# lvrcek/GNNome-assembly

Measured on AMD Instinct MI355X. Metric: GatedGCN edges/sec fwd+bwd, chr19 assembly graph, higher is better.
Workload: dtype f32 (f16x2 split products, f32 accumulate)

## Files before the change

### gnnome_assembly_amd/_lib.py

```python
from __future__ import annotations

import ctypes as C
import os

_HERE = os.path.dirname(os.path.abspath(__file__))
LIB_PATH = os.environ.get("GNM_LIBRARY") or os.path.join(_HERE, "libgnm.so")

_lib = None
ABI_VERSION = 7

_p = C.c_void_p
_i64 = C.c_int64
_i32 = C.c_int
_f32 = C.c_float
_sz = C.c_size_t
_pi = C.POINTER(C.c_int)

SIGNATURES = {
    "gnm_abi_version": (_i32, []),
    "gnm_last_error": (C.c_char_p, []),
    "gnm_num_cus": (_i32, []),
    "gnm_max_partial_blocks": (_i32, []),
    "gnm_graph_build_index": (_i32, [_p, _p, _i64, _i64, _p, _p, _p, _p, _p, _p, _p]),
    "gnm_graph_edge_locality": (_i32, [_p, _p, _i64, _i64, _i64, C.POINTER(C.c_double)]),
    "gnm_graph_locality_order": (_i32, [_p, _p, _i64, _i64, _p, _p, C.POINTER(C.c_double)]),
    "gnm_gemm_f32_workspace_bytes": (_sz, [_i32, _i64, _i64, _i64]),
    "gnm_gemm_f32": (_i32, [_i32, _i64, _i64, _i64, _p, _i64, _p, _i64, _p, _i64, _p, _p, _i64, _i32, _p, _sz, _p]),
    "gnm_gemm_tn_colsum_workspace_bytes": (_sz, [_i64, _i64, _i64]),
    "gnm_gemm_tn_colsum": (_i32, [_i64, _i64, _i64, _p, _i64, _p, _i64, _p, _i64, _p, _p, _sz, _p]),
    "gnm_colsum_workspace_bytes": (_sz, [_i64, _i64]),
    "gnm_colsum_f32": (_i32, [_i64, _i64, _p, _i64, _p, _p, _sz, _p]),
    "gnm_gather_rows_f32": (_i32, [_i64, _i64, _p, _p, _p, _p]),
    "gnm_relu_mask_f32": (_i32, [_i64, _p, _p, _p]),
    "gnm_bn_finalize": (_i32, [_p, _i32, _i64, _i32, _p, _p, _f32, _p, _p]),
    "gnm_bn_bwd_finalize": (_i32, [_p, _i32, _i64, _i32, _p, _p, _p, _p]),
    "gnm_edge_t_stats_fwd": (_i32, [_i64, _i32, _p, _p, _p, _p, _p, _pi, _p]),
    "gnm_edge_gate_fwd": (_i32, [_i64, _i64, _i32, _p, _p, _p, _p, _p, _p, _p, _p, _p, _p]),
    "gnm_node_agg_src_fwd": (_i32, [_i64, _i64, _i32, _p, _p, _p, _p, _p, _p, _p, _p, _p, _p, _pi, _p]),
    "gnm_node_update_fwd": (_i32, [_i64, _i32, _p, _p, _p, _p, _p]),
    "gnm_node_bwd_stats": (_i32, [_i64, _i32, _p, _p, _p, _p, _pi, _p]),
    "gnm_node_bwd_apply": (_i32, [_i64, _i32, _p, _p, _p, _p, _p, _p, _p, _p, _p, _p]),
    "gnm_edge_bwd_dst": (_i32, [_i64, _i64, _i32, _p, _p, _p, _p, _p, _p, _p, _p, _p, _p, _p, _p, _p, _p, _pi, _p]),
    "gnm_edge_bwd_src": (_i32, [_i64, _i64, _i32, _p, _p, _p, _p, _p, _p, _p, _p, _p, _p, _p, _p, _p, _p, _i32, _p]),
    "gnm_edge_bwd_gt": (_i32, [_i64, _i32, _p, _p, _p, _p, _p, _p, _p]),
    "gnm_ln_edge_gate_fwd": (_i32, [_i64, _i64, _i32, _p, _p, _p, _p, _p, _p, _p, _p, _p, _p, _i32, _p]),
    "gnm_ln_node_update_fwd": (_i32, [_i64, _i32, _p, _p, _p, _p, _p, _i32, _p]),
    "gnm_ln_node_bwd": (_i32, [_i64, _i32, _p, _p, _p, _p, _p, _p, _p, _p, _p, _p, _p, _pi, _i32, _p]),
    "gnm_ln_edge_bwd_dst": (_i32, [_i64, _i64, _i32, _p, _p, _p, _p, _p, _p, _p, _p, _p, _p, _p, _p, _pi, _i32, _p]),
    "gnm_ln_edge_bwd_src": (_i32, [_i64, _i64, _i32, _p, _p, _p, _p, _p, _p, _p, _p]),
    "gnm_rowtile_workspace_bytes": (_sz, [_i32]),
    "gnm_set_occupancy_cap": (_i32, [_i32]),
    "gnm_debug_set_variant": (_i32, [C.c_char_p, _i32]),
    "gnm_set_matmul_mode": (_i32, [_i32]),
    "gnm_get_matmul_mode": (_i32, []),
    "gnm_edge_t_fused_fwd": (_i32, [_i64, _i32, _p, _p, _p, _p, _p, _p, _p, _p, _pi, _p, _sz, _p]),
    "gnm_edge_bwd_gt_nn": (_i32, [_i64, _i32, _p, _p, _p, _p, _p, _p, _p, _p, _p, _sz, _p]),
    "gnm_node_proj_fwd": (_i32, [_i64, _i32, _i32, _p, _p, _p, _p, _p, _sz, _p]),
    "gnm_node_proj_bwd_workspace_bytes": (_sz, [_i32]),
    "gnm_node_proj_bwd": (_i32, [_i64, _i32, _i32, _p, _p, _p, _p, _p, _p, _p, _p, _p, _sz, _p]),
    "gnm_node_proj_bwd_nn": (_i32, [_i64, _i32, _i32, _p, _p, _p, _p, _p, _sz, _p]),
    "gnm_node_proj_bwd_tn": (_i32, [_i64, _i32, _i32, _p, _p, _p, _p, _p, _p, _sz, _i32, _p]),
    "gnm_node_proj_bwd_nn_stats": (_i32, [_i64, _i32, _i32, _p, _p, _p, _p, _p, _p, _p, _pi, _p, _sz, _p]),
    "gnm_tn128_bgrad": (_i32, [_i64, _i32, _p, _p, _p, _i64, _p, _p, _p, _p, _p, _p, _p, _p, _p, _p, _p, _sz, _p]),
    "gnm_edge_bwd_chain": (_i32, [_i64, _i64, _i32] + [_p] * 24 + [_pi, _p, _sz, _p]),
    "gnm_edge_bwd_chain_src": (_i32, [_i64, _i64, _i32] + [_p] * 24 + [_p, _i64, _p] + [_pi, _p, _sz, _p]),
    "gnm_edge_bwd_top": (_i32, [_i64, _i64, _i32] + [_p] * 15 + [_p, _i64, _p, _pi, _p, _sz, _p]),
    "gnm_edge_bwd_src_fix": (_i32, [_i64, _p, _i64, _i64, _i32] + [_p] * 10 + [_p]),
    "gnm_node_bgrad": (_i32, [_i64, _i32] + [_p] * 8 + [_i64, _p, _p]),
    "gnm_graph_build_sweep_plan": (_i32, [_p, _p, _p, _i64, _i64, _i64, _i32, _i32, _i64, _p, _p, _p, C.POINTER(C.c_int64), _pi]),
    "gnm_graph_build_sweep_plan_device": (_i32, [_p, _p, _p, _i64, _i64, _i64, _i32, _i32, _i64, _p, _p, _p, _p, _p, _p, _p, _p]),
    "gnm_sweep_partition": (_i32, [_i64, _i32, C.POINTER(C.c_int64), _pi]),
    "gnm_edge_gate2_fwd": (_i32, [_i64, _i64, _i32] + [_p] * 9 + [_i64, _i64] + [_p] * 11 + [_pi, _p]),
    "gnm_ln_edge_gate2_fwd": (_i32, [_i64, _i64, _i32] + [_p] * 4 + [_i32] + [_p] * 6 + [_i64, _i64] + [_p] * 11 + [_pi, _p]),
    "gnm_edge_bwd_fused_workspace_bytes": (_sz, []),
    "gnm_edge_bwd_fused": (_i32, [_i64, _i32, _p, _p, _p, _p, _p, _p, _p, _p, _p, _p, _p, _p, _sz, _p]),
    "gnm_edge_bwd_fused_gt": (_i32, [_i64, _i32, _p, _p, _p, _p, _p, _p, _p, _p, _p, _sz, _p]),
    "gnm_ln_edge_bwd_top": (_i32, [_i64, _i64, _i32, _p, _p, _p, _p, _p, _i32, _p, _p, _p, _p, _p, _p, _p, _p, _p, _p, _p, _i64, _p, _p, _sz, _p]),
    "gnm_ln_edge_bwd_chain": (_i32, [_i64, _i64, _i32, _p, _p, _p, _p, _p, _p, _p, _p, _p, _p, _i32, _p, _p, _p, _p, _p, _p, _p, _p, _p, _p, _p, _i64,
                                     _p, _p, _sz, _p]),
    "gnm_ln_edge_bwd_src_fix": (_i32, [_i64, _p, _i64, _i64, _i32, _p, _p, _p, _p, _p, _p, _p, _p]),
    "gnm_edge_encoder_fwd": (_i32, [_i64, _i32, _i32, _i32, _p, _p, _p, _p, _p, _p, _p, _p]),
    "gnm_edge_encoder_bwd_workspace_bytes": (_sz, []),
    "gnm_edge_encoder_bwd": (_i32, [_i64, _i32, _i32, _i32, _p, _p, _p, _p, _p, _p, _p, _p, _p, _p, _p, _sz, _p]),
    "gnm_edge_encoder_bwd_dx": (_i32, [_i64, _i32, _i32, _i32, _p, _p, _p, _p, _p, _p, _p, _p, _p, _p, _p, _p, _sz, _p]),
    "gnm_predictor_score_fwd": (_i32, [_i64, _i32, _p, _p, _p, _p, _p, _p, _p, _p, _p]),
    "gnm_predictor_score_bwd": (_i32, [_i64, _i32, _p, _p, _p, _p, _p, _pi, _p]),
    "gnm_predictor_fused_workspace_bytes": (_sz, []),
    "gnm_predictor_fused_fwd": (_i32, [_i64, _i32, _i32, _p, _p, _i64, _p, _p, _p, _p, _p, _p, _p, _p, _p, _p, _sz, _p]),
    "gnm_predictor_fused_bwd": (_i32, [_i64, _i32, _i32, _p, _p, _p, _p, _p, _p, _i64, _p, _p, _p, _p, _p, _sz, _p]),
    "gnm_tn128_workspace_bytes": (_sz, []),
    "gnm_tn128": (_i32, [_i64, _p, _i64, _i32, _p, _p, _p, _p, _p, _sz, _p]),
    "gnm_compose_workspace_bytes": (_sz, [_i32]),
    "gnm_compose_partials_doubles": (_sz, []),
    "gnm_layer_forward": (_i32, [_p, _i32, _p, _p, _p, _p]),
    "gnm_stack_backward": (_i32, [_p, _i32, _i32, _p, _p, _p, _p, _p, _p, _p, _p, _p]),
    "gnm_decode_build_adjacency": (_i32, [_p, _p, _i64, _i64, _p, _p, _p, _p, _p, _p]),
    "gnm_decode_iteration": (_i64, [_i64, _p, _p, _p, _p, _p, _p, _p, _p, _p, _p, _i32, _p, _p, _i32, _p, _i64, _p]),
    "gnm_decode_iteration_mt": (_i64, [_i64, _p, _p, _p, _p, _p, _p, _p, _p, _p, _p, _i32, _p, _p, _i32, _p, _i64, _p, _i32]),
    "gnm_decode_sample_workspace_bytes": (_sz, [_i64]),
    "gnm_decode_candidate_sums": (_i32, [_i64, _i64, _p, _p, _p, _p, _p, _sz, _p, _p, _p]),
    "gnm_decode_pick": (_i32, [_i64, _i64, _p, _p, _p, _p, _p, _p, _i32, _p, _p, _p]),
    "gnm_reduce_partials": (_i32, [_p, _i32, _i32, _i32, _p, _p]),
    "gnm_seg_sum_rows": (_i32, [_i64, _i32, _p, _p, _p, _p, _i64, _p]),
    "gnm_pagerank_pe_workspace_bytes": (_sz, [_i64]),
    "gnm_pagerank_pe": (_i32, [_i64, _i64, _p, _p, _p, _i32, C.c_double, _p, _p, _sz, _p]),
    "gnm_edge_feats_zscore": (_i32, [_i64, _p, _p, _p, _p, _sz, _p]),
    "gnm_bce_fwd_bwd": (_i32, [_i64, _p, _p, _f32, _p, _p, _p, _sz, _p]),
}


class GnmError(RuntimeError):
    pass


def load():
    global _lib
    if _lib is not None:
        return _lib
    if not os.path.exists(LIB_PATH):
        raise GnmError(
            f"{LIB_PATH} not found: build it with `python __graft_entry__.py` (hipcc --offload-arch=gfx950). "
            "There is no CPU fallback for the product path.")
    lib = C.CDLL(LIB_PATH)
    for name, (res, args) in SIGNATURES.items():
        try:
# ... 56 lines not shown
```

### gnnome_assembly_amd/csrc/gnm_fused.hip

```cpp
#include <string.h>
#include <type_traits>

#include "gnm_common.h"
#include "gnm_tr.h"

namespace gnm {

typedef float floatx16 __attribute__((ext_vector_type(16)));

constexpr int FH = 128;
constexpr int FTR = 64;
constexpr int FP = FH + 4;
constexpr int FKQ = FH / 8;

using full_t = std::true_type;
using ragged_t = std::false_type;

__global__ void pack_w_k(const float* __restrict__ W, int64_t ld, int ncb, int nn, float* __restrict__ Wp) {
  const int total = ncb * FKQ * 64;
  for (int idx = blockIdx.x * blockDim.x + threadIdx.x; idx < total; idx += gridDim.x * blockDim.x) {
    const int lane = idx & 63, q = (idx >> 6) % FKQ, cb = idx / (64 * FKQ);
    const int i = lane & 31, g = lane >> 5;
    float v[4];
#pragma unroll
// ... 1711 lines not shown

template <class MM>
static int node_proj_fwd_impl(int64_t N, int ncols, const float* h, const float* W, const float* b, float* Pout,
                              void* ws, void* stream) {
  hipStream_t st = (hipStream_t)stream;
  launch_pack<MM>(W, FH, ncols / 32, 0, ws, st);
  GNM_LAUNCH_CHECK("pack_w (NT, node)");
  const int64_t ntiles = cdiv_(N, FTR);
  if constexpr (MM::kSplit) {
    const int ncg = ncols / FH;
    int nslot = (num_cus() * occ_blocks<rowtile_nt_k<MM, false, 1>>()) / ncg / kXcds * kXcds;
    if (nslot > (int)((ntiles + kXcds - 1) / kXcds * kXcds)) nslot = (int)((ntiles + kXcds - 1) / kXcds * kXcds);
    if (nslot < kXcds) nslot = kXcds;
    hipLaunchKernelGGL((rowtile_nt_k<MM, false, 1>), dim3(nslot * ncg), dim3(kBlock), 0, st, N, h, (const void*)ws, b,
                       Pout, (int64_t)ncols, (const float*)nullptr, (const int32_t*)nullptr,
                       (const int32_t*)nullptr, (double*)nullptr, cdiv_(ntiles, nslot), ncg);
  } else {
    const int grid = persistent_grid(ntiles, 2, occ_blocks<rowtile_nt_k<MM, false, 5>>());
    hipLaunchKernelGGL((rowtile_nt_k<MM, false, 5>), dim3(grid), dim3(kBlock), 0, st, N, h, (const void*)ws, b, Pout,
                       (int64_t)ncols, (const float*)nullptr, (const int32_t*)nullptr,
                       (const int32_t*)nullptr, (double*)nullptr, cdiv_(ntiles, grid), 1);
  }
  GNM_LAUNCH_CHECK("node_proj_fwd");
  return 0;
}

extern "C" int gnm_node_proj_fwd(int64_t N, int H, int ncols, const float* h, const float* W, const float* b,
                                 float* Pout, void* ws, size_t ws_bytes, void* stream) {
  GNM_CHECK_ARG(H == FH, "node_proj_fwd: H=%d (only 128 is built)", H);
  GNM_CHECK_ARG(N > 0 && ncols == 5 * FH && h && W && b && Pout, "node_proj_fwd: bad argument (ncols must be 5*128)");
  GNM_CHECK_ARG(ws && ws_bytes >= gnm_rowtile_workspace_bytes(ncols), "node_proj_fwd: workspace too small");
  return g_matmul_mode == 2 ? node_proj_fwd_impl<MmH2>(N, ncols, h, W, b, Pout, ws, stream)
         : g_matmul_mode  ? node_proj_fwd_impl<MmB3>(N, ncols, h, W, b, Pout, ws, stream)
                          : node_proj_fwd_impl<MmF32>(N, ncols, h, W, b, Pout, ws, stream);
}

namespace gnm {
int edge_bwd_chain_launch(const ChainArgs& in, const float* W3, void* wpack, hipStream_t st, bool h2 = false);
}
extern "C" size_t gnm_edge_bwd_fused_workspace_bytes(void);

static int edge_bwd_chain_impl(int64_t N, int64_t E, int H, const float* ge, float* ge_out, const float* t_hi,
                               const float* e_mid, const float* stat_hi, const float* bstat_hi, const float* gamma_hi,
                               const float* W3_hi, float* gW3_hi, float* gb3_hi, double* partials_hi,
                               const float* t_lo, const float* stat_lo, const float* P_lo, const float* Q_lo,
                               const float* hf_lo, const float* hb_lo, const int32_t* isrc, const int32_t* idst,
                               const int32_t* in_ptr, float* gP_lo, float* Ud_lo, float* Td_lo, double* partials_lo,
                               const uint32_t* sinfo, int64_t plan_nodes_per_block, float* UT_lo,
                               int* nblk_out, void* ws, size_t ws_bytes, void* stream) {
  GNM_CHECK_ARG(H == FH, "edge_bwd_chain: H=%d (only 128 is built)", H);
  GNM_CHECK_ARG(g_matmul_mode >= 1, "edge_bwd_chain: only built for the split matmul modes");
  GNM_CHECK_ARG(N > 0 && E > 0 && ge && ge_out && t_hi && e_mid && stat_hi && bstat_hi && gamma_hi && W3_hi && gW3_hi &&
                    gb3_hi && partials_hi && t_lo && stat_lo && P_lo && Q_lo && hf_lo && hb_lo && isrc && idst && in_ptr &&
                    gP_lo && Ud_lo && Td_lo && partials_lo && nblk_out && partials_hi != partials_lo,
                "edge_bwd_chain: null / aliased argument");
  GNM_CHECK_ARG(ws && ws_bytes >= gnm_edge_bwd_fused_workspace_bytes(), "edge_bwd_chain: workspace %zu < %zu", ws_bytes,
                gnm_edge_bwd_fused_workspace_bytes());
  hipStream_t st = (hipStream_t)stream;
  float* slab = (float*)((char*)ws + gnm_rowtile_workspace_bytes(FH));
  ChainArgs a{};
  a.E = E; a.N = N;
  a.ge = ge; a.ge_out = ge_out; a.t_hi = t_hi; a.e_mid = e_mid;
  a.stat_hi = stat_hi; a.bstat_hi = bstat_hi; a.gamma_hi = gamma_hi;
  a.slab = slab; a.partials = partials_hi;
  a.t_lo = t_lo; a.stat_lo = stat_lo; a.P_lo = P_lo; a.Q_lo = Q_lo; a.hf_lo = hf_lo; a.hb_lo = hb_lo;
  a.isrc = isrc; a.idst = idst; a.in_ptr = in_ptr;
  a.gP_lo = gP_lo; a.Ud_lo = Ud_lo; a.Td_lo = Td_lo; a.partials_lo = partials_lo;
  a.sinfo = sinfo; a.UT_lo = UT_lo; a.margin = kSweepMargin;
  a.ud_pitch = Td_lo == Ud_lo + FH ? 2 * FH : FH;
  int64_t npb = 0;
  gnm_sweep_partition(N, 1, &npb, nullptr);
  GNM_CHECK_ARG((npb + 2 * kSweepMargin) * 5 * FH * 4 < (int64_t)INT32_MAX, "edge_bwd_chain: %lld nodes per workgroup exceed the 32-bit buffer offsets",
                (long long)npb);
  if (sinfo) {
    GNM_CHECK_ARG(UT_lo, "edge_bwd_chain_src: UT_lo is null");
    GNM_CHECK_ARG(plan_nodes_per_block == npb, "edge_bwd_chain_src: the sweep plan was built for %lld nodes per workgroup, the kernel uses %lld "
                  "(gnm_sweep_partition(N, 1))", (long long)plan_nodes_per_block, (long long)npb);
  }
  const int grid = edge_bwd_chain_launch(a, W3_hi, ws, st, g_matmul_mode == 2);
  GNM_LAUNCH_CHECK("edge_bwd_chain");
  hipLaunchKernelGGL(slab_reduce_k, dim3(FH * FH / 128), dim3(256), 0, st, (const float*)slab, grid, FH * FH, gW3_hi);
  GNM_LAUNCH_CHECK("edge_bwd_chain slab reduce");
  *nblk_out = grid;
  return gnm_reduce_partials(partials_hi, grid, 1, FH, gb3_hi, stream) ? -3 : 0;
}

extern "C" int gnm_edge_bwd_top(int64_t N, int64_t E, int H, float* ge, const float* e_out, const float* t,
                                const float* stat_e, const float* P, const float* Q, const float* hf, const float* hb,
                                const int32_t* isrc, const int32_t* idst, const int32_t* in_ptr, float* gP, float* Ud,
                                float* Td, double* partials, const uint32_t* sinfo, int64_t plan_nodes_per_block,
                                float* UT, int* nblk_out, void* ws, size_t ws_bytes, void* stream) {
  GNM_CHECK_ARG(H == FH || (H == 2 * FH && sinfo), "edge_bwd_top: H=%d (128; 256 with a sweep plan, one sweep per 128-column half)", H);
  GNM_CHECK_ARG(N > 0 && E > 0 && ge && e_out && t && stat_e && P && Q && hf && hb && isrc && idst && in_ptr && gP && Ud &&
                    Td && partials && nblk_out && (!sinfo || UT), "edge_bwd_top: null argument");
  GNM_CHECK_ARG(ws && ws_bytes >= gnm_edge_bwd_fused_workspace_bytes(), "edge_bwd_top: workspace %zu < %zu", ws_bytes,
                gnm_edge_bwd_fused_workspace_bytes());
  int64_t npb = 0;
  gnm_sweep_partition(N, 1, &npb, nullptr);
  GNM_CHECK_ARG((npb + 2 * kSweepMargin) * 5 * H * 4 < (int64_t)INT32_MAX, "edge_bwd_top: %lld nodes per workgroup exceed the 32-bit buffer offsets",
                (long long)npb);
  GNM_CHECK_ARG(!sinfo || plan_nodes_per_block == npb, "edge_bwd_top: the sweep plan was built for %lld nodes per workgroup, the kernel uses %lld",
                (long long)plan_nodes_per_block, (long long)npb);
  for (int c0 = 0; c0 < H; c0 += FH) {
    ChainArgs a{};
    a.E = E; a.N = N; a.hfull = H;
    a.ge = ge + c0; a.ge_out = ge + c0; a.e_mid = e_out + c0;
    a.slab = (float*)((char*)ws + gnm_rowtile_workspace_bytes(FH));
    a.t_lo = t + c0; a.stat_lo = stat_e + c0; a.P_lo = P + c0; a.Q_lo = Q + c0; a.hf_lo = hf + c0; a.hb_lo = hb + c0;
    a.isrc = isrc; a.idst = idst; a.in_ptr = in_ptr;
    a.gP_lo = gP + c0; a.Ud_lo = Ud + c0; a.Td_lo = Td + c0; a.partials_lo = partials + c0;
    a.sinfo = sinfo; a.UT_lo = UT ? UT + c0 : nullptr; a.margin = kSweepMargin;
    a.ud_pitch = Td == Ud + H ? 2 * H : H;
    const int g = edge_bwd_chain_launch(a, nullptr, nullptr, (hipStream_t)stream);
    GNM_CHECK_ARG(g > 0, "edge_bwd_top: no kernel for this configuration");
    *nblk_out = g;
    GNM_LAUNCH_CHECK("edge_bwd_top");
  }
  return 0;
}

extern "C" int gnm_ln_edge_bwd_top(int64_t N, int64_t E, int H, float* ge, const float* e_out, const float* t, const float* gamma_e,
                                   const float* beta_e, int width, const float* P, const float* Q, const float* hf, const float* hb,
                                   const int32_t* isrc, const int32_t* idst, const int32_t* in_ptr, float* gP, float* gt,
                                   double* partials, const uint32_t* sinfo, int64_t plan_nodes_per_block, int* nblk_out, void* ws,
                                   size_t ws_bytes, void* stream) {
  GNM_CHECK_ARG(H == FH, "ln_edge_bwd_top: H=%d (only 128 is built)", H);
  GNM_CHECK_ARG(width >= 1 && width <= H, "ln_edge_bwd_top: width must be in [1, H]");
  GNM_CHECK_ARG(N > 0 && E > 0 && ge && e_out && t && gamma_e && beta_e && P && Q && hf && hb && isrc && idst && in_ptr && gP && gt &&
                    partials && sinfo && nblk_out, "ln_edge_bwd_top: null argument");
  GNM_CHECK_ARG(ws && ws_bytes >= gnm_edge_bwd_fused_workspace_bytes(), "ln_edge_bwd_top: workspace %zu < %zu", ws_bytes,
                gnm_edge_bwd_fused_workspace_bytes());
  int64_t npb = 0;
  gnm_sweep_partition(N, 1, &npb, nullptr);
  GNM_CHECK_ARG((npb + 2 * kSweepMargin) * 5 * H * 4 < (int64_t)INT32_MAX, "ln_edge_bwd_top: %lld nodes per workgroup exceed the 32-bit buffer offsets",
                (long long)npb);
  GNM_CHECK_ARG(plan_nodes_per_block == npb, "ln_edge_bwd_top: the sweep plan was built for %lld nodes per workgroup, the kernel uses %lld",
                (long long)plan_nodes_per_block, (long long)npb);
  ChainArgs a{};
  a.E = E; a.N = N; a.hfull = H;
  a.ge = ge; a.ge_out = ge; a.e_mid = e_out;
  a.slab = (float*)((char*)ws + gnm_rowtile_workspace_bytes(FH));
  a.t_lo = t; a.P_lo = P; a.Q_lo = Q; a.q_pitch = 4 * H; a.qb_off = 2 * H; a.hf_lo = hf; a.hb_lo = hb;
  a.isrc = isrc; a.idst = idst; a.in_ptr = in_ptr;
  a.gP_lo = gP; a.Ud_lo = gP + 4 * H; a.Td_lo = gP + 4 * H; a.ud_pitch = 5 * H;
  a.UT_lo = gP + 3 * H; a.ut_pitch = 5 * H;
  a.partials_lo = partials;
  a.sinfo = sinfo; a.margin = kSweepMargin;
  a.ln_gamma = gamma_e; a.ln_beta = beta_e; a.ln_width = width; a.gt_out = gt;
  const int g = edge_bwd_chain_launch(a, nullptr, nullptr, (hipStream_t)stream);
  GNM_CHECK_ARG(g > 0, "ln_edge_bwd_top: no kernel for this configuration");
  *nblk_out = g;
  GNM_LAUNCH_CHECK("ln_edge_bwd_top");
  return 0;
}

extern "C" int gnm_ln_edge_bwd_chain(int64_t N, int64_t E, int H, float* ge, const float* gt_hi, const float* e_mid, const float* W3_hi,
                                     float* gW3_hi, float* gb3_hi, double* partials_hi, const float* t_lo, const float* gamma_lo,
                                     const float* beta_lo, int width, const float* P_lo, const float* Q_lo, const float* hf_lo,
                                     const float* hb_lo, const int32_t* isrc, const int32_t* idst, const int32_t* in_ptr, float* gP_lo,
                                     float* gt_lo, double* partials_lo, const uint32_t* sinfo, int64_t plan_nodes_per_block,
                                     int* nblk_out, void* ws, size_t ws_bytes, void* stream) {
  GNM_CHECK_ARG(H == FH, "ln_edge_bwd_chain: H=%d (only 128 is built)", H);
  GNM_CHECK_ARG(g_matmul_mode >= 1, "ln_edge_bwd_chain: only built for the split matmul modes");
  GNM_CHECK_ARG(width >= 1 && width <= H, "ln_edge_bwd_chain: width must be in [1, H]");
  GNM_CHECK_ARG(N > 0 && E > 0 && ge && gt_hi && e_mid && W3_hi && gW3_hi && gb3_hi && partials_hi && t_lo && gamma_lo && beta_lo && P_lo &&
// ... 272 lines not shown
  GNM_LAUNCH_CHECK("pack_w (NN, node, stats)");
  constexpr int T = 4;
  const int64_t ngroups = cdiv_(N, NR3 * T);
  const int grid = persistent_grid(ngroups, 1, h2 ? occ_blocks<rowtile_nn2_k<MmH2, T>>() : occ_blocks<rowtile_nn2_k<MmB3, T>>());
  const Nn2Args a{N, gP, (int64_t)ncols, ncg, (const void*)ws, gh_out, gh_in, cdiv_(ngroups, grid), z_lo, stat_h_lo, partials};
  if (h2) hipLaunchKernelGGL((rowtile_nn2_k<MmH2, T>), dim3(grid), dim3(kBlock), 0, st, a);
  else hipLaunchKernelGGL((rowtile_nn2_k<MmB3, T>), dim3(grid), dim3(kBlock), 0, st, a);
  *nblk_out = grid;
  GNM_LAUNCH_CHECK("node_proj_bwd_nn_stats");
  return 0;
}

extern "C" int gnm_node_proj_bwd_tn(int64_t N, int H, int ncols, const float* gP, const float* h_in, float* gW, float* gb,
                                    double* partials, void* ws, size_t ws_bytes, int max_blocks_per_cu, void* stream) {
  GNM_CHECK_ARG(H == FH, "node_proj_bwd_tn: H=%d (only 128 is built)", H);
  GNM_CHECK_ARG(N > 0 && ncols > 0 && ncols % FH == 0 && gP && h_in && gW && gb && partials && max_blocks_per_cu >= 0,
                "node_proj_bwd_tn: bad argument");
  GNM_CHECK_ARG(ws && ws_bytes >= gnm_node_proj_bwd_workspace_bytes(ncols), "node_proj_bwd_tn: workspace too small");
  float* slab = (float*)((char*)ws + gnm_rowtile_workspace_bytes(ncols));
  return tn_colgroups(N, gP, ncols, ncols / FH, h_in, gW, gb, partials, slab, stream, max_blocks_per_cu);
}

extern "C" int gnm_node_proj_bwd(int64_t N, int H, int ncols, const float* gP, const float* h_in, const float* W,
                                 const float* gh_out, float* gh_in, float* gW, float* gb, double* partials,
                                 void* ws, size_t ws_bytes, void* stream) {
  GNM_CHECK_ARG(ws && ws_bytes >= gnm_node_proj_bwd_workspace_bytes(ncols), "node_proj_bwd: workspace too small");
  const int rc = gnm_node_proj_bwd_nn(N, H, ncols, gP, W, gh_out, gh_in, ws, ws_bytes, stream);
  return rc ? rc : gnm_node_proj_bwd_tn(N, H, ncols, gP, h_in, gW, gb, partials, ws, ws_bytes, 0, stream);
}

extern "C" size_t gnm_tn128_workspace_bytes(void) { return (size_t)kMaxPartialBlocks * FH * FH * sizeof(float); }

extern "C" int gnm_tn128(int64_t M, const float* A, int64_t lda, int ncg, const float* B, float* out, float* colsum,
                         double* partials, void* ws, size_t ws_bytes, void* stream) {
  GNM_CHECK_ARG(M > 0 && A && B && out && colsum && partials && ncg > 0 && lda >= (int64_t)ncg * FH && ncg <= 16,
                "tn128: bad argument");
  GNM_CHECK_ARG(ws && ws_bytes >= gnm_tn128_workspace_bytes(), "tn128: workspace too small");
  return tn_colgroups(M, A, lda, ncg, B, out, colsum, partials, (float*)ws, stream);
}

extern "C" int gnm_tn128_bgrad(int64_t M, int H, const float* UT, const float* Ud, const float* Td, int64_t ud_pitch,
                               const float* stat_e, const float* bstat_e, const float* gamma_e, const int32_t* in_ptr,
                               const int32_t* out_ptr, float* gP, const float* B, float* out, float* colsum,
                               double* partials, void* ws, size_t ws_bytes, void* stream) {
  GNM_CHECK_ARG(H == FH, "tn128_bgrad: H=%d (only 128 is built)", H);
  GNM_CHECK_ARG(g_matmul_mode >= 1, "tn128_bgrad: split matmul modes only");
  GNM_CHECK_ARG(M > 0 && UT && Ud && Td && (ud_pitch == H || ud_pitch == 2 * H) && stat_e && bstat_e && gamma_e && in_ptr &&
                    out_ptr && gP && B && out && colsum && partials, "tn128_bgrad: bad argument");
  GNM_CHECK_ARG(ws && ws_bytes >= gnm_tn128_workspace_bytes(), "tn128_bgrad: workspace too small");
  const TnConv cv{{UT, Ud}, {UT + H, Td}, {(int64_t)2 * H, ud_pitch}, {out_ptr, in_ptr}, stat_e, bstat_e, gamma_e,
                  gP + 3 * H, (int64_t)5 * H};
  return tn_colgroups(M, nullptr, 0, 2, B, out, colsum, partials, (float*)ws, stream, 0, &cv);
}
```

### gnnome_assembly_amd/csrc/gnm_sweep.hip

```cpp
#include <type_traits>

#include "gnm_tr.h"
#include "gnm_ln.h"

namespace gnm {

int gate2_wg();
constexpr int GT = 512;
constexpr int GR = kSweepTileRows;
typedef unsigned int u32x4g_ __attribute__((ext_vector_type(4)));

struct Gate2Args {
  int64_t N, E;
  const float* t; const float* e_in; const float* stat; const float* P;
  const int32_t* isrc; const int32_t* idst; const int32_t* in_ptr;
  const uint32_t* sinfo; const uint32_t* dinfo;
  float* e_out; float* hf; float* inv_f; float* hb; float* inv_b;
  int64_t nodes_per_block, margin;
  const float* gamma; const float* beta; int width;
};

constexpr int G2_LDS = 3 * GR * SW * 4 + 2 * kSweepSlots * SW * 4 + 2 * 2 * SW * 4 + 2 * SW * 4 + 3 * 4 * GR * 4;

__device__ __forceinline__ u32x4g_ bits4g(const float4& v) {
  const u32x4g_ b = {__builtin_bit_cast(unsigned, v.x), __builtin_bit_cast(unsigned, v.y),
                     __builtin_bit_cast(unsigned, v.z), __builtin_bit_cast(unsigned, v.w)};
  return b;
}

template <bool RES, bool INV, int HF, bool LN = false>
__global__ __launch_bounds__(GT, 4) void edge_gate2_fwd_k(const Gate2Args a) {
  static_assert(!LN || HF == SW, "the LayerNorm sweep is built for 128-wide layers");
  __shared__ __attribute__((aligned(16))) unsigned char lds[G2_LDS];
  float* i1 = reinterpret_cast<float*>(lds);
  float* i2 = i1 + GR * SW;
  float* i3 = i2 + GR * SW;
  float* sslots = i3 + GR * SW;
  float* dslots = sslots + 2 * kSweepSlots * SW;
  float* cs = dslots + 2 * 2 * SW;
  int* ring = reinterpret_cast<int*>(cs + 2 * SW);
  const int tid = threadIdx.x;
  const int row = tid >> 5, c4 = (tid & 31) * 4;
  const int chunk = xcd_chunk(blockIdx.x, gridDim.x);
  const int64_t v0 = (int64_t)chunk * a.nodes_per_block < a.N ? (int64_t)chunk * a.nodes_per_block : a.N;
  const int64_t v1 = v0 + a.nodes_per_block < a.N ? v0 + a.nodes_per_block : a.N;
  const int64_t rb = a.in_ptr[v0], re = a.in_ptr[v1];
  const int64_t ntile = (re - rb + GR - 1) / GR;
  for (int c = tid; c < SW; c += GT) {
    cs[c] = LN ? a.gamma[c] : a.stat[2 * HF + c];
    cs[SW + c] = LN ? a.beta[c] : a.stat[3 * HF + c];
  }
  const int64_t vbase = v0 - a.margin;
  const int nspan = (int)(v1 - v0 + 2 * a.margin);
  const __amdgpu_buffer_rsrc_t rs_e = __builtin_amdgcn_make_buffer_rsrc(a.e_out + rb * HF, 0, (int)(re - rb) * HF * 4, 0x00020000);
  const __amdgpu_buffer_rsrc_t rs_hf = __builtin_amdgcn_make_buffer_rsrc(a.hf + v0 * HF, 0, (int)(v1 - v0) * HF * 4, 0x00020000);
  const __amdgpu_buffer_rsrc_t rs_if = __builtin_amdgcn_make_buffer_rsrc(INV ? a.inv_f + v0 * HF : a.hf, 0, INV ? (int)(v1 - v0) * HF * 4 : 0, 0x00020000);
  const __amdgpu_buffer_rsrc_t rs_hb = __builtin_amdgcn_make_buffer_rsrc(a.hb + vbase * HF, 0, nspan * HF * 4, 0x00020000);
  const __amdgpu_buffer_rsrc_t rs_ib = __builtin_amdgcn_make_buffer_rsrc(INV ? a.inv_b + vbase * HF : a.hb, 0, INV ? nspan * HF * 4 : 0, 0x00020000);
  __syncthreads();
  if (ntile == 0) return;

  float4 ptA, peA = f4(0.f), ptB, peB = f4(0.f), ptC, peC = f4(0.f);
  float4 ga2, ga3;
  int fs = 0, fd = 0;
  unsigned fi = 0, fj = 0;
  const int64_t klast = ntile - 1;
  auto clamp_row = [&](int64_t k) __attribute__((always_inline)) {
    const int64_t left = re - (rb + k * GR);
    const int nv = left < GR ? (int)left : GR;
    return row < nv ? row : nv - 1;
  };
  auto prefetch_idx = [&](int64_t k) __attribute__((always_inline)) {
    const int cr = clamp_row(k);
    const int64_t r = rb + k * GR + cr;
    fs = a.isrc[r];
    fd = a.idst[r];
    const unsigned w1 = a.sinfo[r], w2 = a.dinfo[r];
    fi = cr == row ? w1 : 0u;
    fj = cr == row ? w2 : 0u;
  };
  auto prefetch_rows = [&](int64_t k, float4& pt, float4& pe_) __attribute__((always_inline)) {
    const int64_t o = (rb + k * GR + clamp_row(k)) * HF + c4;
    pt = ld4_nt(a.t + o);
    if constexpr (RES) pe_ = ld4_nt(a.e_in + o);
  };
  auto gather = [&](int64_t s, int64_t d) __attribute__((always_inline)) {
    ga2 = ld4(a.P + s * (5 * HF) + HF + c4);
    ga3 = ld4(a.P + d * (5 * HF) + 2 * HF + c4);
  };
  auto ring_put = [&](int64_t k) __attribute__((always_inline)) {
    if ((tid & 31) == 0) {
      int* rk = ring + (int)(k % 3) * 4 * GR;
      rk[row] = fs;
      rk[GR + row] = fd;
      rk[2 * GR + row] = (int)fi;
      rk[3 * GR + row] = (int)fj;
    }
  };
  prefetch_idx(0);
  ring_put(0);
  const int s0 = fs, d0 = fd;
  prefetch_idx(klast < 1 ? klast : 1);
  prefetch_rows(0, ptA, peA);
  prefetch_rows(klast < 1 ? klast : 1, ptB, peB);
  prefetch_rows(klast < 2 ? klast : 2, ptC, peC);
  gather(s0, d0);
  const float4 sc = ld4(cs + c4), sh = ld4(cs + SW + c4);
  const float4 ln_live = LN ? live_mask(c4, a.width) : f4(1.f);
  const float ln_inv_w = LN ? 1.0f / (float)a.width : 0.f;
  auto tile = [&](int64_t k, float4& pt, float4& pe_) __attribute__((always_inline)) {
    const int64_t r0 = rb + k * GR;
    const int nvalid = re - r0 < GR ? (int)(re - r0) : GR;
    const int* rk = ring + (int)(k % 3) * 4 * GR;
    {
      const bool live = row < nvalid;
      float4 x = pt;
      if constexpr (LN) {
        float rstd;
        x = row_normalize<SW>(pt, ln_live, ln_inv_w, rstd);
      }
      const float4 eo = relu4(fma4(x, sc, sh)) + pe_;
      __builtin_amdgcn_raw_buffer_store_b128(bits4g(eo), rs_e, live ? (int)(((k * GR + row) * HF + c4) * 4) : (int)0x80000000, 0, 2);
      const float4 sg = live ? sigmoid4(eo) : f4(0.f);
      st4(i1 + row * SW + c4, sg * ga2);
      st4(i2 + row * SW + c4, sg);
      st4(i3 + row * SW + c4, sg * ga3);
      ring_put(k + 1);
    }
    __syncthreads();
    prefetch_idx(k + 2 < klast ? k + 2 : klast);
    prefetch_rows(k + 3 < klast ? k + 3 : klast, pt, pe_);
    {
      const int* rn = ring + (int)((k + 1) % 3) * 4 * GR;
      gather(rn[row], rn[GR + row]);
    }
    {
      const unsigned wd = (unsigned)rk[3 * GR + row], ws_ = (unsigned)rk[2 * GR + row];
      const unsigned md = wd & 0xffffu;
      unsigned ms = ws_ & 0xffffu;
      const int nd = __builtin_popcount(md);
      float4 dn_ = ld4(i1 + row * SW + c4), dd = ld4(i2 + row * SW + c4);
      float4 sn_ = ld4(i3 + row * SW + c4), sdn = dd;
      float* pd = dslots + ((wd >> 16) & 1u) * SW + c4;
      float* ps = sslots + ((ws_ >> 16) & (kSweepSlots - 1)) * SW + c4;
      const float4 e1 = ld4(pd), e2 = ld4(pd + 2 * SW);
      const float4 q1 = ld4(ps), q2 = ld4(ps + kSweepSlots * SW);
      float4 x1[3] = {f4(0.f), f4(0.f), f4(0.f)}, x2[3] = {f4(0.f), f4(0.f), f4(0.f)};
#pragma unroll
      for (int j = 0; j < 3; ++j) {
        if (j + 1 < nd) {
          x1[j] = ld4(i1 + (row + 1 + j) * SW + c4);
          x2[j] = ld4(i2 + (row + 1 + j) * SW + c4);
        }
      }
#pragma unroll
      for (int j = 0; j < 3; ++j) {
        dn_ += x1[j];
        dd += x2[j];
      }
      for (int j = 4; j < nd; ++j) {
        dn_ += ld4(i1 + (row + j) * SW + c4);
        dd += ld4(i2 + (row + j) * SW + c4);
      }
      ms &= ms - 1;
      while (ms) {
        const int b = __builtin_ctz(ms);
        ms &= ms - 1;
        sn_ += ld4(i3 + b * SW + c4);
        sdn += ld4(i2 + b * SW + c4);
      }
      const bool ld_ = md != 0, ls_ = (ws_ & 0xffffu) != 0;
      if (ld_ && !(wd & kSweepOpen)) { dn_ += e1; dd += e2; }
      if (ls_ && !(ws_ & kSweepOpen)) { sn_ += q1; sdn += q2; }
      if (ld_ && !(wd & kSweepClose)) { st4(pd, dn_); st4(pd + 2 * SW, dd); }
      if (ls_ && !(ws_ & kSweepClose)) { st4(ps, sn_); st4(ps + kSweepSlots * SW, sdn); }
      const bool outd = ld_ && (wd & kSweepClose), outs = ls_ && (ws_ & kSweepClose);
      if (__builtin_amdgcn_ballot_w64(outd) != 0) {
        const float4 inv = make_float4(1.f / (dd.x + kEpsDen), 1.f / (dd.y + kEpsDen), 1.f / (dd.z + kEpsDen), 1.f / (dd.w + kEpsDen));
        const int o = outd ? ((rk[GR + row] - (int)v0) * HF + c4) * 4 : (int)0x80000000;
        __builtin_amdgcn_raw_buffer_store_b128(bits4g(dn_ * inv), rs_hf, o, 0, 2);
        if constexpr (INV) __builtin_amdgcn_raw_buffer_store_b128(bits4g(inv), rs_if, o, 0, 2);
      }
      if (__builtin_amdgcn_ballot_w64(outs) != 0) {
        const float4 inv = make_float4(1.f / (sdn.x + kEpsDen), 1.f / (sdn.y + kEpsDen), 1.f / (sdn.z + kEpsDen), 1.f / (sdn.w + kEpsDen));
        const int o = outs ? ((rk[row] - (int)vbase) * HF + c4) * 4 : (int)0x80000000;
        __builtin_amdgcn_raw_buffer_store_b128(bits4g(sn_ * inv), rs_hb, o, 0, 2);
        if constexpr (INV) __builtin_amdgcn_raw_buffer_store_b128(bits4g(inv), rs_ib, o, 0, 2);
      }
    }
    __syncthreads();
  };
  for (int64_t k = 0; k < ntile; k += 3) {
    tile(k, ptA, peA);
    if (k + 1 < ntile) tile(k + 1, ptB, peB);
    if (k + 2 < ntile) tile(k + 2, ptC, peC);
  }
}

template <int HF>
__global__ __launch_bounds__(256) void gate2_empty_segments_k(int64_t N, const int32_t* __restrict__ in_ptr,
                                                              float* __restrict__ hf, float* __restrict__ inv_f) {
  const int lane = threadIdx.x & 63;
  const int64_t wave0 = ((int64_t)blockIdx.x * 4 + (threadIdx.x >> 6)) * 64;
  const int64_t stride = (int64_t)gridDim.x * 4 * 64;
  for (int64_t base = wave0; base < N; base += stride) {
    const int64_t v = base + lane;
    const bool empty = v < N && in_ptr[v + 1] == in_ptr[v];
    unsigned long long m = __ballot(empty);
    while (m) {
      const int b = __ffsll((long long)m) - 1;
      m &= m - 1;
      const int64_t u = base + b;
      const int c4 = (lane & 31) * 4;
      if (lane < 32) st4(hf + u * HF + c4, f4(0.f));
      else if (inv_f) st4(inv_f + u * HF + c4, f4(1.f / kEpsDen));
    }
  }
}

template <int HF>
__global__ __launch_bounds__(kBlock, 8) void node_agg_src_fix_k(int64_t nfix, const int32_t* __restrict__ fix_nodes,
                                                                const float* __restrict__ e_out, const float* __restrict__ P,
                                                                const int32_t* __restrict__ out_ptr,
                                                                const int32_t* __restrict__ out_pos,
                                                                const int32_t* __restrict__ out_dst, float* __restrict__ hb,
                                                                float* __restrict__ inv_b) {
  constexpr int H = SW, G = H / 4, RPW = 64 / G;
  const int lane = threadIdx.x & 63;
  const int wave = __builtin_amdgcn_readfirstlane(threadIdx.x >> 6);
  const int sub = lane / G, c4 = (lane % G) * 4;
  for (int64_t i = (int64_t)blockIdx.x * kWavesPerBlock + wave; i < nfix; i += (int64_t)gridDim.x * kWavesPerBlock) {
    const int64_t v = fix_nodes[i];
    if (v < 0) continue;
    const int a = out_ptr[v], b = out_ptr[v + 1];
    float4 num = f4(0.f), den = f4(0.f);
    for (int64_t m = a + sub; m < b; m += RPW) {
      const int64_t j = out_pos[m], d = out_dst[m];
      const float4 sg = sigmoid4(ld4_nt(e_out + j * HF + c4));
      num = fma4(sg, ld4(P + d * (5 * HF) + 2 * HF + c4), num);
      den += sg;
    }
#pragma unroll
    for (int off = G; off < 64; off <<= 1) {
      num += shfl_xor4(num, off);
      den += shfl_xor4(den, off);
    }
    if (sub == 0) {
      const float4 inv = make_float4(1.f / (den.x + kEpsDen), 1.f / (den.y + kEpsDen), 1.f / (den.z + kEpsDen),
                                     1.f / (den.w + kEpsDen));
      st4_nt(hb + v * HF + c4, num * inv);
      if (inv_b) st4_nt(inv_b + v * HF + c4, inv);
    }
  }
}

template <int HF>
__global__ __launch_bounds__(kBlock) void node_z_stats_k(int64_t N, const float* __restrict__ P, const float* __restrict__ hf,
                                                         const float* __restrict__ hb, float* __restrict__ z,
                                                         double* __restrict__ partials, int64_t rows_per_block) {
  constexpr int H = SW, G = H / 4, RPW = 64 / G;
  __shared__ double lds[kWavesPerBlock * 2 * H];
  const int lane = threadIdx.x & 63, wave = threadIdx.x >> 6;
  const int sub = lane / G, c4 = (lane % G) * 4;
  const int chunk = xcd_chunk(blockIdx.x, gridDim.x);
  const int64_t r0 = (int64_t)chunk * rows_per_block;
  const int64_t r1 = min(N, r0 + rows_per_block);
  Stat4 st;
  st.zero();
  for (int64_t v = r0 + wave * RPW + sub; v < r1; v += kWavesPerBlock * RPW) {
    const float4 zz = ld4_nt(P + v * (5 * HF) + c4) + ld4_nt(hf + v * HF + c4) + ld4_nt(hb + v * HF + c4);
    st4_nt(z + v * HF + c4, zz);
    st.add_prod(zz, zz);
  }
  block_stat_store<H, HF>(st, lds, partials, chunk);
}

}

using namespace gnm;

extern "C" int gnm_sweep_partition(int64_t N, int wg_per_cu, int64_t* nodes_per_block, int* grid_out) {
  GNM_CHECK_ARG(N > 0 && nodes_per_block && wg_per_cu >= 1 && wg_per_cu <= 8, "sweep_partition: bad argument");
  const int grid = persistent_grid(N, 64, wg_per_cu, 8);
  *nodes_per_block = (N + grid - 1) / grid;
  if (grid_out) *grid_out = grid;
  return 0;
}

static int edge_gate2_fwd_impl(int64_t N, int64_t E, int H, const float* t, const float* e_in, const float* stat_e,
                               const float* ln_gamma, const float* ln_beta, int ln_width,
                               const float* P, const int32_t* isrc, const int32_t* idst, const int32_t* in_ptr,
                               const uint32_t* sinfo, const uint32_t* dinfo, int64_t plan_nodes_per_block,
                               int64_t nfix, const int32_t* fix_nodes, const int32_t* out_ptr, const int32_t* out_pos,
                               const int32_t* out_dst, float* e_out, float* hf, float* inv_f, float* hb, float* inv_b,
                               float* z, double* partials, int* nblk_out, void* stream) {
  GNM_CHECK_ARG(H == SW || (H == 2 * SW && !ln_gamma), "edge_gate2_fwd: H=%d (128 and 256 are built; LayerNorm: 128)", H);
  GNM_CHECK_ARG(N > 0 && E > 0 && t && (stat_e || ln_gamma) && P && isrc && idst && in_ptr && sinfo && dinfo && (nfix == 0 || fix_nodes) &&
                    nfix >= 0 && out_ptr && out_pos && out_dst && e_out && hf && hb && z && partials && nblk_out &&
                    (inv_f != nullptr) == (inv_b != nullptr),
                "edge_gate2_fwd: null/neg argument");
  hipStream_t st = (hipStream_t)stream;
  Gate2Args a{};
  a.N = N; a.E = E; a.t = t; a.e_in = e_in; a.stat = stat_e; a.P = P; a.isrc = isrc; a.idst = idst; a.in_ptr = in_ptr;
  a.sinfo = sinfo; a.dinfo = dinfo; a.e_out = e_out; a.hf = hf; a.inv_f = inv_f; a.hb = hb; a.inv_b = inv_b;
  a.margin = kSweepMargin;
  a.gamma = ln_gamma; a.beta = ln_beta; a.width = ln_width;
  int grid = 0;
  gnm_sweep_partition(N, gate2_wg(), &a.nodes_per_block, &grid);
  GNM_CHECK_ARG(plan_nodes_per_block == a.nodes_per_block, "edge_gate2_fwd: the sweep plan was built for %lld nodes per workgroup, the "
                "kernel uses %lld (gnm_sweep_partition(N, %d))", (long long)plan_nodes_per_block, (long long)a.nodes_per_block, gate2_wg());
  GNM_CHECK_ARG((a.nodes_per_block + 2 * kSweepMargin) * H * 4 < (int64_t)INT32_MAX && (E / grid + 64) * H * 4 < (int64_t)INT32_MAX,
                "edge_gate2_fwd: a workgroup's share exceeds the 32-bit buffer offsets");
  const int gz = H == SW ? persistent_grid(N, 256, occ_blocks<node_z_stats_k<SW>>()) : persistent_grid(N, 256, occ_blocks<node_z_stats_k<2 * SW>>());
  auto run = [&](auto hf_tag, int c0) -> int {
    constexpr int HF = decltype(hf_tag)::value;
    Gate2Args b = a;
    b.t = t + c0; b.e_in = e_in ? e_in + c0 : nullptr; b.stat = stat_e ? stat_e + c0 : nullptr; b.P = P + c0; b.e_out = e_out + c0; b.hf = hf + c0;
    b.inv_f = inv_f ? inv_f + c0 : nullptr; b.hb = hb + c0; b.inv_b = inv_b ? inv_b + c0 : nullptr;
    hipLaunchKernelGGL(gate2_empty_segments_k<HF>, dim3(num_cus() * 2), dim3(256), 0, st, N, in_ptr, b.hf, b.inv_f);
    auto launch = [&](auto ln_tag) {
      constexpr bool LN_ = decltype(ln_tag)::value;
      if (e_in && inv_f) hipLaunchKernelGGL((edge_gate2_fwd_k<true, true, HF, LN_>), dim3(grid), dim3(GT), 0, st, b);
      else if (e_in) hipLaunchKernelGGL((edge_gate2_fwd_k<true, false, HF, LN_>), dim3(grid), dim3(GT), 0, st, b);
      else if (inv_f) hipLaunchKernelGGL((edge_gate2_fwd_k<false, true, HF, LN_>), dim3(grid), dim3(GT), 0, st, b);
      else hipLaunchKernelGGL((edge_gate2_fwd_k<false, false, HF, LN_>), dim3(grid), dim3(GT), 0, st, b);
    };
    if constexpr (HF == SW) {
      if (ln_gamma) launch(std::true_type{});
      else launch(std::false_type{});
    } else {
      launch(std::false_type{});
    }
    GNM_LAUNCH_CHECK("edge_gate2_fwd");
    if (nfix > 0) {
      int64_t g2 = (nfix + kWavesPerBlock - 1) / kWavesPerBlock;
      const int64_t cap = (int64_t)num_cus() * 8;
      if (g2 > cap) g2 = cap;
      hipLaunchKernelGGL(node_agg_src_fix_k<HF>, dim3((int)g2), dim3(kBlock), 0, st, nfix, fix_nodes, b.e_out, b.P, out_ptr, out_pos,
                         out_dst, b.hb, b.inv_b);
      GNM_LAUNCH_CHECK("edge_gate2_fwd fix");
    }
    hipLaunchKernelGGL(node_z_stats_k<HF>, dim3(gz), dim3(kBlock), 0, st, N, b.P, b.hf, b.hb, z + c0, partials + c0, (N + gz - 1) / gz);
    GNM_LAUNCH_CHECK("edge_gate2_fwd z");
    return 0;
  };
  if (H == SW) {
    if (run(std::integral_constant<int, SW>{}, 0)) return -2;
  } else {
    for (int c0 = 0; c0 < H; c0 += SW)
      if (run(std::integral_constant<int, 2 * SW>{}, c0)) return -2;
  }
  *nblk_out = gz;
  return 0;
}

extern "C" int gnm_edge_gate2_fwd(int64_t N, int64_t E, int H, const float* t, const float* e_in, const float* stat_e,
                                  const float* P, const int32_t* isrc, const int32_t* idst, const int32_t* in_ptr,
                                  const uint32_t* sinfo, const uint32_t* dinfo, int64_t plan_nodes_per_block,
                                  int64_t nfix, const int32_t* fix_nodes, const int32_t* out_ptr, const int32_t* out_pos,
                                  const int32_t* out_dst, float* e_out, float* hf, float* inv_f, float* hb, float* inv_b,
                                  float* z, double* partials, int* nblk_out, void* stream) {
  GNM_CHECK_ARG(stat_e, "edge_gate2_fwd: stat_e is null");
  return edge_gate2_fwd_impl(N, E, H, t, e_in, stat_e, nullptr, nullptr, 0, P, isrc, idst, in_ptr, sinfo, dinfo, plan_nodes_per_block, nfix,
                             fix_nodes, out_ptr, out_pos, out_dst, e_out, hf, inv_f, hb, inv_b, z, partials, nblk_out, stream);
}

extern "C" int gnm_ln_edge_gate2_fwd(int64_t N, int64_t E, int H, const float* t, const float* e_in, const float* gamma_e,
                                     const float* beta_e, int width, const float* P, const int32_t* isrc, const int32_t* idst,
                                     const int32_t* in_ptr, const uint32_t* sinfo, const uint32_t* dinfo, int64_t plan_nodes_per_block,
                                     int64_t nfix, const int32_t* fix_nodes, const int32_t* out_ptr, const int32_t* out_pos,
                                     const int32_t* out_dst, float* e_out, float* hf, float* inv_f, float* hb, float* inv_b,
                                     float* z, double* partials, int* nblk_out, void* stream) {
  GNM_CHECK_ARG(gamma_e && beta_e && width >= 1 && width <= H, "ln_edge_gate2_fwd: null argument or width outside [1, H]");
  return edge_gate2_fwd_impl(N, E, H, t, e_in, nullptr, gamma_e, beta_e, width, P, isrc, idst, in_ptr, sinfo, dinfo, plan_nodes_per_block, nfix,
                             fix_nodes, out_ptr, out_pos, out_dst, e_out, hf, inv_f, hb, inv_b, z, partials, nblk_out, stream);
}
```

### gnnome_assembly_amd/csrc/gnm_tr.h

```cpp
#pragma once
#include "gnm_common.h"

namespace gnm {

typedef float floatx16 __attribute__((ext_vector_type(16)));
typedef __bf16 bf16x8 __attribute__((ext_vector_type(8)));
typedef __bf16 bf16x4 __attribute__((ext_vector_type(4)));
typedef __attribute__((__vector_size__(4 * sizeof(__bf16)))) __bf16 tr_bf16x4;

constexpr int SW = 128;
constexpr int SPITCH = SW * 2;

__device__ __forceinline__ int swz(int r) { return ((r & 3) << 2) | ((0x78 >> (((r >> 2) & 3) * 2)) & 3); }
__device__ __forceinline__ int simg_off(int r, int c) {
  return r * SPITCH + ((((c >> 3) ^ swz(r)) << 4) | ((c & 4) << 1));
}

__device__ __forceinline__ void split3f(const float4& v, bf16x4& hi, bf16x4& mid, bf16x4& lo) {
  const float x[4] = {v.x, v.y, v.z, v.w};
#pragma unroll
  for (int j = 0; j < 4; ++j) {
    const __bf16 h = (__bf16)x[j];
    const float r1 = x[j] - (float)h;
    const __bf16 m = (__bf16)r1;
// ... 124 lines not shown
  const tr_bf16x4 b = __builtin_amdgcn_ds_read_tr16_b64_v4bf16((lds_ptr)(img + base1_x_mb));
  bf16x8 f;
#pragma unroll
  for (int j = 0; j < 4; ++j) {
    f[j] = a[j];
    f[4 + j] = b[j];
  }
  return f;
}

__device__ __forceinline__ h16x8 simg_col_frag_h(const unsigned char* img, int k0, int c0, int lane) {
  return __builtin_bit_cast(h16x8, simg_col_frag(img, k0, c0, lane));
}

typedef float floatx4_acc __attribute__((ext_vector_type(4)));
__device__ __forceinline__ void mfb16s(floatx4_acc& acc, const bf16x8& a, const bf16x8& b) {
  acc = __builtin_amdgcn_mfma_f32_16x16x32_bf16(a, b, acc, 0, 0, 0);
}
__device__ __forceinline__ void mfh16s(floatx4_acc& acc, const h16x8& a, const h16x8& b) {
  acc = __builtin_amdgcn_mfma_f32_16x16x32_f16(a, b, acc, 0, 0, 0);
}
__device__ __forceinline__ void mfb16(floatx16& acc, const bf16x8& a, const bf16x8& b) {
  acc = __builtin_amdgcn_mfma_f32_32x32x16_bf16(a, b, acc, 0, 0, 0);
}

__device__ __forceinline__ constexpr int b3_pa(int t) { return t == 0 ? 2 : (t == 2 || t == 3) ? 1 : 0; }
__device__ __forceinline__ constexpr int b3_pb(int t) { return t == 1 ? 2 : (t == 2 || t == 4) ? 1 : 0; }

struct ChainArgs {
  int64_t E, N;
  const float* ge; float* ge_out; const float* t_hi; const float* e_mid;
  const float* stat_hi; const float* bstat_hi; const float* gamma_hi; const bf16x8* Wp;
  float* slab; double* partials;
  const float* t_lo; const float* stat_lo; const float* P_lo; const float* Q_lo; const float* hf_lo; const float* hb_lo;
  const int32_t* isrc; const int32_t* idst; const int32_t* in_ptr;
  float* gP_lo; float* Ud_lo; float* Td_lo; double* partials_lo;
  int64_t nodes_per_block;
  const uint32_t* sinfo; float* UT_lo; int64_t margin; int ud_pitch;
  int hfull;
  const float* ln_gamma; const float* ln_beta; int ln_width; float* gt_out;
  int ut_pitch;
  int q_pitch, qb_off;
};

struct TnConv {
  const float* U[2]; const float* T[2]; int64_t pitch[2]; const int32_t* ptr[2];
  const float* stat_e; const float* bstat_e; const float* gamma_e;
  float* Xw; int64_t ldxw;
};


constexpr int kSweepTileRows = 16;
constexpr int kSweepSlots = 32;
constexpr int64_t kSweepMargin = 1 << 16;
constexpr unsigned kSweepOpen = 1u << 22, kSweepClose = 1u << 23;

}
```

### gnnome_assembly_amd/csrc/gnm_tr.hip

```cpp
#include <stdlib.h>

#include "gnm_tr.h"
#include "gnm_ln.h"

namespace gnm {

constexpr int TRR = 32;
constexpr int TRIMG = TRR * SPITCH;

__device__ __forceinline__ int h2_tn_da(int R, int P) { const int d = R - P; return d > 0 ? (d > 200 ? 100 : d >> 1) : 0; }
template <bool CONV, int OCC, bool H2 = false>
__global__ __launch_bounds__(kBlock, OCC) void tn_tr_k(int64_t M, const float* __restrict__ A, int64_t lda, int ncg,
                                                     const void* __restrict__ Bv, int64_t ldb, int ncgb,
                                                     float* __restrict__ slab, double* __restrict__ partials, int nslot,
                                                     int64_t tiles_per_slot, const TnConv cv) {
  const float* __restrict__ B = reinterpret_cast<const float*>(Bv);
  __shared__ __attribute__((aligned(16))) unsigned char lds[6 * TRIMG];
  unsigned char* ia = lds;
  unsigned char* ib = lds + 3 * TRIMG;
  const int tid = threadIdx.x, lane = tid & 63;
  const int wave = __builtin_amdgcn_readfirstlane(tid >> 6);
  const int li = lane & 31, lg = lane >> 5;
  const int wn = wave >> 1, wc = wave & 1;
  const int xcd = blockIdx.x % kXcds, jj = blockIdx.x / kXcds;
// ... 572 lines not shown
#pragma unroll
    for (int k = 0; k < 8; ++k) s_ += all[4 * (32 * k + (tid >> 2)) + (tid & 3)];
    partials[(size_t)chunk * SW + tid] = s_;
  }
}

int eb_variant();
size_t edge_bwd_tr_pack_bytes() { return (size_t)(SW / 16) * (SW / 32) * 3 * 64 * sizeof(bf16x8); }
int edge_bwd_tr_launch(int64_t E, const float* ge, float* ge_out, const float* t, const float* e_in, const float* stat_e,
                       const float* bstat_e, const float* gamma_e, const float* W3, void* wpack, float* slab,
                       double* partials, hipStream_t st, bool h2, bool given) {
  if (h2) {
    hipLaunchKernelGGL(pack_w2_nn16_k, dim3(SW / 16), dim3(256), 0, st, W3, (int64_t)SW, (unsigned char*)wpack);
    const int64_t ntiles = (E + ER - 1) / ER;
    const int grid = persistent_grid(ntiles, 16, occ_blocks<edge_bwd_tr_k<3, true>>());
    if (given)
      hipLaunchKernelGGL((edge_bwd_tr_k<7, true>), dim3(grid), dim3(kBlock), 0, st, E, ge, ge_out, t, e_in, stat_e, bstat_e, gamma_e,
                         (const bf16x8*)wpack, slab, partials, (ntiles + grid - 1) / grid);
    else
      hipLaunchKernelGGL((edge_bwd_tr_k<3, true>), dim3(grid), dim3(kBlock), 0, st, E, ge, ge_out, t, e_in, stat_e, bstat_e, gamma_e,
                         (const bf16x8*)wpack, slab, partials, (ntiles + grid - 1) / grid);
    return grid;
  }
  hipLaunchKernelGGL(pack_w3_nn16_k, dim3(8), dim3(256), 0, st, W3, (int64_t)SW, (bf16x8*)wpack);
  const int64_t ntiles = (E + ER - 1) / ER;
  if (given) {
    const int grid = persistent_grid(ntiles, 16, occ_blocks<edge_bwd_tr_k<3>>());
    hipLaunchKernelGGL(edge_bwd_tr_k<7>, dim3(grid), dim3(kBlock), 0, st, E, ge, ge_out, t, e_in, stat_e, bstat_e, gamma_e,
                       (const bf16x8*)wpack, slab, partials, (ntiles + grid - 1) / grid);
    return grid;
  }
  const int var = eb_variant();
  const int grid = persistent_grid(ntiles, 16, occ_blocks<edge_bwd_tr_k<3>>());
#define GNM_EB_LAUNCH(V)                                                                                               \
  hipLaunchKernelGGL(edge_bwd_tr_k<V>, dim3(grid), dim3(kBlock), 0, st, E, ge, ge_out, t, e_in, stat_e, bstat_e, gamma_e, \
                     (const bf16x8*)wpack, slab, partials, (ntiles + grid - 1) / grid)
  if (var == 2) GNM_EB_LAUNCH(0);
  else GNM_EB_LAUNCH(3);
#undef GNM_EB_LAUNCH
  return grid;
}


constexpr int CT = 512;
constexpr int WG_ = 4;
typedef unsigned int u32x4_ __attribute__((ext_vector_type(4)));
constexpr int CH_LDS = 6 * EIMG + ER * EOP * 4 + 7 * SW * 4 + 4 * SW * 4 + 5 * ER * SW * 4 + 3 * 2 * ER * 4;
constexpr int CH_LDS_SRC = CH_LDS + 3 * ER * 4 + ER * SW * 4 + 3 * kSweepSlots * SW * 4;
static_assert(ER == kSweepTileRows, "the sweep plan is built for the chained kernel's tile");
static_assert(CH_LDS % 16 == 0 && CH_LDS_SRC <= 160 * 1024, "LDS layout");

struct W3Frag16 { bf16x8 w[SW / 32][3]; };

template <int ABL, bool SRC, bool WSKIP = true, bool HI = true, int HF = SW, bool H2 = false, bool LN = false>
__global__ __launch_bounds__(CT, 2) void edge_bwd_chain_k(const ChainArgs a) {
  static_assert(HF == SW || !HI, "the chained (matrix) half of the kernel is built for 128-wide layers only");
  static_assert(HI || !H2, "f16x2 belongs to the matrix half");
  static_assert(!LN || (SRC && HF == SW), "the LayerNorm sweep: two-sided, 128 wide");
  __shared__ __attribute__((aligned(16))) unsigned char lds[(SRC ? CH_LDS_SRC : CH_LDS) + (LN ? ER * SW * 4 : 0)];
  unsigned char* ig = lds;
  unsigned char* ie = lds + 3 * EIMG;
  float* og = reinterpret_cast<float*>(lds + 6 * EIMG);
  float* cs = og + ER * EOP;
  float* cl = cs + 7 * SW;
  float* v1 = cl + 4 * SW;
  float* v2 = v1 + ER * SW;
  float* v3 = v2 + ER * SW;
  float* tl = v3 + ER * SW;
  float* ef = tl + ER * SW;
  int* sd = reinterpret_cast<int*>(ef + ER * SW);
  unsigned* si = reinterpret_cast<unsigned*>(sd + 3 * 2 * ER);
  float* v5 = reinterpret_cast<float*>(si + 3 * ER);
  float* slots = v5 + ER * SW;
  float* v6 = slots + 3 * kSweepSlots * SW;
  const int tid = threadIdx.x, lane = tid & 63;
  const int wave = __builtin_amdgcn_readfirstlane(tid >> 6);
  const int li = lane & 31, lg = lane >> 5;
  const int wn = wave >> 2, wc = wave & 3;
  const int chunk = xcd_chunk(blockIdx.x, gridDim.x);
  const int64_t v0 = (int64_t)chunk * a.nodes_per_block < a.N ? (int64_t)chunk * a.nodes_per_block : a.N;
  const int64_t v1n = v0 + a.nodes_per_block < a.N ? v0 + a.nodes_per_block : a.N;
  const int64_t rb = a.in_ptr[v0], re = a.in_ptr[v1n];
  const int64_t ntile = (re - rb + ER - 1) / ER;
  const int row = tid >> 5, lc4 = (tid & 31) * 4;
  for (int c = tid; c < SW; c += CT) {
    if constexpr (HI && !LN) {
      cs[c] = a.stat_hi[c];
      cs[SW + c] = a.stat_hi[SW + c];
      cs[2 * SW + c] = a.stat_hi[2 * SW + c];
      cs[3 * SW + c] = a.stat_hi[3 * SW + c];
      cs[4 * SW + c] = a.bstat_hi[c];
      cs[5 * SW + c] = a.bstat_hi[SW + c];
      cs[6 * SW + c] = a.gamma_hi[c] * a.stat_hi[SW + c];
    }
    if constexpr (LN) {
      cl[2 * SW + c] = a.ln_gamma[c];
      cl[3 * SW + c] = a.ln_beta[c];
    } else {
      cl[c] = a.stat_lo[c];
      cl[SW + c] = a.stat_lo[HF + c];
      cl[2 * SW + c] = a.stat_lo[2 * HF + c];
      cl[3 * SW + c] = a.stat_lo[3 * HF + c];
    }
  }
  W3Frag16 wf;
  h16x8 wfh[H2 ? SW / 32 : 1][2];
  float cinv = 1.f;
  if constexpr (HI && !H2) {
    const bf16x8* p = a.Wp + ((int64_t)wave * (SW / 32) * 3) * 64 + lane;
#pragma unroll
    for (int kc = 0; kc < SW / 32; ++kc)
#pragma unroll
      for (int s_ = 0; s_ < 3; ++s_) wf.w[kc][s_] = p[(kc * 3 + s_) * 64];
  }
  if constexpr (H2) {
    const unsigned char* wp = reinterpret_cast<const unsigned char*>(a.Wp);
    const h16x8* p = reinterpret_cast<const h16x8*>(wp) + ((int64_t)wave * (SW / 32) * 2) * 64 + lane;
#pragma unroll
    for (int kc = 0; kc < SW / 32; ++kc)
#pragma unroll
      for (int s_ = 0; s_ < 2; ++s_) wfh[kc][s_] = p[(kc * 2 + s_) * 64];
    cinv = reinterpret_cast<const float*>(wp + kW2Nn16FragBytes)[wave * 16 + (lane & 15)];
  }
  int* const rexp = reinterpret_cast<int*>(lds + 2 * EIMG);
  float* const rinv = reinterpret_cast<float*>(lds + 2 * EIMG) + ER;
  constexpr int kNoRef = -100000;
  int Rref = kNoRef;
  if constexpr (H2) { if (tid == 0) rexp[2 * ER] = 0; }
  floatx16 tn[2];
#pragma unroll
  for (int x = 0; x < 2; ++x)
#pragma unroll
    for (int e = 0; e < 16; ++e) tn[x][e] = 0.f;
  double cg0 = 0.0, cg1 = 0.0, cg2 = 0.0, cg3 = 0.0;
  const int trq0 = simg_tr_base(lane, 0), trq1 = simg_tr_base(lane, 1);
  const int ni = lane & 15, ng = lane >> 4;
  const int nnb = ni * SPITCH + ((((ni & 3) << 2) | (ng ^ (swz(ni) & 3))) << 4);
  const bool walker = wave < 3 && lane < 32 && !(LN && wave == 1), bnsum = tid >= 256;
  const int role = wave, wc4 = (tid & 31) * 4;
  const int brow = 2 * ((tid - 256) >> 5);
  int cur = -1;
  float4 acc0 = f4(0.f);
  double s_gu[4] = {0.0, 0.0, 0.0, 0.0}, s_gut[4] = {0.0, 0.0, 0.0, 0.0};
  float* const wout = role == 0 ? a.gP_lo + 2 * HF : role == 1 ? a.Td_lo : a.Ud_lo;
  const int wpitch32 = role == 0 ? 5 * HF : a.ud_pitch;
  const __amdgpu_buffer_rsrc_t wrs = __builtin_amdgcn_make_buffer_rsrc(wout + v0 * wpitch32, 0, (int)(v1n - v0) * wpitch32 * 4, 0x00020000);
  float* const dummy_row = a.slab + (size_t)(gridDim.x + chunk) * SW * SW + lc4;
  const int64_t vbase = v0 - a.margin;
  const int nspan = (int)(v1n - v0 + 2 * a.margin);
  const __amdgpu_buffer_rsrc_t srs_g = __builtin_amdgcn_make_buffer_rsrc(
      SRC ? a.gP_lo + vbase * (5 * HF) + HF : a.gP_lo, 0, SRC ? nspan * 5 * HF * 4 : 0, 0x00020000);
  const int utp = a.ut_pitch ? a.ut_pitch : 2 * HF;
  const __amdgpu_buffer_rsrc_t srs_u = __builtin_amdgcn_make_buffer_rsrc(
      SRC ? a.UT_lo + vbase * utp : a.gP_lo, 0, SRC ? nspan * utp * 4 : 0, 0x00020000);
  const int qp = a.q_pitch ? a.q_pitch : 2 * HF, qbo = a.q_pitch ? a.qb_off : HF;
  const float4 ln_live = LN ? live_mask((tid & 31) * 4, a.ln_width) : f4(1.f);
  const float ln_inv_w = LN ? 1.0f / (float)a.ln_width : 0.f;
  __syncthreads();

  float4 pg, pt, pe_, pl;
  float4 gt_keep = f4(0.f);
  int row_ea = 0;
  float4 ga2, gqb, ghb, gqf, ghf, ga3;
  int fs = 0, fd = 0;
  unsigned fi = 0;
  const int64_t klast = ntile - 1;
  auto clamp_row = [&](int64_t k) __attribute__((always_inline)) {
    const int64_t left = re - (rb + k * ER);
    const int nv = left < ER ? (int)left : ER;
    return row < nv ? row : nv - 1;
  };
  auto prefetch_idx = [&](int64_t k) __attribute__((always_inline)) {
    const int cr = clamp_row(k);
    const int64_t r = rb + k * ER + cr;
    fs = a.isrc[r];
    fd = a.idst[r];
    if constexpr (SRC) {
      const unsigned w = a.sinfo[r];
      fi = cr == row ? w : 0u;
    }
  };
  auto prefetch_rows = [&](int64_t k) __attribute__((always_inline)) {
    const int64_t r0 = rb + k * ER;
    const int o = clamp_row(k) * HF + lc4;
    pg = ld4(a.ge + r0 * HF + o);
    if constexpr (HI) pt = ld4(a.t_hi + r0 * HF + o);
    pe_ = ld4(a.e_mid + r0 * HF + o);
    pl = ld4_nt(a.t_lo + r0 * HF + o);
  };
  auto gather = [&](int64_t s, int64_t d) __attribute__((always_inline)) {
    ga2 = ld4(a.P_lo + s * (5 * HF) + HF + lc4);
// ... 210 lines not shown
#pragma unroll
      for (int r4 = 0; r4 < ER; r4 += WG_) {
        int dn[WG_];
        float4 xs[WG_];
#pragma unroll
        for (int q = 0; q < WG_; ++q) {
          dn[q] = __builtin_amdgcn_readfirstlane(sdk[ER + r4 + q]);
          xs[q] = ld4(vsrc + (r4 + q) * SW);
        }
        const int dafter = r4 + WG_ < ER ? __builtin_amdgcn_readfirstlane(sdk[ER + r4 + WG_])
                                         : (k == klast ? -1 : __builtin_amdgcn_readfirstlane(sd[(int)((k + 1) % 3) * 2 * ER + ER]));
#pragma unroll
        for (int q = 0; q < WG_; ++q) {
          const float keep = dn[q] == cur ? 1.f : 0.f;
          acc0 = fma4(acc0, f4(keep), xs[q]);
          cur = dn[q];
          const bool ends = (q + 1 < WG_ ? dn[q + 1] : dafter) != cur;
          const u32x4_ bits = {__builtin_bit_cast(unsigned, acc0.x), __builtin_bit_cast(unsigned, acc0.y),
                               __builtin_bit_cast(unsigned, acc0.z), __builtin_bit_cast(unsigned, acc0.w)};
          if (WSKIP) { if (ends) __builtin_amdgcn_raw_buffer_store_b128(bits, wrs, ((cur - (int)v0) * wpitch32 + wc4) * 4, 0, 0); }
          else __builtin_amdgcn_raw_buffer_store_b128(bits, wrs, ends ? ((cur - (int)v0) * wpitch32 + wc4) * 4 : (int)0x80000000, 0, 0);
        }
      }
    }
    if (!(ABL & 1) && bnsum) {
#pragma unroll
      for (int q = 0; q < 2; ++q) {
        const float4 x = ld4((LN ? v6 : v2) + (brow + q) * SW + wc4);
        const float4 th = ld4(v3 + (brow + q) * SW + wc4);
        s_gu[0] += (double)x.x; s_gu[1] += (double)x.y; s_gu[2] += (double)x.z; s_gu[3] += (double)x.w;
        s_gut[0] += (double)x.x * (double)th.x; s_gut[1] += (double)x.y * (double)th.y;
        s_gut[2] += (double)x.z * (double)th.z; s_gut[3] += (double)x.w * (double)th.w;
      }
    }
    if constexpr (SRC) {
      auto bits4 = [](const float4& v) __attribute__((always_inline)) {
        const u32x4_ b = {__builtin_bit_cast(unsigned, v.x), __builtin_bit_cast(unsigned, v.y),
                          __builtin_bit_cast(unsigned, v.z), __builtin_bit_cast(unsigned, v.w)};
        return b;
      };
      if (!(ABL & 1) && !(ABL & 8) && wave >= 3) {
        const int q = (tid - 192) >> 5;
        const unsigned* sik = si + (int)(k % 3) * ER;
        const int rr[2] = {q, (q + 10) & (ER - 1)};
        unsigned w[2] = {sik[rr[0]], q + 10 < ER ? sik[rr[1]] : 0u};
        float4 s1[2], s2[2], s3[2], p1[2], p2[2], p3[2];
        unsigned m[2];
#pragma unroll
        for (int u = 0; u < 2; ++u) {
          m[u] = w[u] & 0xffffu;
          const int b = rr[u];
          s1[u] = ld4(v5 + b * SW + wc4);
          s2[u] = ld4(v2 + b * SW + wc4);
          s3[u] = ld4(v3 + b * SW + wc4);
          const float* p = slots + ((w[u] >> 16) & (kSweepSlots - 1)) * SW + wc4;
          p1[u] = ld4(p);
          p2[u] = ld4(p + kSweepSlots * SW);
          p3[u] = ld4(p + 2 * kSweepSlots * SW);
          m[u] &= m[u] - 1;
        }
#pragma unroll
        for (int u = 0; u < 2; ++u) {
          while (m[u]) {
            const int b = __builtin_ctz(m[u]);
            m[u] &= m[u] - 1;
            s1[u] += ld4(v5 + b * SW + wc4);
            s2[u] += ld4(v2 + b * SW + wc4);
            s3[u] += ld4(v3 + b * SW + wc4);
          }
          const bool lead = (w[u] & 0xffffu) != 0;
          if (lead && !(w[u] & kSweepOpen)) {
            s1[u] += p1[u];
            s2[u] += p2[u];
            s3[u] += p3[u];
          }
          float* p = slots + ((w[u] >> 16) & (kSweepSlots - 1)) * SW + wc4;
          if (lead && !(w[u] & kSweepClose)) {
            st4(p, s1[u]);
            st4(p + kSweepSlots * SW, s2[u]);
            st4(p + 2 * kSweepSlots * SW, s3[u]);
          }
          const bool out = lead && (w[u] & kSweepClose);
          const int sn = sdk[rr[u]] - (int)vbase;
          const int og_ = out ? (sn * (5 * HF) + wc4) * 4 : (int)0x80000000;
          const int ou_ = out ? (sn * utp + wc4) * 4 : (int)0x80000000;
          if (!(ABL & 16) && __builtin_amdgcn_ballot_w64(out) != 0) {
            __builtin_amdgcn_raw_buffer_store_b128(bits4(s1[u]), srs_g, og_, 0, 0);
            __builtin_amdgcn_raw_buffer_store_b128(bits4(s2[u]), srs_u, ou_, 0, 0);
            if constexpr (!LN) __builtin_amdgcn_raw_buffer_store_b128(bits4(s3[u]), srs_u, ou_, HF * 4, 0);
          }
        }
      }
    }
    {
      const int* sdn = sd + (int)((k + 1) % 3) * 2 * ER;
      gather(sdn[row], sdn[ER + row]);
    }
  }

  if constexpr (HI) {
    float* sl = a.slab + (size_t)chunk * SW * SW;
    const float unit = !H2 ? 1.f : Rref == kNoRef ? 0.f : pow2_biased(127 + Rref - 8);
#pragma unroll
    for (int x = 0; x < 2; ++x)
#pragma unroll
      for (int e = 0; e < 16; ++e) {
        const int m = (2 * wn + x) * 32 + (e & 3) + 8 * (e >> 2) + 4 * lg;
        sl[m * SW + wc * 32 + li] = H2 ? tn[x][e] * unit : tn[x][e];
      }
  }
  __syncthreads();
  {
    double* bnr = reinterpret_cast<double*>(lds);
    if (bnsum) {
      const int grp = brow >> 1;
#pragma unroll
      for (int j = 0; j < 4; ++j) {
        bnr[(grp * 2 + 0) * SW + wc4 + j] = s_gu[j];
        bnr[(grp * 2 + 1) * SW + wc4 + j] = s_gut[j];
      }
    }
    __syncthreads();
    if (tid < 2 * SW) {
      double s_ = 0.0;
#pragma unroll
      for (int g8 = 0; g8 < 8; ++g8) s_ += bnr[g8 * 2 * SW + tid];
      a.partials_lo[(size_t)chunk * 2 * HF + (tid / SW) * HF + (tid % SW)] = s_;
    }
    __syncthreads();
  }
  if constexpr (!HI) return;
  double* red = reinterpret_cast<double*>(lds);
  red[row * SW + lc4 + 0] = cg0;
  red[row * SW + lc4 + 1] = cg1;
  red[row * SW + lc4 + 2] = cg2;
  red[row * SW + lc4 + 3] = cg3;
  __syncthreads();
  if (tid < SW) {
    double s_ = 0.0;
#pragma unroll
    for (int k = 0; k < ER; ++k) s_ += red[k * SW + tid];
    a.partials[(size_t)chunk * SW + tid] = s_;
  }
}


template <int HF>
__global__ __launch_bounds__(256) void zero_empty_segments_k(int64_t N, const int32_t* __restrict__ in_ptr,
                                                             float* __restrict__ gP, float* __restrict__ Ud,
                                                             float* __restrict__ Td, int ud_pitch) {
  const int lane = threadIdx.x & 63;
  const int64_t wave0 = ((int64_t)blockIdx.x * 4 + (threadIdx.x >> 6)) * 64;
  const int64_t stride = (int64_t)gridDim.x * 4 * 64;
  for (int64_t base = wave0; base < N; base += stride) {
    const int64_t v = base + lane;
    const bool empty = v < N && in_ptr[v + 1] == in_ptr[v];
    unsigned long long m = __ballot(empty);
    while (m) {
      const int b = __ffsll((long long)m) - 1;
      m &= m - 1;
      const int64_t u = base + b;
      const int c4 = (lane & 31) * 4;
      if (lane < 32) {
        st4(gP + u * (5 * HF) + 2 * HF + c4, f4(0.f));
        st4(Td + u * ud_pitch + c4, f4(0.f));
      } else {
        st4(Ud + u * ud_pitch + c4, f4(0.f));
      }
    }
  }
}

int edge_bwd_chain_launch(const ChainArgs& in, const float* W3, void* wpack, hipStream_t st, bool h2) {
  if (W3 && h2) {
    hipLaunchKernelGGL(pack_w2_nn16_k, dim3(SW / 16), dim3(256), 0, st, W3, (int64_t)SW, (unsigned char*)wpack);
  }
  else if (W3) hipLaunchKernelGGL(pack_w3_nn16_k, dim3(8), dim3(256), 0, st, W3, (int64_t)SW, (bf16x8*)wpack);
  ChainArgs a = in;
  a.Wp = (const bf16x8*)wpack;
  int grid = 0;
  gnm_sweep_partition(a.N, 1, &a.nodes_per_block, &grid);
  if (a.hfull == 2 * SW) {
    hipLaunchKernelGGL(zero_empty_segments_k<2 * SW>, dim3(num_cus() * 2), dim3(256), 0, st, a.N, a.in_ptr, a.gP_lo, a.Ud_lo, a.Td_lo, a.ud_pitch);
    if (a.t_hi || !a.sinfo) return -1;
    hipLaunchKernelGGL((edge_bwd_chain_k<0, true, true, false, 2 * SW>), dim3(grid), dim3(CT), 0, st, a);
    return grid;
  }
  hipLaunchKernelGGL(zero_empty_segments_k<SW>, dim3(num_cus() * 2), dim3(256), 0, st, a.N, a.in_ptr, a.gP_lo, a.Ud_lo, a.Td_lo, a.ud_pitch);
#ifdef GNM_TIMING_ABLATIONS
  static const int abl = getenv("GNM_CHAIN_ABL") ? atoi(getenv("GNM_CHAIN_ABL")) : 0;
  switch (abl) {
    case 1: hipLaunchKernelGGL((edge_bwd_chain_k<1, false>), dim3(grid), dim3(CT), 0, st, a); return grid;
    case 2: hipLaunchKernelGGL((edge_bwd_chain_k<2, false>), dim3(grid), dim3(CT), 0, st, a); return grid;
    case 4: hipLaunchKernelGGL((edge_bwd_chain_k<4, false>), dim3(grid), dim3(CT), 0, st, a); return grid;
    case 7: hipLaunchKernelGGL((edge_bwd_chain_k<7, false>), dim3(grid), dim3(CT), 0, st, a); return grid;
    case 8: if (a.sinfo && a.t_hi) { hipLaunchKernelGGL((edge_bwd_chain_k<8, true>), dim3(grid), dim3(CT), 0, st, a); return grid; } break;
    case 16: if (a.sinfo && a.t_hi) { hipLaunchKernelGGL((edge_bwd_chain_k<16, true>), dim3(grid), dim3(CT), 0, st, a); return grid; } break;
    case 9: if (a.sinfo && a.t_hi) { hipLaunchKernelGGL((edge_bwd_chain_k<9, true>), dim3(grid), dim3(CT), 0, st, a); return grid; } break;
    default: break;
  }
#endif
  if (!a.t_hi) {
    if (a.ln_gamma) {
      if (!a.sinfo || !a.gt_out || !a.ln_beta) return -1;
      hipLaunchKernelGGL((edge_bwd_chain_k<0, true, true, false, SW, false, true>), dim3(grid), dim3(CT), 0, st, a);
      return grid;
    }
    if (a.sinfo) hipLaunchKernelGGL((edge_bwd_chain_k<0, true, true, false>), dim3(grid), dim3(CT), 0, st, a);
    else hipLaunchKernelGGL((edge_bwd_chain_k<0, false, true, false>), dim3(grid), dim3(CT), 0, st, a);
    return grid;
  }
  if (a.ln_gamma) {
    if (!a.sinfo || !a.gt_out || !a.ln_beta) return -1;
    if (h2) hipLaunchKernelGGL((edge_bwd_chain_k<0, true, true, true, SW, true, true>), dim3(grid), dim3(CT), 0, st, a);
    else hipLaunchKernelGGL((edge_bwd_chain_k<0, true, true, true, SW, false, true>), dim3(grid), dim3(CT), 0, st, a);
    return grid;
  }
  if (h2) {
    if (a.sinfo) hipLaunchKernelGGL((edge_bwd_chain_k<0, true, true, true, SW, true>), dim3(grid), dim3(CT), 0, st, a);
    else hipLaunchKernelGGL((edge_bwd_chain_k<0, false, true, true, SW, true>), dim3(grid), dim3(CT), 0, st, a);
    return grid;
  }
  if (a.sinfo) hipLaunchKernelGGL((edge_bwd_chain_k<0, true>), dim3(grid), dim3(CT), 0, st, a);
  else hipLaunchKernelGGL((edge_bwd_chain_k<0, false>), dim3(grid), dim3(CT), 0, st, a);
  return grid;
}

int tn_tr_rows_per_tile() { return TRR; }
int tn_tr_occupancy(bool conv, bool h2) {
  if (h2) return conv ? occ_blocks<tn_tr_k<true, 2, true>>() : occ_blocks<tn_tr_k<false, 2, true>>();
  return conv ? occ_blocks<tn_tr_k<true, 2>>() : occ_blocks<tn_tr_k<false, 2>>();
}
void tn_tr_launch(int64_t M, const float* A, int64_t lda, int ncg, const void* B, int64_t ldb, int ncgb, float* slab,
                  double* partials, int nslot, int64_t tiles_per_slot, hipStream_t st, const TnConv* cv, bool h2) {
  const TnConv none{};
  const dim3 grid(nslot * ncg * (cv ? 1 : ncgb));
#define GNM_TN_LAUNCH(CONV, H2)                                                                                             \
  hipLaunchKernelGGL((tn_tr_k<CONV, 2, H2>), grid, dim3(kBlock), 0, st, M, A, lda, ncg, B, ldb, cv ? 1 : ncgb, slab, partials, \
                     nslot, tiles_per_slot, cv ? *cv : none)
  if (cv && h2) GNM_TN_LAUNCH(true, true);
  else if (cv) GNM_TN_LAUNCH(true, false);
  else if (h2) GNM_TN_LAUNCH(false, true);
  else GNM_TN_LAUNCH(false, false);
#undef GNM_TN_LAUNCH
}

}
```

### gnnome_assembly_amd/engine.py

```python
from __future__ import annotations

import contextlib
import ctypes as C
import functools
import operator
import os
import threading
from dataclasses import dataclass, field
from typing import Dict, List, Optional

import torch

from . import _lib

NT, NN, TN = 0, 1, 2
_D_FUSED = True
EPS_BN = 1e-5

LIN5 = ("A_1", "A_2", "A_3", "B_1", "B_2")

_D_ACTIVATIONS = os.environ.get("GNM_ACTIVATIONS", "saved").strip().lower()


_OPTION_NAMES = ("FUSED", "ACTIVATIONS", "CHAIN", "TN_SIDE", "TN_SIDE_CAP", "SRC_SIDE_CAP", "TN_AT", "TN_SPLIT", "TWO_SIDED", "TWO_SIDED_FWD", "WIDE_FUSED",
                 "NODE_FUSED", "LN_SWEEP")


class Options:
    __slots__ = _OPTION_NAMES

    def __init__(self, **kw):
        for k in _OPTION_NAMES:
            object.__setattr__(self, k, kw[k])

    def __setattr__(self, k, v):
        raise AttributeError("engine.Options is immutable: use replace(), options(...) or set_default(...)")

    def replace(self, **kw) -> "Options":
        bad = [k for k in kw if k not in _OPTION_NAMES]
        if bad:
            raise _lib.GnmError(f"engine.options: unknown switch {bad}; known: {_OPTION_NAMES}")
        if "ACTIVATIONS" in kw and kw["ACTIVATIONS"] not in ("saved", "lean"):
            raise _lib.GnmError(f"activation mode {kw['ACTIVATIONS']!r}: expected 'saved' or 'lean'")
        if "TN_AT" in kw and kw["TN_AT"] not in ("now", "next", "auto"):
            raise _lib.GnmError(f"TN_AT {kw['TN_AT']!r}: expected 'now', 'next' or 'auto'")
        d = {k: getattr(self, k) for k in _OPTION_NAMES}
        d.update(kw)
        return Options(**d)

    def __repr__(self):
        return "Options(" + ", ".join(f"{k}={getattr(self, k)!r}" for k in _OPTION_NAMES) + ")"


_tls = threading.local()
_default: Optional[Options] = None


def current() -> Options:
    o = getattr(_tls, "opts", None)
    return o if o is not None else _default


@contextlib.contextmanager
def use(opts: Optional[Options]):
    if opts is None:
        yield current()
        return
    prev = getattr(_tls, "opts", None)
    _tls.opts = opts
    try:
        yield opts
    finally:
        _tls.opts = prev


@contextlib.contextmanager
def options(**kw):
    with use(current().replace(**kw)) as o:
        yield o


def set_default(**kw) -> None:
    global _default
    _default = _default.replace(**kw)


def _scoped(saved_arg: Optional[int] = None):
    def deco(fn):
        @functools.wraps(fn)
        def w(*a, opts: Optional[Options] = None, **k):
            if opts is None and saved_arg is not None and len(a) > saved_arg:
                opts = getattr(a[saved_arg], "opts", None)
                scoped = getattr(_tls, "opts", None)
                if opts is not None and scoped is not None and scoped is not opts and repr(scoped) != repr(opts):
                    import warnings
                    warnings.warn("engine: this backward runs under the options its forward saved "
# ... 257 lines not shown
    if nperm is None:
        return x
    out = torch.empty_like(x)
    _call("gnm_gather_rows_f32", x.shape[0], x.shape[1], _ptr(x), _ptr(nperm), _ptr(out), _stream())
    return out


def edge_rank(idx) -> torch.Tensor:
    er = idx.get("erank")
    if er is None:
        perm = idx["perm"]
        er = torch.empty_like(perm)
        er[perm.long()] = torch.arange(perm.numel(), dtype=perm.dtype, device=perm.device)
        idx["erank"] = er
    return er


def node_rows_out(idx, x: torch.Tensor) -> torch.Tensor:
    nrank = idx.get("nrank")
    if nrank is None:
        return x
    out = torch.empty_like(x)
    _call("gnm_gather_rows_f32", x.shape[0], x.shape[1], _ptr(x), _ptr(nrank), _ptr(out), _stream())
    return out



@dataclass
class LayerParams:
    W5: torch.Tensor
    b5: torch.Tensor
    W3: torch.Tensor
    b3: torch.Tensor
    gamma_e: torch.Tensor
    beta_e: torch.Tensor
    gamma_h: torch.Tensor
    beta_h: torch.Tensor


@dataclass
class LayerSaved:
    h_in: torch.Tensor = None
    e_in: torch.Tensor = None
    P: torch.Tensor = None
    t: torch.Tensor = None
    stat_e: torch.Tensor = None
    e_out: torch.Tensor = None
    hf: torch.Tensor = None
    inv_f: torch.Tensor = None
    hb: torch.Tensor = None
    inv_b: torch.Tensor = None
    z: torch.Tensor = None
    stat_h: torch.Tensor = None
    opts: "Options" = None
    chunks: list = None
    matmul: str = None


def _proj_and_t(idx, N, E, H, prm, h_in, e_in, nblk):
    lib = _lib.load()
    dev = h_in.device
    sc = scratch(dev)
    st = _stream()
    P = torch.empty(N, 5 * H, dtype=torch.float32, device=dev)
    t = torch.empty(E, H, dtype=torch.float32, device=dev)
    if H == 128 and current().FUSED and h_in.shape[1] == H:
        need = lib.gnm_rowtile_workspace_bytes(5 * H)
        ws = sc.ws(need)
        _call("gnm_node_proj_fwd", N, H, 5 * H, _ptr(h_in), _ptr(prm.W5), _ptr(prm.b5), _ptr(P), _ptr(ws), need, st)
        _call("gnm_edge_t_fused_fwd", E, H, _ptr(e_in), _ptr(prm.W3), _ptr(prm.b3), _ptr(P), _ptr(idx["isrc"]),
              _ptr(idx["idst"]), _ptr(t), _ptr(sc.partials), C.byref(nblk), _ptr(ws), need, st)
    elif H == 256 and current().FUSED and current().WIDE_FUSED and e_in.shape[1] == H and _lib.split_mode():
        gemm(NT, h_in, prm.W5, P, bias=prm.b5)
        need = lib.gnm_rowtile_workspace_bytes(5 * H)
        ws = sc.ws(need)
        _call("gnm_edge_t_fused_fwd", E, H, _ptr(e_in), _ptr(prm.W3), _ptr(prm.b3), _ptr(P), _ptr(idx["isrc"]),
              _ptr(idx["idst"]), _ptr(t), _ptr(sc.partials), C.byref(nblk), _ptr(ws), need, st, tag="gnm_edge_t_fused_fwd[256]")
    else:
        gemm(NT, h_in, prm.W5, P, bias=prm.b5)
        gemm(NT, e_in, prm.W3, t, bias=prm.b3)
        _call("gnm_edge_t_stats_fwd", E, H, _ptr(t), _ptr(P), _ptr(idx["isrc"]), _ptr(idx["idst"]),
              _ptr(sc.partials), C.byref(nblk), st)
    return P, t


@on_device_of(lambda idx, N, E, H, prm, h_in, *a, **k: h_in)
@_scoped()
def layer_forward(idx, N: int, E: int, H: int, prm: LayerParams, h_in, e_in, save: bool, batch_norm: bool = True,
                  residual: bool = True, plan: Optional[dict] = None, ln_width: Optional[int] = None):
    lnw = H if ln_width is None else int(ln_width)
    if residual and h_in.shape[1] != H:
        raise _lib.GnmError("layer_forward: a residual layer needs in_channels == out_channels")
    if H > WIDE_CHUNK:
        return _wide_layer_forward(idx, N, E, H, prm, h_in, e_in, save, batch_norm, residual, plan)
    nblk = C.c_int(0)
    P, t = _proj_and_t(idx, N, E, H, prm, h_in, e_in, nblk)
    return _layer_forward_tail(idx, N, E, H, prm, h_in, e_in, P, t, nblk, save, batch_norm, residual, plan, lnw)


def _layer_forward_tail(idx, N, E, H, prm, h_in, e_in, P, t, nblk, save, batch_norm, residual, plan, lnw):
    res_e = _ptr(e_in) if residual else C.c_void_p(0)
    res_h = _ptr(h_in) if residual else C.c_void_p(0)
    lib = _lib.load()
    dev = h_in.device
    sc = scratch(dev)
    st = _stream()
    f32 = dict(dtype=torch.float32, device=dev)
    e_out = torch.empty(E, H, **f32)
    hf = torch.empty(N, H, **f32)
    two_sided = plan is not None and (H in (128, 256) if batch_norm else H == 128) and current().TWO_SIDED_FWD
    inv_f = torch.empty(N, H, **f32) if (save or not two_sided) else None
    if two_sided and not batch_norm:
        hb = torch.empty(N, H, **f32)
        inv_b = torch.empty(N, H, **f32) if save else None
        z = torch.empty(N, H, **f32)
        stat_e = None
        _call("gnm_ln_edge_gate2_fwd", N, E, H, _ptr(t), res_e, _ptr(prm.gamma_e), _ptr(prm.beta_e), lnw, _ptr(P), _ptr(idx["isrc"]),
              _ptr(idx["idst"]), _ptr(idx["in_ptr"]), _ptr(plan["sinfo"]), _ptr(plan["dinfo"]), plan["nodes_per_block"], plan["nfix"],
              _ptr(plan["fix_nodes"]), _ptr(idx["out_ptr"]), _ptr(idx["out_pos"]), _ptr(idx["out_dst"]), _ptr(e_out),
              _ptr(hf), _ptr(inv_f), _ptr(hb), _ptr(inv_b), _ptr(z), _ptr(sc.partials), C.byref(nblk), st)
    elif two_sided:
        hb = torch.empty(N, H, **f32)
        inv_b = torch.empty(N, H, **f32) if save else None
        z = torch.empty(N, H, **f32)
        stat_e = bn_finalize(sc.partials, nblk.value, E, H, prm.gamma_e, prm.beta_e)
        _call("gnm_edge_gate2_fwd", N, E, H, _ptr(t), res_e, _ptr(stat_e), _ptr(P), _ptr(idx["isrc"]), _ptr(idx["idst"]),
              _ptr(idx["in_ptr"]), _ptr(plan["sinfo"]), _ptr(plan["dinfo"]), plan["nodes_per_block"], plan["nfix"],
              _ptr(plan["fix_nodes"]), _ptr(idx["out_ptr"]), _ptr(idx["out_pos"]), _ptr(idx["out_dst"]), _ptr(e_out),
              _ptr(hf), _ptr(inv_f), _ptr(hb), _ptr(inv_b), _ptr(z), _ptr(sc.partials), C.byref(nblk), st)
    elif batch_norm:
        stat_e = bn_finalize(sc.partials, nblk.value, E, H, prm.gamma_e, prm.beta_e)
        _call("gnm_edge_gate_fwd", N, E, H, _ptr(t), res_e, _ptr(stat_e), _ptr(P), _ptr(idx["isrc"]),
              _ptr(idx["in_ptr"]), _ptr(e_out), _ptr(hf), _ptr(inv_f), st)
    else:
        stat_e = None
        _call("gnm_ln_edge_gate_fwd", N, E, H, _ptr(t), res_e, _ptr(prm.gamma_e), _ptr(prm.beta_e), _ptr(P),
              _ptr(idx["isrc"]), _ptr(idx["in_ptr"]), _ptr(e_out), _ptr(hf), _ptr(inv_f), lnw, st)
    if not two_sided:
        hb = torch.empty(N, H, **f32)
        inv_b = torch.empty(N, H, **f32)
        z = torch.empty(N, H, **f32)
        _call("gnm_node_agg_src_fwd", N, E, H, _ptr(e_out), _ptr(P), _ptr(idx["out_ptr"]),
              _ptr(idx["out_pos"]), _ptr(idx["out_dst"]), _ptr(hf), _ptr(hb),
              _ptr(inv_b), _ptr(z), _ptr(sc.partials), C.byref(nblk), st)
    h_out = torch.empty(N, H, **f32)
    if batch_norm:
        stat_h = bn_finalize(sc.partials, nblk.value, N, H, prm.gamma_h, prm.beta_h)
        _call("gnm_node_update_fwd", N, H, _ptr(z), _ptr(stat_h), res_h, _ptr(h_out), st)
    else:
        stat_h = None
        _call("gnm_ln_node_update_fwd", N, H, _ptr(z), _ptr(prm.gamma_h), _ptr(prm.beta_h), res_h, _ptr(h_out), lnw, st)
    saved = None
    if save:
        lean = current().ACTIVATIONS == "lean"
        saved = LayerSaved(opts=current(), h_in=h_in, e_in=e_in, P=None if lean else P, t=None if lean else t, stat_e=stat_e, e_out=e_out,
                           hf=hf, inv_f=inv_f, hb=hb, inv_b=inv_b, z=z, stat_h=stat_h, matmul=_lib.get_matmul_mode())
    return h_out, e_out, saved


WIDE_CHUNK = 256


def _cols(x: torch.Tensor, c0: int, w: int, blocks: int = 1) -> torch.Tensor:
    R, Hb = x.shape[0], x.shape[1] // blocks
    return x.view(R, blocks, Hb)[:, :, c0:c0 + w].reshape(R, blocks * w).contiguous()


def _put_cols(dst: torch.Tensor, src: torch.Tensor, c0: int, w: int, blocks: int = 1) -> None:
    R, Hb = dst.shape[0], dst.shape[1] // blocks
    dst.view(R, blocks, Hb)[:, :, c0:c0 + w] = src.view(R, blocks, w)


def _chunk_params(prm: LayerParams, c0: int, w: int) -> LayerParams:
    sl = slice(c0, c0 + w)
    return LayerParams(W5=None, b5=None, W3=None, b3=None, gamma_e=prm.gamma_e[sl], beta_e=prm.beta_e[sl],
                       gamma_h=prm.gamma_h[sl], beta_h=prm.beta_h[sl])


def _wide_layer_forward(idx, N, E, H, prm, h_in, e_in, save, batch_norm, residual, plan):
    if not batch_norm:
        raise NotImplementedError(f"GatedGCN_1d with LayerNorm at width {H}: the LayerNorm kernels hold a row in one wavefront "
                                  f"(widths up to {WIDE_CHUNK}); BatchNorm layers run at any width")
    if H % WIDE_CHUNK:
        raise _lib.GnmError(f"layer_forward: a wide layer runs zero-padded to a multiple of {WIDE_CHUNK} (layers.padded_width), got {H}")
    dev = h_in.device
    sc = scratch(dev)
    f32 = dict(dtype=torch.float32, device=dev)
    P = torch.empty(N, 5 * H, **f32)
    t = torch.empty(E, H, **f32)
    gemm(NT, h_in, prm.W5, P, bias=prm.b5)
    gemm(NT, e_in, prm.W3, t, bias=prm.b3)
    h_out, e_out = torch.empty(N, H, **f32), torch.empty(E, H, **f32)
    chunks = []
    w = WIDE_CHUNK
    for c0 in range(0, H, w):
        Pc, tc = _cols(P, c0, w, 5), _cols(t, c0, w)
        hc = _cols(h_in, c0, w) if residual else h_in
        ec = _cols(e_in, c0, w) if residual else e_in
        nblk = C.c_int(0)
        _call("gnm_edge_t_stats_fwd", E, w, _ptr(tc), _ptr(Pc), _ptr(idx["isrc"]), _ptr(idx["idst"]), _ptr(sc.partials), C.byref(nblk),
              _stream())
        ho, eo, sv = _layer_forward_tail(idx, N, E, w, _chunk_params(prm, c0, w), hc, ec, Pc, tc, nblk, save, True, residual, plan, w)
        _put_cols(h_out, ho, c0, w)
        _put_cols(e_out, eo, c0, w)
        if save:
            sv.h_in = sv.e_in = None
            chunks.append(sv)
    saved = LayerSaved(opts=current(), h_in=h_in, e_in=e_in, chunks=chunks, matmul=_lib.get_matmul_mode()) if save else None
    return h_out, e_out, saved
# ... 193 lines not shown
                deferred_first = False
            else:
                g["b3"] = gemm_tn_colsum(gt, s.e_in, g["W3"], out.get("b3"))
            del gt
        else:
            gt = torch.empty(E, H, **f32)
            _call("gnm_edge_bwd_gt", E, H, _ptr(ge), _ptr(s.t), _ptr(s.stat_e), _ptr(bstat_e),
                  _ptr(prm.gamma_e), _ptr(gt), st)
            g["b3"] = gemm_tn_colsum(gt, s.e_in, g["W3"], out.get("b3"))
            if residual:
                gemm(NN, gt, prm.W3, ge, resid=ge)
            else:
                ge = gemm(NN, gt, prm.W3, torch.empty(E, Hin, **f32))
            del gt
    g["W5"] = new("W5", 5 * H, Hin)
    gh_in = torch.empty(N, Hin, **f32)
    if fused:
        g["b5"] = new("b5", 5 * H)
        need = lib.gnm_node_proj_bwd_workspace_bytes(5 * H)
        ws = sc.ws(need)
        _call("gnm_node_proj_bwd_nn", N, H, 5 * H, _ptr(gP), _ptr(prm.W5), _ptr(gh_out), _ptr(gh_in), _ptr(ws), need, st)
        if lane is not None:
            lane.begin()
            lane.node_proj_bwd_tn(N, H, gP, s.h_in, g["W5"], g["b5"])
        else:
            _call("gnm_node_proj_bwd_tn", N, H, 5 * H, _ptr(gP), _ptr(s.h_in), _ptr(g["W5"]), _ptr(g["b5"]),
                  _ptr(sc.partials), _ptr(ws), need, 0, st)
    else:
        gemm(NN, gP, prm.W5, gh_in, resid=gh_out if residual else None)
        if defer_side:
            g["b5"] = new("b5", 5 * H)
            lane.begin() if deferred_first else lane.wait_for_main()
            lane.gemm_tn_colsum(gP, s.h_in, g["W5"], g["b5"])
        else:
            g["b5"] = gemm_tn_colsum(gP, s.h_in, g["W5"], out.get("b5"))
    return gh_in, ge, g


_D_CHAIN = os.environ.get("GNM_CHAIN", "1") != "0"
_D_TN_SIDE = os.environ.get("GNM_TN_SIDE", "1") != "0"
_D_TN_SIDE_CAP = int(os.environ.get("GNM_TN_CAP", "0"))
_D_TN_AT = os.environ.get("GNM_TN_AT", "auto")
TN_AT_NOW_NODES = int(os.environ.get("GNM_TN_AT_NOW_NODES", "1100000"))


def tn_at(N: int) -> str:
    v = current().TN_AT
    return ("now" if N >= TN_AT_NOW_NODES else "next") if v == "auto" else v
_D_TN_SPLIT = os.environ.get("GNM_TN_SPLIT", "1") != "0"
_D_SRC_SIDE_CAP = int(os.environ.get("GNM_SRC_CAP", "4"))


_D_TWO_SIDED = os.environ.get("GNM_TWO_SIDED", "1") != "0"
_D_TWO_SIDED_FWD = os.environ.get("GNM_TWO_SIDED_FWD", "1") != "0"
_D_WIDE_FUSED = os.environ.get("GNM_WIDE_FUSED", "1") != "0"


_D_NODE_FUSED = os.environ.get("GNM_NODE_FUSED", "1") != "0"
_D_LN_SWEEP = os.environ.get("GNM_LN_SWEEP", "1") != "0"


def tn128(N: int, A: torch.Tensor, lda: int, ncg: int, h: torch.Tensor, W, b, partials, ws, need, tag: str = None):
    _call("gnm_tn128", N, _ptr(A), lda, ncg, _ptr(h), _ptr(W), _ptr(b), _ptr(partials), _ptr(ws), need, _stream(), tag=tag)


GATE2_WG = int(os.environ.get("GNM_GATE2_WG", "2"))


def sweep_width(H: int, batch_norm: bool = True) -> bool:
    return H == 128 or (batch_norm and (H == 256 or (H > WIDE_CHUNK and H % WIDE_CHUNK == 0)))


def chain_eligible(H: int, batch_norm: bool) -> bool:
    return current().CHAIN and current().FUSED and H == 128 and batch_norm and _lib.split_mode()


def layers_backward_chained(idx, N: int, E: int, H: int, P: Dict[str, torch.Tensor], L: int, saved: List[LayerSaved],
                            gh, ge, outs: List[Optional[Dict[str, torch.Tensor]]], plan: Optional[dict] = None,
                            lane: Optional[SideLane] = None, first: int = 0):
    lib = _lib.load()
    dev = gh.device
    sc, sc2 = scratch(dev), scratch(dev, "chain")
    st = _stream()
    f32 = dict(dtype=torch.float32, device=dev)
    grads: List[Dict[str, torch.Tensor]] = [dict() for _ in range(L)]
    prms = [None] * L

    def tgt(i, key, *shape):
        o = outs[i] or {}
        return o[key] if key in o else torch.empty(*shape, **f32)

    def ensure(i):
        if prms[i] is None:
            prms[i] = layer_params(P, first + i)
        s = saved[i]
        if s.P is None or s.t is None:
            s.P, s.t = _proj_and_t(idx, N, E, H, prms[i], s.h_in, s.e_in, C.c_int(0))
        return prms[i], s

    def node(i, gh_out, nblk_h=None):
        prm, s = ensure(i)
        o = outs[i] or {}
        gP = torch.empty(N, 5 * H, **f32)
        Q = torch.empty(N, 2 * H, **f32)
        if nblk_h is None:
            nblk_h = C.c_int(0)
            _call("gnm_node_bwd_stats", N, H, _ptr(s.z), _ptr(s.stat_h), _ptr(gh_out), _ptr(sc.partials), C.byref(nblk_h), st)
        bstat_h, grads[i]["gamma_h"], grads[i]["beta_h"] = bn_bwd_finalize(sc.partials, nblk_h.value, N, H, dev,
                                                                          o.get("gamma_h"), o.get("beta_h"))
        _call("gnm_node_bwd_apply", N, H, _ptr(s.z), _ptr(s.stat_h), _ptr(bstat_h), _ptr(prm.gamma_h),
              _ptr(gh_out), _ptr(s.inv_f), _ptr(s.inv_b), _ptr(gP), _ptr(Q), st)
        return gP, Q

    need_f = lib.gnm_edge_bwd_fused_workspace_bytes()
    need_p = lib.gnm_node_proj_bwd_workspace_bytes(5 * H)
    need_t = lib.gnm_tn128_workspace_bytes()
    i = L - 1
    prm, s = ensure(i)
    gP, Q = node(i, gh)
    nblk = C.c_int(0)
    UT = None
    if plan is None:
        Ud, Td = torch.empty(N, H, **f32), torch.empty(N, H, **f32)
        _call("gnm_edge_bwd_dst", N, E, H, _ptr(s.e_out), _ptr(s.t), _ptr(s.stat_e), _ptr(ge), _ptr(s.P),
              _ptr(Q), _ptr(s.hf), _ptr(s.hb), _ptr(idx["isrc"]), _ptr(idx["in_ptr"]), _ptr(gP), _ptr(Ud), _ptr(Td),
              _ptr(sc.partials), C.byref(nblk), st)
    else:
        UT = torch.empty(N, 2 * H, **f32)
        DT = torch.empty(N, 2 * H, **f32)
        Ud, Td = DT[:, :H], DT[:, H:]
        ws = sc.ws(max(need_p, need_f, need_t))
        _call("gnm_edge_bwd_top", N, E, H, _ptr(ge), _ptr(s.e_out), _ptr(s.t), _ptr(s.stat_e), _ptr(s.P), _ptr(Q), _ptr(s.hf),
              _ptr(s.hb), _ptr(idx["isrc"]), _ptr(idx["idst"]), _ptr(idx["in_ptr"]), _ptr(gP), _ptr(Ud), _ptr(Td),
              _ptr(sc.partials), _ptr(plan["sinfo"]), plan["nodes_per_block"], _ptr(UT), C.byref(nblk), _ptr(ws), need_f, st)
        _call("gnm_edge_bwd_src_fix", plan["nfix"], _ptr(plan["fix_nodes"]), N, E, H, _ptr(s.e_out), _ptr(s.t),
              _ptr(s.stat_e), _ptr(ge), _ptr(Q), _ptr(idx["out_ptr"]), _ptr(idx["out_pos"]), _ptr(idx["out_dst"]),
              _ptr(gP), _ptr(UT), st)
    if current().ACTIVATIONS == "lean":
        s.P = None
    fusedn = current().NODE_FUSED and plan is not None
    at_now = tn_at(N) == "now"
    pending = None
    pending2 = None
    while True:
        prm, s = prms[i], saved[i]
        o = outs[i] or {}
        g = grads[i]
        bstat_e, g["gamma_e"], g["beta_e"] = bn_bwd_finalize(sc.partials, nblk.value, E, H, dev, o.get("gamma_e"), o.get("beta_e"))
        g["W5"], g["b5"] = tgt(i, "W5", 5 * H, H), tgt(i, "b5", 5 * H)
        gh_in = torch.empty(N, H, **f32)
        ws = sc.ws(max(need_p, need_f, need_t))
        nblk_h = None
        if fusedn:
            if pending is not None:
                lane.begin()
                lane.tn128(N, pending[0], 5 * H, 3, *pending[1:])
                pending = None
            _call("gnm_tn128_bgrad", N, H, _ptr(UT), _ptr(Ud), _ptr(Td), Ud.stride(0), _ptr(s.stat_e), _ptr(bstat_e),
                  _ptr(prm.gamma_e), _ptr(idx["in_ptr"]), _ptr(idx["out_ptr"]), _ptr(gP),
                  _ptr(s.h_in), _ptr(g["W5"][3 * H:]), _ptr(g["b5"][3 * H:]),
                  _ptr(sc.partials), _ptr(ws), need_t, st)
            del Ud, Td, Q
            UT = None
            if i > 0:
                s_j = ensure(i - 1)[1]
                nblk_h = C.c_int(0)
                _call("gnm_node_proj_bwd_nn_stats", N, H, 5 * H, _ptr(gP), _ptr(prm.W5), _ptr(gh), _ptr(gh_in), _ptr(s_j.z),
                      _ptr(s_j.stat_h), _ptr(sc.partials), C.byref(nblk_h), _ptr(ws), need_p, st)
            else:
                _call("gnm_node_proj_bwd_nn", N, H, 5 * H, _ptr(gP), _ptr(prm.W5), _ptr(gh), _ptr(gh_in), _ptr(ws), need_p, st)
            if lane is not None and at_now:
                lane.begin()
                lane.tn128(N, gP, 5 * H, 3, s.h_in, g["W5"], g["b5"])
            elif lane is not None and i > 0:
                pending = (gP, s.h_in, g["W5"], g["b5"])
            else:
                sw = sc if nblk_h is None else scratch(dev, "wgrad")
                tn128(N, gP, 5 * H, 3, s.h_in, g["W5"], g["b5"], sw.partials, sw.ws(need_t), need_t, tag="gnm_tn128[3]")
        else:
            src_cap = 0
            if pending is not None:
                pgP, ph, pW, pb = pending
                lane.begin()
                if current().TN_SPLIT and UT is not None:
                    lane.tn128(N, pgP[:, 3 * H:], 5 * H, 2, ph, pW[3 * H:], pb[3 * H:])
                    pending2 = pending
                else:
                    lane.node_proj_bwd_tn(N, H, *pending)
                pending = None
                src_cap = current().SRC_SIDE_CAP
            if UT is None:
                _call("gnm_edge_bwd_src", N, E, H, _ptr(s.e_out), _ptr(s.t), _ptr(s.stat_e), _ptr(bstat_e),
                      _ptr(prm.gamma_e), _ptr(ge), _ptr(Q), _ptr(idx["in_ptr"]), _ptr(idx["out_ptr"]),
                      _ptr(idx["out_pos"]), _ptr(idx["out_dst"]), _ptr(Ud), _ptr(Td), _ptr(gP), src_cap, st)
            else:
                _call("gnm_node_bgrad", N, H, _ptr(s.stat_e), _ptr(bstat_e), _ptr(prm.gamma_e), _ptr(idx["in_ptr"]),
                      _ptr(idx["out_ptr"]), _ptr(UT), _ptr(Ud), _ptr(Td), Ud.stride(0), _ptr(gP), st)
            split2 = UT is not None
            del Ud, Td, Q
            UT = None
            if not (lane is not None and at_now):
                _call("gnm_node_proj_bwd_nn", N, H, 5 * H, _ptr(gP), _ptr(prm.W5), _ptr(gh), _ptr(gh_in), _ptr(ws), need_p, st)
            if pending2 is not None:
                lane.wait_for_main()
                lane.tn128(N, pending2[0], 5 * H, 3, *pending2[1:])
                pending2 = None
            if lane is not None and at_now:
                lane.begin()
                lane.node_proj_bwd_tn(N, H, gP, s.h_in, g["W5"], g["b5"])
                _call("gnm_node_proj_bwd_nn", N, H, 5 * H, _ptr(gP), _ptr(prm.W5), _ptr(gh), _ptr(gh_in), _ptr(ws), need_p, st)
            elif lane is not None and i > 0:
                pending = (gP, s.h_in, g["W5"], g["b5"])
            elif lane is None and i > 0 and current().TN_SPLIT and split2:
                ws_t = sc.ws(max(need_p, need_f, need_t))
                tn128(N, gP[:, 3 * H:], 5 * H, 2, s.h_in, g["W5"][3 * H:], g["b5"][3 * H:], sc.partials, ws_t, need_t,
                      tag="gnm_node_proj_bwd_tn")
                tn128(N, gP, 5 * H, 3, s.h_in, g["W5"], g["b5"], sc.partials, ws_t, need_t, tag="gnm_node_proj_bwd_tn")
            else:
                _call("gnm_node_proj_bwd_tn", N, H, 5 * H, _ptr(gP), _ptr(s.h_in), _ptr(g["W5"]), _ptr(g["b5"]),
                      _ptr(sc.partials), _ptr(ws), need_p, 0, st)
        del gP
        gh = gh_in
        g["W3"], g["b3"] = tgt(i, "W3", H, H), tgt(i, "b3", H)
        if i == 0:
            _call("gnm_edge_bwd_fused", E, H, _ptr(ge), _ptr(ge), _ptr(s.t), _ptr(s.e_in), _ptr(s.stat_e), _ptr(bstat_e),
                  _ptr(prm.gamma_e), _ptr(prm.W3), _ptr(g["W3"]), _ptr(g["b3"]), _ptr(sc.partials), _ptr(ws), need_f, st)
            saved[0] = None
            break
        j = i - 1
        prm_j, s_j = ensure(j)
        gP, Q = node(j, gh, nblk_h)
        if plan is None:
            Ud, Td = torch.empty(N, H, **f32), torch.empty(N, H, **f32)
            _call("gnm_edge_bwd_chain", N, E, H, _ptr(ge), _ptr(ge), _ptr(s.t), _ptr(s.e_in), _ptr(s.stat_e), _ptr(bstat_e),
                  _ptr(prm.gamma_e), _ptr(prm.W3), _ptr(g["W3"]), _ptr(g["b3"]), _ptr(sc2.partials),
                  _ptr(s_j.t), _ptr(s_j.stat_e), _ptr(s_j.P), _ptr(Q), _ptr(s_j.hf), _ptr(s_j.hb),
                  _ptr(idx["isrc"]), _ptr(idx["idst"]), _ptr(idx["in_ptr"]), _ptr(gP), _ptr(Ud), _ptr(Td), _ptr(sc.partials),
                  C.byref(nblk), _ptr(ws), need_f, st)
        else:
            UT = torch.empty(N, 2 * H, **f32)
            DT = torch.empty(N, 2 * H, **f32)
            Ud, Td = DT[:, :H], DT[:, H:]
            _call("gnm_edge_bwd_chain_src", N, E, H, _ptr(ge), _ptr(ge), _ptr(s.t), _ptr(s.e_in), _ptr(s.stat_e), _ptr(bstat_e),
                  _ptr(prm.gamma_e), _ptr(prm.W3), _ptr(g["W3"]), _ptr(g["b3"]), _ptr(sc2.partials),
                  _ptr(s_j.t), _ptr(s_j.stat_e), _ptr(s_j.P), _ptr(Q), _ptr(s_j.hf), _ptr(s_j.hb),
                  _ptr(idx["isrc"]), _ptr(idx["idst"]), _ptr(idx["in_ptr"]), _ptr(gP), _ptr(Ud), _ptr(Td), _ptr(sc.partials),
                  _ptr(plan["sinfo"]), plan["nodes_per_block"], _ptr(UT), C.byref(nblk), _ptr(ws), need_f, st)
            _call("gnm_edge_bwd_src_fix", plan["nfix"], _ptr(plan["fix_nodes"]), N, E, H, _ptr(s_j.e_out), _ptr(s_j.t),
                  _ptr(s_j.stat_e), _ptr(ge), _ptr(Q), _ptr(idx["out_ptr"]), _ptr(idx["out_pos"]), _ptr(idx["out_dst"]),
                  _ptr(gP), _ptr(UT), st)
        saved[i] = None
        if current().ACTIVATIONS == "lean":
            s_j.P = None
        i = j
    return gh, ge, grads


def ln_chain_eligible(H: int, batch_norm: bool) -> bool:
    o = current()
    return (not batch_norm) and o.CHAIN and o.FUSED and o.TWO_SIDED and o.LN_SWEEP and H == 128 and _lib.split_mode()


def layers_backward_chained_ln(idx, N: int, E: int, H: int, P: Dict[str, torch.Tensor], L: int, saved: List[LayerSaved], gh, ge,
                               outs: List[Optional[Dict[str, torch.Tensor]]], plan: dict, lnw: int, lane: Optional[SideLane] = None,
                               first: int = 0):
    lib = _lib.load()
    dev = gh.device
    sc, sc2 = scratch(dev), scratch(dev, "chain")
    st = _stream()
    f32 = dict(dtype=torch.float32, device=dev)
    grads: List[Dict[str, torch.Tensor]] = [dict() for _ in range(L)]
    prms = [None] * L
    need_f = lib.gnm_edge_bwd_fused_workspace_bytes()
    need_p = lib.gnm_node_proj_bwd_workspace_bytes(5 * H)

    def tgt(i, key, *shape):
        o = outs[i] or {}
        return o[key] if key in o else torch.empty(*shape, **f32)

    def ensure(i):
        if prms[i] is None:
            prms[i] = layer_params(P, first + i)
        s = saved[i]
        _same_matmul_mode(s)
        if s.P is None or s.t is None:
            s.P, s.t = _proj_and_t(idx, N, E, H, prms[i], s.h_in, s.e_in, C.c_int(0))
        return prms[i], s

    def node(i, gh_out):
        prm, s = ensure(i)
        o = outs[i] or {}
        gP = torch.empty(N, 5 * H, **f32)
        Q = torch.empty(N, 4 * H, **f32)
        nb = C.c_int(0)
        _call("gnm_ln_node_bwd", N, H, _ptr(s.z), _ptr(prm.gamma_h), _ptr(prm.beta_h), _ptr(gh_out), _ptr(s.hf),
              _ptr(s.inv_f), _ptr(s.hb), _ptr(s.inv_b), _ptr(gP), _ptr(Q), _ptr(sc.partials), C.byref(nb), lnw, st)
        _, grads[i]["gamma_h"], grads[i]["beta_h"] = bn_bwd_finalize(sc.partials, nb.value, N, H, dev, o.get("gamma_h"), o.get("beta_h"))
        return gP, Q

    def fix_and_finalize(j, s_j, gt_j, Q_j, gP_j, nblk):
# ... 251 lines not shown
    t0 = ts[0]
    adjacent = all(t.is_contiguous() and t.dtype == t0.dtype and t.shape[1:] == t0.shape[1:] for t in ts) and all(
        a.untyped_storage().data_ptr() == b.untyped_storage().data_ptr()
        and a.data_ptr() + a.numel() * a.element_size() == b.data_ptr() for a, b in zip(ts[:-1], ts[1:]))
    if not adjacent:
        return torch.cat(ts, 0)
    rows = sum(t.shape[0] for t in ts)
    size = (rows,) + tuple(t0.shape[1:])
    stride = t0.stride()
    return torch.as_strided(t0, size, stride)


def layer_params(P: Dict[str, torch.Tensor], i: int) -> LayerParams:
    p = f"gnn.convs.{i}."
    return LayerParams(
        W5=stacked([P[p + k + ".weight"] for k in LIN5]),
        b5=stacked([P[p + k + ".bias"] for k in LIN5]),
        W3=P[p + "B_3.weight"], b3=P[p + "B_3.bias"],
        gamma_e=P[p + "bn_e.weight"], beta_e=P[p + "bn_e.bias"],
        gamma_h=P[p + "bn_h.weight"], beta_h=P[p + "bn_h.bias"])


@on_device_of(lambda graph, e_raw, pe, *a, **k: pe)
@_scoped()
def model_forward(graph, e_raw, pe, P: Dict[str, torch.Tensor], num_layers: int, save: bool, batch_norm: bool = True,
                  ln_width: Optional[int] = None, checkpoint: int = 0):
    checkpoint = _checkpoint_arg(checkpoint)
    lib = _lib.load()
    dev = pe.device
    _chk_dev(e_raw, pe)
    idx = graph.index(dev)
    N, E = graph.num_nodes(), graph.num_edges()
    H = P["linear_pe.weight"].shape[0]
    f32 = dict(dtype=torch.float32, device=dev)
    pe = node_rows_in(idx, _f32c(pe))
    e_raw = _f32c(e_raw)
    h = torch.empty(N, H, **f32)
    gemm(NT, pe, P["linear_pe.weight"], h, bias=P["linear_pe.bias"])
    Fe, Q = e_raw.shape[1], P["linear1_edge.weight"].shape[0]
    fused_enc = current().FUSED and (H == 128 or (H == 256 and current().WIDE_FUSED)) and Fe == 2 and Q == 16
    e = torch.empty(E, H, **f32)
    e_int = a1 = None
    if fused_enc:
        _call("gnm_edge_encoder_fwd", E, H, Fe, Q, _ptr(e_raw), _ptr(idx["perm"]), _ptr(P["linear1_edge.weight"]),
              _ptr(P["linear1_edge.bias"]), _ptr(P["linear2_edge.weight"]), _ptr(P["linear2_edge.bias"]),
              _ptr(e), _stream())
    else:
        e_int = torch.empty(E, Fe, **f32)
        _call("gnm_gather_rows_f32", E, Fe, _ptr(e_raw), _ptr(idx["perm"]), _ptr(e_int), _stream())
        a1 = torch.empty(E, Q, **f32)
        gemm(NT, e_int, P["linear1_edge.weight"], a1, bias=P["linear1_edge.bias"], relu=True)
        gemm(NT, a1, P["linear2_edge.weight"], e, bias=P["linear2_edge.bias"])
    ms = ModelSaved(pe=pe, e_int=e_int, a1=a1, e_raw=e_raw, opts=current(), matmul=_lib.get_matmul_mode()) if save else None
    plan2 = graph.sweep_plan(dev, GATE2_WG) if (current().TWO_SIDED_FWD and sweep_width(H, batch_norm) and hasattr(graph, "sweep_plan")) else None
    if save and checkpoint:
        ms.checkpoint = checkpoint
        firsts = {a for a, _ in checkpoint_segments(num_layers, checkpoint)}
        for i in range(num_layers):
            if i in firsts:
                ms.boundaries.append((h, e))
            h, e, _ = layer_forward(idx, N, E, H, layer_params(P, i), h, e, False, batch_norm, plan=plan2, ln_width=ln_width)
    else:
        for i in range(num_layers):
            h, e, ls = layer_forward(idx, N, E, H, layer_params(P, i), h, e, save, batch_norm, plan=plan2, ln_width=ln_width)
            if save:
                ms.layers.append(ls)
    scores, ps = predictor_forward(idx, N, E, H, P["predictor.W1.weight"], P["predictor.W1.bias"],
                                   P["predictor.W2.weight"], P["predictor.W2.bias"], h, e, save)
    if save:
        ms.pred = ps
    return scores, ms


def grad_targets(out: Dict[str, torch.Tensor], i: int) -> Optional[Dict[str, torch.Tensor]]:
    p = f"gnn.convs.{i}."
    w = [out[p + k + ".weight"] for k in LIN5]
    b = [out[p + k + ".bias"] for k in LIN5]
    W5, b5 = stacked(w), stacked(b)
    if W5.data_ptr() != w[0].data_ptr() or b5.data_ptr() != b[0].data_ptr():
        return None
    return {"W5": W5, "b5": b5, "W3": out[p + "B_3.weight"], "b3": out[p + "B_3.bias"],
            "gamma_e": out[p + "bn_e.weight"], "beta_e": out[p + "bn_e.bias"],
            "gamma_h": out[p + "bn_h.weight"], "beta_h": out[p + "bn_h.bias"]}


@on_device_of(lambda graph, P, num_layers, ms, gscores, *a, **k: gscores)
@_scoped(3)
def model_backward(graph, P: Dict[str, torch.Tensor], num_layers: int, ms: ModelSaved, gscores, batch_norm: bool = True,
                   out: Optional[Dict[str, torch.Tensor]] = None, ln_width: Optional[int] = None, inputs: bool = False):
    dev = ms.pe.device
    _same_matmul_mode(ms)
    idx = graph.index(dev)
    N, E = graph.num_nodes(), graph.num_edges()
    H = P["linear_pe.weight"].shape[0]
    f32 = dict(dtype=torch.float32, device=dev)
    G: Dict[str, torch.Tensor] = {}
    tgt = (lambda k, like: out[k]) if out else (lambda k, like: torch.empty_like(like))
    pout = {"W1": out["predictor.W1.weight"], "b1": out["predictor.W1.bias"], "W2": out["predictor.W2.weight"],
            "b2": out["predictor.W2.bias"]} if out else None
    gh, ge, gp = predictor_backward(idx, N, E, H, P["predictor.W1.weight"], P["predictor.W2.weight"],
                                    ms.pred, gscores, pout)
    G["predictor.W1.weight"], G["predictor.W1.bias"] = gp["W1"], gp["b1"]
    G["predictor.W2.weight"], G["predictor.W2.bias"] = gp["W2"], gp["b2"]
    ms.pred = None
    louts = [grad_targets(out, i) if out else None for i in range(num_layers)]
    plan_w = graph.sweep_plan(dev) if (sweep_width(H, batch_norm) and current().TWO_SIDED and not chain_eligible(H, batch_norm)
                                       and hasattr(graph, "sweep_plan")) else None
    lane = SideLane(dev) if (current().TN_SIDE and _prof is None and current().ACTIVATIONS != "lean") else None
    segs = checkpoint_segments(num_layers, ms.checkpoint) if ms.checkpoint else [(0, num_layers)]
    plan2 = (graph.sweep_plan(dev, GATE2_WG) if (ms.checkpoint and current().TWO_SIDED_FWD and sweep_width(H, batch_norm)
                                                 and hasattr(graph, "sweep_plan")) else None)
    grads = [None] * num_layers
    try:
        for si in reversed(range(len(segs))):
            a, b = segs[si]
            if ms.checkpoint:
                h, e = ms.boundaries[si]
                ms.boundaries[si] = None
                layers = []
                for i in range(a, b):
                    h, e, ls = layer_forward(idx, N, E, H, layer_params(P, i), h, e, True, batch_norm, plan=plan2, ln_width=ln_width)
                    layers.append(ls)
                del h, e, ls
            else:
                layers = ms.layers
            if chain_eligible(H, batch_norm):
                plan = graph.sweep_plan(dev) if current().TWO_SIDED and hasattr(graph, "sweep_plan") else None
                gh, ge, grads[a:b] = layers_backward_chained(idx, N, E, H, P, b - a, layers, gh, ge, louts[a:b], plan, lane, first=a)
            elif ln_chain_eligible(H, batch_norm) and plan_w is not None:
                gh, ge, grads[a:b] = layers_backward_chained_ln(idx, N, E, H, P, b - a, layers, gh, ge, louts[a:b], plan_w,
                                                                H if ln_width is None else int(ln_width), lane, first=a)
            else:
                for i in reversed(range(a, b)):
                    gh, ge, grads[i] = layer_backward(idx, N, E, H, layer_params(P, i), layers[i - a], gh, ge, batch_norm, louts[i],
                                                      plan=plan_w, ln_width=ln_width, lane=lane)
                    layers[i - a] = None
            del layers
            if lane is not None and si > 0:
                lane.drain()
    finally:
        if lane is not None:
            lane.drain()
    for i in reversed(range(num_layers)):
        p = f"gnn.convs.{i}."
        gl = grads[i]
        for j, k in enumerate(LIN5):
            G[p + k + ".weight"] = gl["W5"][j * H:(j + 1) * H]
            G[p + k + ".bias"] = gl["b5"][j * H:(j + 1) * H]
        if out and louts[i] is None:
            for j, k in enumerate(LIN5):
                G[p + k + ".weight"] = out[p + k + ".weight"].copy_(G[p + k + ".weight"])
                G[p + k + ".bias"] = out[p + k + ".bias"].copy_(G[p + k + ".bias"])
            for key, name in (("W3", "B_3.weight"), ("b3", "B_3.bias"), ("gamma_e", "bn_e.weight"), ("beta_e", "bn_e.bias"),
                              ("gamma_h", "bn_h.weight"), ("beta_h", "bn_h.bias")):
                gl[key] = out[p + name].copy_(gl[key])
        G[p + "B_3.weight"], G[p + "B_3.bias"] = gl["W3"], gl["b3"]
        G[p + "bn_e.weight"], G[p + "bn_e.bias"] = gl["gamma_e"], gl["beta_e"]
        G[p + "bn_h.weight"], G[p + "bn_h.bias"] = gl["gamma_h"], gl["beta_h"]
    lib = _lib.load()
    G["linear_pe.weight"] = tgt("linear_pe.weight", P["linear_pe.weight"])
    G["linear_pe.bias"] = gemm_tn_colsum(gh, ms.pe, G["linear_pe.weight"], out["linear_pe.bias"] if out else None)
    g_e_raw = g_pe = None
    if inputs:
        g_pe = node_rows_out(idx, gemm(NN, gh, P["linear_pe.weight"], torch.empty(N, ms.pe.shape[1], **f32)))
# ... 51 lines not shown
```

### gnnome_assembly_amd/graph.py

```python
from __future__ import annotations

import contextlib
import ctypes as C
import collections
import os
import time

import numpy as np
import torch

from . import _lib

__all__ = ["AssemblyGraph", "from_dgl", "as_assembly_graph"]

_INDEX_KEYS = ("perm", "isrc", "idst", "in_ptr", "out_ptr", "out_pos", "out_dst")

NODE_ORDER = os.environ.get("GNM_NODE_ORDER", "auto").strip().lower()
LOCAL_WINDOW = 2048
LOCAL_FRAC = 0.9


def set_node_order(mode: str) -> None:
    global NODE_ORDER
    if mode not in ("auto", "keep", "bfs"):
# ... 133 lines not shown
            if self._nrank_t is not None:
                rank = np.ascontiguousarray(self._nrank_t.cpu().numpy(), dtype=np.int32)
                order = np.ascontiguousarray(np.argsort(rank, kind="stable").astype(np.int32))
                src, dst = np.ascontiguousarray(rank[src]), np.ascontiguousarray(rank[dst])
                info = {"mode": "given", "relabelled": True}
                relabel = False
            elif mode == "auto":
                frac = C.c_double(1.0)
                _lib.check(lib.gnm_graph_edge_locality(ptr(src), ptr(dst), n, e, LOCAL_WINDOW, C.byref(frac)),
                           "gnm_graph_edge_locality")
                info["local_edge_fraction"] = frac.value
                relabel = n > LOCAL_WINDOW and frac.value < LOCAL_FRAC
            else:
                relabel = mode == "bfs"
            if relabel:
                t0 = time.perf_counter()
                order, rank = np.empty(n, np.int32), np.empty(n, np.int32)
                core = C.c_double(0.0)
                _lib.check(lib.gnm_graph_locality_order(ptr(src), ptr(dst), n, e, ptr(order), ptr(rank), C.byref(core)),
                           "gnm_graph_locality_order")
                src, dst = np.ascontiguousarray(rank[src]), np.ascontiguousarray(rank[dst])
                frac = C.c_double(1.0)
                lib.gnm_graph_edge_locality(ptr(src), ptr(dst), n, e, LOCAL_WINDOW, C.byref(frac))
                info.update(relabelled=True, seconds=time.perf_counter() - t0, triangle_edge_fraction=core.value,
                            local_edge_fraction_after=frac.value)
            self.relabel_info.clear()
            self.relabel_info.update(info)
            idx = {
                "perm": np.empty(e, np.int32), "isrc": np.empty(e, np.int32), "idst": np.empty(e, np.int32),
                "in_ptr": np.empty(n + 1, np.int32), "out_ptr": np.empty(n + 1, np.int32),
                "out_pos": np.empty(e, np.int32), "out_dst": np.empty(e, np.int32),
            }
            _lib.check(lib.gnm_graph_build_index(ptr(src), ptr(dst), n, e, *[ptr(idx[k]) for k in _INDEX_KEYS]),
                       "gnm_graph_build_index")
            if order is not None:
                idx["nperm"], idx["nrank"] = order, rank
            self._host_index = idx
        return self._host_index

    def index(self, device=None):
        device = torch.device(device) if device is not None else self.device
        if device not in self._dev_index:
            if self._src_t is not None and self._host_index is None:
                idx = tensor_index(self._src_t, self._dst_t, self._n, self._nrank_t)
                self._dev_index[self._src_t.device] = idx
                if device != self._src_t.device:
                    self._dev_index[device] = {k: v.to(device) for k, v in idx.items()}
            else:
                h = self.host_index()
                self._dev_index[device] = {k: torch.from_numpy(v).to(device) for k, v in h.items()}
        return self._dev_index[device]


    def sweep_plan(self, device=None, wg_per_cu: int = 1):
        device = torch.device(device) if device is not None else self.device
        key = (device, wg_per_cu)
        if key in self._plans:
            return self._plans[key]
        plan = None
        if (self._src_t is None or self._host_index is not None) and self.num_edges() > 0 and device.type == "cuda":
            lib = _lib.load()
            h = self.host_index()
            n, e = self._n, self.num_edges()
            npb, grid = C.c_int64(0), C.c_int(0)
            with torch.cuda.device(device):
                _lib.check(lib.gnm_sweep_partition(n, wg_per_cu, C.byref(npb), C.byref(grid)), "gnm_sweep_partition")
            plan = build_sweep_plan(h, n, npb.value)
            if plan is not None:
                plan = {k: (torch.from_numpy(v).to(device) if isinstance(v, np.ndarray) else v) for k, v in plan.items()}
        elif self.num_edges() > 0 and device.type == "cuda" and DEVICE_PLANS:
            plan = build_sweep_plan_device(self.index(device), self._n, device, wg_per_cu)
        self._plans[key] = plan
        return plan


SWEEP_TILE_ROWS, SWEEP_SLOTS, SWEEP_MARGIN = 16, 32, 1 << 16


def build_sweep_plan(host_index, n: int, nodes_per_block: int, nslots: int = SWEEP_SLOTS, margin: int = SWEEP_MARGIN):
    lib = _lib.load()
    e = int(host_index["isrc"].size)
    ptr = lambda a: a.ctypes.data_as(C.c_void_p)
    sinfo, dinfo = np.zeros(e, np.uint32), np.zeros(e, np.uint32)
    fix = np.empty(max(n, 1), np.int32)
    nfix, peak = C.c_int64(0), C.c_int(0)
    rc = lib.gnm_graph_build_sweep_plan(ptr(host_index["isrc"]), ptr(host_index["idst"]), ptr(host_index["in_ptr"]), n, e,
                                        int(nodes_per_block), SWEEP_TILE_ROWS, nslots, margin, ptr(sinfo), ptr(dinfo),
                                        ptr(fix), C.byref(nfix), C.byref(peak))
    if rc == 3:
        return None
    _lib.check(rc, "gnm_graph_build_sweep_plan")
    return {"sinfo": sinfo.view(np.int32), "dinfo": dinfo.view(np.int32), "fix_nodes": fix[:nfix.value].copy(),
            "nodes_per_block": int(nodes_per_block), "nfix": int(nfix.value), "peak_live": int(peak.value)}


DEVICE_PLANS = os.environ.get("GNM_DEVICE_PLANS", "1") != "0"


def build_sweep_plan_device(idx, n: int, device, wg_per_cu: int, nslots: int = SWEEP_SLOTS, margin: int = SWEEP_MARGIN):
    lib = _lib.load()
    e = int(idx["isrc"].numel())
    i32 = dict(dtype=torch.int32, device=device)
    npb, grid = C.c_int64(0), C.c_int(0)
    with torch.cuda.device(device):
        _lib.check(lib.gnm_sweep_partition(n, wg_per_cu, C.byref(npb), C.byref(grid)), "gnm_sweep_partition")
        if (e + 64) * 1024 >= 2 ** 31:
            b = torch.arange(0, n + npb.value, npb.value, device=device).clamp_(max=n)
            rows = idx["in_ptr"].long()[b]
            if int((rows[1:] - rows[:-1]).max()) + 64 >= 2 ** 21:
                return None
        sinfo, dinfo = torch.empty(e, **i32), torch.empty(e, **i32)
        served = torch.empty(n, dtype=torch.uint8, device=device)
        fix = torch.empty(n, **i32)
        first, last, peak = torch.empty(n, **i32), torch.empty(n, **i32), torch.empty(1, **i32)
        p = lambda t: C.c_void_p(t.data_ptr())
        _lib.check(lib.gnm_graph_build_sweep_plan_device(p(idx["isrc"]), p(idx["idst"]), p(idx["in_ptr"]), n, e, npb.value,
                                                         SWEEP_TILE_ROWS, nslots, margin, p(sinfo), p(dinfo), p(served), p(fix),
                                                         p(first), p(last), p(peak),
                                                         C.c_void_p(torch.cuda.current_stream(device).cuda_stream)),
                   "gnm_graph_build_sweep_plan_device")
    return {"sinfo": sinfo, "dinfo": dinfo, "fix_nodes": fix, "nodes_per_block": int(npb.value), "nfix": int(n),
            "peak_live": None, "served": served, "peak_dev": peak}


def _to_numpy(a):
    if isinstance(a, torch.Tensor):
        return a.detach().cpu().numpy()
    return np.asarray(a)


def from_dgl(g):
    s, d = g.edges()
    ag = AssemblyGraph(s, d, g.num_nodes())
    ag.ndata = dict(getattr(g, "ndata", {}))
    ag.edata = dict(getattr(g, "edata", {}))
    dev = getattr(g, "device", None)
    if dev is None and torch.is_tensor(s):
        dev = s.device
    return ag.to(dev) if dev is not None and torch.device(dev).type != "cpu" else ag


_WRAPPED = {}
_BY_CONTENT = collections.OrderedDict()
GRAPH_CACHE = int(os.environ.get("GNM_GRAPH_CACHE", "16"))
GRAPH_CACHE_BYTES = int(os.environ.get("GNM_GRAPH_CACHE_BYTES", str(8 << 30)))
GRAPH_CACHE_MIN_EDGES = int(os.environ.get("GNM_GRAPH_CACHE_MIN_EDGES", "65536"))


def _edge_tensors(g):
    s, d = g.edges()
    if not (torch.is_tensor(s) and torch.is_tensor(d)):
        s, d = torch.as_tensor(np.asarray(s)), torch.as_tensor(np.asarray(d))
    return s, d


def _fingerprint(g):
    s, d = _edge_tensors(g)
    w = torch.arange(1, 2 * s.numel() + 1, 2, dtype=torch.int64, device=s.device)
    h = torch.stack(((s.long() * w).sum(), (d.long() * w).sum()))
    return (int(g.num_nodes()), int(s.numel())) + tuple(int(x) for x in h.cpu())


def _same_edges(base: "AssemblyGraph", g) -> bool:
    s, d = _edge_tensors(g)
    if s.numel() != base.num_edges():
        return False
    have = base._dev_edges.get(s.device)
    if have is None and s.device.type != "cpu":
        have = (torch.from_numpy(base._src).to(s.device), torch.from_numpy(base._dst).to(s.device))
        base._dev_edges[s.device] = have
    if have is None:
        have = (torch.from_numpy(base._src), torch.from_numpy(base._dst))
    return bool(torch.equal(have[0].to(torch.int64), s.to(torch.int64)) and torch.equal(have[1].to(torch.int64), d.to(torch.int64)))


# ... 69 lines not shown
```

### include/gnm.h

```cpp
#ifndef GNM_H
#define GNM_H

#include <stddef.h>
#include <stdint.h>

#ifdef __cplusplus
extern "C" {
#endif

#define GNM_ABI_VERSION 7

#define GNM_GEMM_NT 0
#define GNM_GEMM_NN 1
#define GNM_GEMM_TN 2

int gnm_abi_version(void);
const char* gnm_last_error(void);
int gnm_num_cus(void);
int gnm_max_partial_blocks(void);
int gnm_set_occupancy_cap(int blocks_per_cu);

int gnm_graph_build_index(const int32_t* src, const int32_t* dst, int64_t N, int64_t E,
                          int32_t* perm, int32_t* isrc, int32_t* idst, int32_t* in_ptr,
                          int32_t* out_ptr, int32_t* out_pos, int32_t* out_dst);
// ... 21 lines not shown
                             const int32_t* pred_eid, uint8_t* visited, int nb, const int32_t* start_src,
                             const int32_t* start_dst, int len_threshold, int32_t* walk_out,
                             int64_t walk_cap, int64_t* best_length_out);
int64_t gnm_decode_iteration_mt(int64_t N, const float* scores, const int64_t* prefix_length,
                                const int64_t* read_length, const int32_t* succ_ptr, const int32_t* succ_nbr,
                                const int32_t* succ_eid, const int32_t* pred_ptr, const int32_t* pred_nbr,
                                const int32_t* pred_eid, uint8_t* visited, int nb, const int32_t* start_src,
                                const int32_t* start_dst, int len_threshold, int32_t* walk_out,
                                int64_t walk_cap, int64_t* best_length_out, int threads);

size_t gnm_decode_sample_workspace_bytes(int64_t E);
int gnm_decode_candidate_sums(int64_t E, int64_t N, const float* scores, const int32_t* src, const int32_t* dst,
                              const uint8_t* visited, void* ws, size_t ws_bytes, float* w_out, void* stats, void* stream);
int gnm_decode_pick(int64_t E, int64_t N, const float* scores, const int32_t* src, const int32_t* dst,
                    const uint8_t* visited, const void* ws, const void* stats, int nb, const double* u, int32_t* picks,
                    void* stream);

size_t gnm_gemm_f32_workspace_bytes(int mode, int64_t M, int64_t N, int64_t K);
int gnm_gemm_f32(int mode, int64_t M, int64_t N, int64_t K,
                 const float* A, int64_t lda, const float* B, int64_t ldb,
                 float* C, int64_t ldc,
                 const float* bias,
                 const float* resid, int64_t ldr,
                 int relu, void* ws, size_t ws_bytes, void* stream);

size_t gnm_colsum_workspace_bytes(int64_t M, int64_t W);
int gnm_colsum_f32(int64_t M, int64_t W, const float* X, int64_t ld, float* out,
                   void* ws, size_t ws_bytes, void* stream);

size_t gnm_gemm_tn_colsum_workspace_bytes(int64_t M, int64_t N, int64_t K);
int gnm_gemm_tn_colsum(int64_t M, int64_t N, int64_t K, const float* A, int64_t lda, const float* B, int64_t ldb,
                       float* C, int64_t ldc, float* colsum, void* ws, size_t ws_bytes, void* stream);

int gnm_gather_rows_f32(int64_t M, int64_t W, const float* X, const int32_t* idx, float* out,
                        void* stream);
int gnm_relu_mask_f32(int64_t n, float* x, const float* ref, void* stream);

int gnm_bn_finalize(const double* partials, int nblk, int64_t count, int H,
                    const float* gamma, const float* beta, float eps, float* stat, void* stream);
int gnm_bn_bwd_finalize(const double* partials, int nblk, int64_t count, int H,
                        float* bstat, float* ggamma, float* gbeta, void* stream);

int gnm_edge_t_stats_fwd(int64_t E, int H, float* t, const float* P, const int32_t* isrc,
                         const int32_t* idst, double* partials, int* nblk_out, void* stream);
int gnm_edge_gate_fwd(int64_t N, int64_t E, int H, const float* t, const float* e_in,
                      const float* stat_e, const float* P, const int32_t* isrc,
                      const int32_t* in_ptr, float* e_out, float* hf, float* inv_f, void* stream);
int gnm_edge_gate2_fwd(int64_t N, int64_t E, int H, const float* t, const float* e_in, const float* stat_e,
                       const float* P, const int32_t* isrc, const int32_t* idst, const int32_t* in_ptr,
                       const uint32_t* sinfo, const uint32_t* dinfo, int64_t plan_nodes_per_block, int64_t nfix,
                       const int32_t* fix_nodes, const int32_t* out_ptr, const int32_t* out_pos, const int32_t* out_dst,
                       float* e_out, float* hf, float* inv_f, float* hb, float* inv_b, float* z, double* partials,
                       int* nblk_out, void* stream);
int gnm_ln_edge_gate2_fwd(int64_t N, int64_t E, int H, const float* t, const float* e_in, const float* gamma_e,
                          const float* beta_e, int width, const float* P, const int32_t* isrc, const int32_t* idst,
                          const int32_t* in_ptr, const uint32_t* sinfo, const uint32_t* dinfo, int64_t plan_nodes_per_block,
                          int64_t nfix, const int32_t* fix_nodes, const int32_t* out_ptr, const int32_t* out_pos,
                          const int32_t* out_dst, float* e_out, float* hf, float* inv_f, float* hb, float* inv_b, float* z,
                          double* partials, int* nblk_out, void* stream);
int gnm_node_agg_src_fwd(int64_t N, int64_t E, int H, const float* e_out, const float* P,
                         const int32_t* out_ptr, const int32_t* out_pos, const int32_t* out_dst,
                         const float* hf, float* hb, float* inv_b, float* z, double* partials,
                         int* nblk_out, void* stream);
int gnm_node_update_fwd(int64_t N, int H, const float* z, const float* stat_h, const float* h_in,
                        float* h_out, void* stream);
int gnm_node_bwd_stats(int64_t N, int H, const float* z, const float* stat_h, const float* gh_out,
                       double* partials, int* nblk_out, void* stream);
int gnm_node_bwd_apply(int64_t N, int H, const float* z, const float* stat_h, const float* bstat_h,
                       const float* gamma_h, const float* gh_out, const float* inv_f, const float* inv_b,
                       float* gP, float* Q, void* stream);
int gnm_edge_bwd_dst(int64_t N, int64_t E, int H, const float* e_out, const float* t,
                     const float* stat_e, float* ge, const float* P, const float* Q,
                     const float* hf, const float* hb,
                     const int32_t* isrc, const int32_t* in_ptr, float* gP, float* Ud, float* Td,
                     double* partials, int* nblk_out, void* stream);
int gnm_edge_bwd_src(int64_t N, int64_t E, int H, const float* e_out, const float* t,
                     const float* stat_e, const float* bstat_e, const float* gamma_e,
                     const float* ge, const float* Q, const int32_t* in_ptr,
                     const int32_t* out_ptr, const int32_t* out_pos, const int32_t* out_dst,
                     const float* Ud, const float* Td, float* gP, int max_blocks_per_cu, void* stream);
int gnm_edge_bwd_gt(int64_t E, int H, const float* ge, const float* t, const float* stat_e,
                    const float* bstat_e, const float* gamma_e, float* gt, void* stream);

int gnm_ln_edge_gate_fwd(int64_t N, int64_t E, int H, const float* t, const float* e_in,
                         const float* gamma, const float* beta, const float* P, const int32_t* isrc,
                         const int32_t* in_ptr, float* e_out, float* hf, float* inv_f, int width, void* stream);
int gnm_ln_node_update_fwd(int64_t N, int H, const float* z, const float* gamma, const float* beta,
                           const float* h_in, float* h_out, int width, void* stream);
int gnm_ln_node_bwd(int64_t N, int H, const float* z, const float* gamma, const float* beta,
                    const float* gh_out, const float* hf, const float* inv_f, const float* hb,
                    const float* inv_b, float* gP, float* Q, double* partials, int* nblk_out,
                    int width, void* stream);
int gnm_ln_edge_bwd_dst(int64_t N, int64_t E, int H, const float* e_out, const float* t,
                        const float* gamma, const float* beta, float* ge, const float* P, const float* Q,
                        const int32_t* isrc, const int32_t* in_ptr, float* gP, float* gt,
                        double* partials, int* nblk_out, int width, void* stream);
int gnm_ln_edge_bwd_src(int64_t N, int64_t E, int H, const float* e_out, const float* gt, const float* Q,
                        const int32_t* out_ptr, const int32_t* out_pos, const int32_t* out_dst,
                        float* gP, void* stream);
int gnm_ln_edge_bwd_top(int64_t N, int64_t E, int H, float* ge, const float* e_out, const float* t, const float* gamma_e,
                        const float* beta_e, int width, const float* P, const float* Q, const float* hf, const float* hb,
                        const int32_t* isrc, const int32_t* idst, const int32_t* in_ptr, float* gP, float* gt,
                        double* partials, const uint32_t* sinfo, int64_t plan_nodes_per_block, int* nblk_out, void* ws,
                        size_t ws_bytes, void* stream);
int gnm_ln_edge_bwd_src_fix(int64_t nfix, const int32_t* fix_nodes, int64_t N, int64_t E, int H, const float* e_out,
                            const float* gt, const float* Q, const int32_t* out_ptr, const int32_t* out_pos,
// ... 8 lines not shown
size_t gnm_rowtile_workspace_bytes(int ncols);
int gnm_debug_set_variant(const char* what, int v);
int gnm_set_matmul_mode(int mode);
int gnm_get_matmul_mode(void);
int gnm_edge_t_fused_fwd(int64_t E, int H, const float* e_in, const float* W3, const float* b3,
                         const float* P, const int32_t* isrc, const int32_t* idst, float* t,
                         double* partials, int* nblk_out, void* ws, size_t ws_bytes, void* stream);
int gnm_edge_bwd_gt_nn(int64_t E, int H, const float* ge, const float* t, const float* stat_e, const float* bstat_e,
                       const float* gamma_e, const float* W3, float* gt, float* ge_out, void* ws, size_t ws_bytes,
                       void* stream);
int gnm_node_proj_fwd(int64_t N, int H, int ncols, const float* h, const float* W, const float* b,
                      float* Pout, void* ws, size_t ws_bytes, void* stream);
int gnm_edge_bwd_chain(int64_t N, int64_t E, int H, const float* ge, float* ge_out, const float* t_hi,
                       const float* e_mid, const float* stat_hi, const float* bstat_hi, const float* gamma_hi,
                       const float* W3_hi, float* gW3_hi, float* gb3_hi, double* partials_hi,
                       const float* t_lo, const float* stat_lo, const float* P_lo, const float* Q_lo,
                       const float* hf_lo, const float* hb_lo, const int32_t* isrc, const int32_t* idst,
                       const int32_t* in_ptr, float* gP_lo, float* Ud_lo, float* Td_lo, double* partials_lo,
                       int* nblk_out, void* ws, size_t ws_bytes, void* stream);
int gnm_edge_bwd_chain_src(int64_t N, int64_t E, int H, const float* ge, float* ge_out, const float* t_hi,
                           const float* e_mid, const float* stat_hi, const float* bstat_hi, const float* gamma_hi,
                           const float* W3_hi, float* gW3_hi, float* gb3_hi, double* partials_hi,
                           const float* t_lo, const float* stat_lo, const float* P_lo, const float* Q_lo,
                           const float* hf_lo, const float* hb_lo, const int32_t* isrc, const int32_t* idst,
                           const int32_t* in_ptr, float* gP_lo, float* Ud_lo, float* Td_lo, double* partials_lo,
                           const uint32_t* sinfo, int64_t plan_nodes_per_block, float* UT_lo,
                           int* nblk_out, void* ws, size_t ws_bytes, void* stream);
int gnm_edge_bwd_top(int64_t N, int64_t E, int H, float* ge, const float* e_out, const float* t, const float* stat_e,
                     const float* P, const float* Q, const float* hf, const float* hb, const int32_t* isrc,
                     const int32_t* idst, const int32_t* in_ptr, float* gP, float* Ud, float* Td, double* partials,
                     const uint32_t* sinfo, int64_t plan_nodes_per_block, float* UT, int* nblk_out, void* ws,
                     size_t ws_bytes, void* stream);
int gnm_edge_bwd_src_fix(int64_t nfix, const int32_t* fix_nodes, int64_t N, int64_t E, int H, const float* e_out,
                         const float* t, const float* stat_e, const float* ge, const float* Q, const int32_t* out_ptr,
                         const int32_t* out_pos, const int32_t* out_dst, float* gP, float* UT, void* stream);
int gnm_node_bgrad(int64_t N, int H, const float* stat_e, const float* bstat_e, const float* gamma_e,
                   const int32_t* in_ptr, const int32_t* out_ptr, const float* UT, const float* Ud, const float* Td,
                   int64_t ud_pitch, float* gP, void* stream);
size_t gnm_node_proj_bwd_workspace_bytes(int ncols);
int gnm_node_proj_bwd(int64_t N, int H, int ncols, const float* gP, const float* h_in, const float* W,
                      const float* gh_out, float* gh_in, float* gW, float* gb, double* partials,
                      void* ws, size_t ws_bytes, void* stream);
int gnm_node_proj_bwd_nn(int64_t N, int H, int ncols, const float* gP, const float* W, const float* gh_out,
                         float* gh_in, void* ws, size_t ws_bytes, void* stream);
int gnm_node_proj_bwd_tn(int64_t N, int H, int ncols, const float* gP, const float* h_in, float* gW, float* gb,
                         double* partials, void* ws, size_t ws_bytes, int max_blocks_per_cu, void* stream);
int gnm_node_proj_bwd_nn_stats(int64_t N, int H, int ncols, const float* gP, const float* W, const float* gh_out,
                               float* gh_in, const float* z_lo, const float* stat_h_lo, double* partials, int* nblk_out,
                               void* ws, size_t ws_bytes, void* stream);
int gnm_tn128_bgrad(int64_t M, int H, const float* UT, const float* Ud, const float* Td, int64_t ud_pitch,
                    const float* stat_e, const float* bstat_e, const float* gamma_e, const int32_t* in_ptr,
                    const int32_t* out_ptr, float* gP, const float* B, float* out, float* colsum,
                    double* partials, void* ws, size_t ws_bytes, void* stream);
size_t gnm_edge_bwd_fused_workspace_bytes(void);
int gnm_edge_bwd_fused(int64_t E, int H, const float* ge, float* ge_out, const float* t, const float* e_in,
                       const float* stat_e, const float* bstat_e, const float* gamma_e,
                       const float* W3, float* gW3, float* gb3, double* partials, void* ws,
                       size_t ws_bytes, void* stream);
int gnm_edge_bwd_fused_gt(int64_t E, int H, const float* ge, float* ge_out, const float* gt, const float* e_in,
                          const float* W3, float* gW3, float* gb3, double* partials, void* ws, size_t ws_bytes, void* stream);

int gnm_edge_encoder_fwd(int64_t E, int H, int F, int Q, const float* e_raw, const int32_t* perm,
                         const float* W1, const float* b1, const float* W2, const float* b2,
                         float* e0, void* stream);
size_t gnm_edge_encoder_bwd_workspace_bytes(void);
int gnm_edge_encoder_bwd(int64_t E, int H, int F, int Q, const float* ge0, const float* e_raw,
                         const int32_t* perm, const float* W1, const float* b1, const float* W2,
                         float* gW1, float* gb1, float* gW2, float* gb2, void* ws, size_t ws_bytes,
                         void* stream);
int gnm_edge_encoder_bwd_dx(int64_t E, int H, int F, int Q, const float* ge0, const float* e_raw,
                            const int32_t* perm, const float* W1, const float* b1, const float* W2,
                            float* gW1, float* gb1, float* gW2, float* gb2, float* ge_raw, void* ws,
                            size_t ws_bytes, void* stream);

int gnm_predictor_score_fwd(int64_t E, int HS, float* hid, const float* Pn, const int32_t* isrc,
                            const int32_t* idst, const float* W2, const float* b2,
                            const int32_t* perm, float* scores, void* stream);
int gnm_predictor_score_bwd(int64_t E, int HS, float* hid, const float* gscore, const float* W2,
                            const int32_t* perm, double* partials, int* nblk_out, void* stream);
size_t gnm_predictor_fused_workspace_bytes(void);
int gnm_predictor_fused_fwd(int64_t E, int H, int HS, const float* e, const float* W1e, int64_t ldw,
                            const float* b1, const float* Pn, const int32_t* isrc, const int32_t* idst,
                            const int32_t* perm, const float* W2, const float* b2, float* hid,
                            float* scores, void* ws, size_t ws_bytes, void* stream);
int gnm_predictor_fused_bwd(int64_t E, int H, int HS, float* hid, const float* gscore,
                            const int32_t* perm, const float* W2, const float* e, const float* W1e,
                            int64_t ldw, float* ge, float* gW1e, float* gsums, double* partials,
                            void* ws, size_t ws_bytes, void* stream);
size_t gnm_tn128_workspace_bytes(void);
int gnm_tn128(int64_t M, const float* A, int64_t lda, int ncg, const float* B, float* out, float* colsum,
              double* partials, void* ws, size_t ws_bytes, void* stream);
int gnm_reduce_partials(const double* partials, int nblk, int rows, int W, float* out, void* stream);
int gnm_seg_sum_rows(int64_t N, int W, const float* X, const int32_t* ptr, const int32_t* pos,
                     float* out, int64_t ldo, void* stream);

size_t gnm_pagerank_pe_workspace_bytes(int64_t N);
int gnm_pagerank_pe(int64_t N, int64_t E, const int32_t* isrc, const int32_t* in_ptr,
                    const int32_t* out_ptr, int pe_dim, double alpha, float* pe, void* ws,
                    size_t ws_bytes, void* stream);
int gnm_edge_feats_zscore(int64_t E, const float* overlap_length, const float* overlap_similarity,
                          float* e, void* ws, size_t ws_bytes, void* stream);

int gnm_bce_fwd_bwd(int64_t E, const float* scores, const float* y, float pos_weight,
                    float* loss_out, float* gscore, void* ws, size_t ws_bytes, void* stream);

typedef struct gnm_graph_view {
// ... 34 lines not shown
```

Before: 49.41 million.

## Accumulate per-node normalized edge sums in forward sweep to drop backward Td pass

Extends the two-sided gate2 forward sweep with a third running sum: per-node sums of the BatchNorm-normalized edge pre-activations over both incoming and outgoing edges, written into a new XT buffer. The backward chain and tn128 bgrad can then read XT instead of producing and reading the separate Td segment-sum buffer. The aim is to remove a backward-pass reduction over edges and its memory traffic. In exchange, the forward kernel uses more LDS and extra slots, which may limit occupancy, and it does additional stores during the forward pass.

After: 48.72 million. 1.4% lower.

```diff
diff --git a/gnnome_assembly_amd/_lib.py b/gnnome_assembly_amd/_lib.py
--- a/gnnome_assembly_amd/_lib.py
+++ b/gnnome_assembly_amd/_lib.py
@@ -71,6 +71,9 @@
     "gnm_graph_build_sweep_plan_device": (_i32, [_p, _p, _p, _i64, _i64, _i64, _i32, _i32, _i64, _p, _p, _p, _p, _p, _p, _p, _p]),
     "gnm_sweep_partition": (_i32, [_i64, _i32, C.POINTER(C.c_int64), _pi]),
     "gnm_edge_gate2_fwd": (_i32, [_i64, _i64, _i32] + [_p] * 9 + [_i64, _i64] + [_p] * 11 + [_pi, _p]),
+    "gnm_gate2_xt_slots": (_i32, []),
+    "gnm_edge_gate2_fwd_xt": (_i32, [_i64, _i64, _i32] + [_p] * 9 + [_i64, _i32, _i64] + [_p] * 12 + [_pi, _p]),
+    "gnm_tn128_bgrad_xt": (_i32, [_i64, _i32] + [_p] * 14 + [_sz, _p]),
     "gnm_ln_edge_gate2_fwd": (_i32, [_i64, _i64, _i32] + [_p] * 4 + [_i32] + [_p] * 6 + [_i64, _i64] + [_p] * 11 + [_pi, _p]),
     "gnm_edge_bwd_fused_workspace_bytes": (_sz, []),
     "gnm_edge_bwd_fused": (_i32, [_i64, _i32, _p, _p, _p, _p, _p, _p, _p, _p, _p, _p, _p, _p, _sz, _p]),
diff --git a/gnnome_assembly_amd/csrc/gnm_fused.hip b/gnnome_assembly_amd/csrc/gnm_fused.hip
--- a/gnnome_assembly_amd/csrc/gnm_fused.hip
+++ b/gnnome_assembly_amd/csrc/gnm_fused.hip
@@ -1787,7 +1787,7 @@
   GNM_CHECK_ARG(g_matmul_mode >= 1, "edge_bwd_chain: only built for the split matmul modes");
   GNM_CHECK_ARG(N > 0 && E > 0 && ge && ge_out && t_hi && e_mid && stat_hi && bstat_hi && gamma_hi && W3_hi && gW3_hi &&
                     gb3_hi && partials_hi && t_lo && stat_lo && P_lo && Q_lo && hf_lo && hb_lo && isrc && idst && in_ptr &&
-                    gP_lo && Ud_lo && Td_lo && partials_lo && nblk_out && partials_hi != partials_lo,
+                    gP_lo && Ud_lo && (Td_lo || sinfo) && partials_lo && nblk_out && partials_hi != partials_lo,
                 "edge_bwd_chain: null / aliased argument");
   GNM_CHECK_ARG(ws && ws_bytes >= gnm_edge_bwd_fused_workspace_bytes(), "edge_bwd_chain: workspace %zu < %zu", ws_bytes,
                 gnm_edge_bwd_fused_workspace_bytes());
@@ -1802,7 +1802,7 @@
   a.isrc = isrc; a.idst = idst; a.in_ptr = in_ptr;
   a.gP_lo = gP_lo; a.Ud_lo = Ud_lo; a.Td_lo = Td_lo; a.partials_lo = partials_lo;
   a.sinfo = sinfo; a.UT_lo = UT_lo; a.margin = kSweepMargin;
-  a.ud_pitch = Td_lo == Ud_lo + FH ? 2 * FH : FH;
+  a.ud_pitch = (!Td_lo || Td_lo == Ud_lo + FH) ? 2 * FH : FH;
   int64_t npb = 0;
   gnm_sweep_partition(N, 1, &npb, nullptr);
   GNM_CHECK_ARG((npb + 2 * kSweepMargin) * 5 * FH * 4 < (int64_t)INT32_MAX, "edge_bwd_chain: %lld nodes per workgroup exceed the 32-bit buffer offsets",
@@ -1827,7 +1827,7 @@
                                 float* UT, int* nblk_out, void* ws, size_t ws_bytes, void* stream) {
   GNM_CHECK_ARG(H == FH || (H == 2 * FH && sinfo), "edge_bwd_top: H=%d (128; 256 with a sweep plan, one sweep per 128-column half)", H);
   GNM_CHECK_ARG(N > 0 && E > 0 && ge && e_out && t && stat_e && P && Q && hf && hb && isrc && idst && in_ptr && gP && Ud &&
-                    Td && partials && nblk_out && (!sinfo || UT), "edge_bwd_top: null argument");
+                    (Td || (sinfo && H == FH)) && partials && nblk_out && (!sinfo || UT), "edge_bwd_top: null argument");
   GNM_CHECK_ARG(ws && ws_bytes >= gnm_edge_bwd_fused_workspace_bytes(), "edge_bwd_top: workspace %zu < %zu", ws_bytes,
                 gnm_edge_bwd_fused_workspace_bytes());
   int64_t npb = 0;
@@ -1843,9 +1843,9 @@
     a.slab = (float*)((char*)ws + gnm_rowtile_workspace_bytes(FH));
     a.t_lo = t + c0; a.stat_lo = stat_e + c0; a.P_lo = P + c0; a.Q_lo = Q + c0; a.hf_lo = hf + c0; a.hb_lo = hb + c0;
     a.isrc = isrc; a.idst = idst; a.in_ptr = in_ptr;
-    a.gP_lo = gP + c0; a.Ud_lo = Ud + c0; a.Td_lo = Td + c0; a.partials_lo = partials + c0;
+    a.gP_lo = gP + c0; a.Ud_lo = Ud + c0; a.Td_lo = Td ? Td + c0 : nullptr; a.partials_lo = partials + c0;
     a.sinfo = sinfo; a.UT_lo = UT ? UT + c0 : nullptr; a.margin = kSweepMargin;
-    a.ud_pitch = Td == Ud + H ? 2 * H : H;
+    a.ud_pitch = (!Td || Td == Ud + H) ? 2 * H : H;
     const int g = edge_bwd_chain_launch(a, nullptr, nullptr, (hipStream_t)stream);
     GNM_CHECK_ARG(g > 0, "edge_bwd_top: no kernel for this configuration");
     *nblk_out = g;
@@ -2224,3 +2224,16 @@
                   gP + 3 * H, (int64_t)5 * H};
   return tn_colgroups(M, nullptr, 0, 2, B, out, colsum, partials, (float*)ws, stream, 0, &cv);
 }
+
+extern "C" int gnm_tn128_bgrad_xt(int64_t M, int H, const float* UT, const float* Ud, const float* XT, const float* stat_e,
+                                  const float* bstat_e, const float* gamma_e, const int32_t* in_ptr, const int32_t* out_ptr, float* gP,
+                                  const float* B, float* out, float* colsum, double* partials, void* ws, size_t ws_bytes, void* stream) {
+  GNM_CHECK_ARG(H == FH, "tn128_bgrad_xt: H=%d (only 128 is built)", H);
+  GNM_CHECK_ARG(g_matmul_mode >= 1, "tn128_bgrad_xt: split matmul modes only");
+  GNM_CHECK_ARG(M > 0 && UT && Ud && XT && stat_e && bstat_e && gamma_e && in_ptr && out_ptr && gP && B && out && colsum && partials,
+                "tn128_bgrad_xt: bad argument");
+  GNM_CHECK_ARG(ws && ws_bytes >= gnm_tn128_workspace_bytes(), "tn128_bgrad_xt: workspace too small");
+  const TnConv cv{{UT, Ud}, {XT, XT + H}, {(int64_t)2 * H, (int64_t)2 * H}, {out_ptr, in_ptr}, stat_e, bstat_e, gamma_e,
+                  gP + 3 * H, (int64_t)5 * H};
+  return tn_colgroups(M, nullptr, 0, 2, B, out, colsum, partials, (float*)ws, stream, 0, &cv);
+}
diff --git a/gnnome_assembly_amd/csrc/gnm_sweep.hip b/gnnome_assembly_amd/csrc/gnm_sweep.hip
--- a/gnnome_assembly_amd/csrc/gnm_sweep.hip
+++ b/gnnome_assembly_amd/csrc/gnm_sweep.hip
@@ -18,9 +18,12 @@
   float* e_out; float* hf; float* inv_f; float* hb; float* inv_b;
   int64_t nodes_per_block, margin;
   const float* gamma; const float* beta; int width;
+  float* XT;
 };
 
 constexpr int G2_LDS = 3 * GR * SW * 4 + 2 * kSweepSlots * SW * 4 + 2 * 2 * SW * 4 + 2 * SW * 4 + 3 * 4 * GR * 4;
+constexpr int G2X_LDS = 4 * GR * SW * 4 + 3 * kGate2XSlots * SW * 4 + 3 * 2 * SW * 4 + 4 * SW * 4 + 3 * 4 * GR * 4;
+static_assert(2 * G2X_LDS <= 160 * 1024, "the two-sided forward sweep keeps two workgroups per CU");
 
 __device__ __forceinline__ u32x4g_ bits4g(const float4& v) {
   const u32x4g_ b = {__builtin_bit_cast(unsigned, v.x), __builtin_bit_cast(unsigned, v.y),
@@ -28,17 +31,20 @@
   return b;
 }
 
-template <bool RES, bool INV, int HF, bool LN = false>
+template <bool RES, bool INV, int HF, bool LN = false, bool XS = false>
 __global__ __launch_bounds__(GT, 4) void edge_gate2_fwd_k(const Gate2Args a) {
   static_assert(!LN || HF == SW, "the LayerNorm sweep is built for 128-wide layers");
-  __shared__ __attribute__((aligned(16))) unsigned char lds[G2_LDS];
+  static_assert(!XS || (!LN && INV && HF == SW), "the that sums: BatchNorm, 128 wide, a forward that keeps state for its backward");
+  constexpr int NSL = XS ? kGate2XSlots : kSweepSlots, NSUM = XS ? 3 : 2;
+  __shared__ __attribute__((aligned(16))) unsigned char lds[XS ? G2X_LDS : G2_LDS];
   float* i1 = reinterpret_cast<float*>(lds);
   float* i2 = i1 + GR * SW;
   float* i3 = i2 + GR * SW;
-  float* sslots = i3 + GR * SW;
-  float* dslots = sslots + 2 * kSweepSlots * SW;
-  float* cs = dslots + 2 * 2 * SW;
-  int* ring = reinterpret_cast<int*>(cs + 2 * SW);
+  float* i4 = i3 + GR * SW;
+  float* sslots = i3 + (XS ? 2 : 1) * GR * SW;
+  float* dslots = sslots + NSUM * NSL * SW;
+  float* cs = dslots + NSUM * 2 * SW;
+  int* ring = reinterpret_cast<int*>(cs + (XS ? 4 : 2) * SW);
   const int tid = threadIdx.x;
   const int row = tid >> 5, c4 = (tid & 31) * 4;
   const int chunk = xcd_chunk(blockIdx.x, gridDim.x);
@@ -49,6 +55,10 @@
   for (int c = tid; c < SW; c += GT) {
     cs[c] = LN ? a.gamma[c] : a.stat[2 * HF + c];
     cs[SW + c] = LN ? a.beta[c] : a.stat[3 * HF + c];
+    if constexpr (XS) {
+      cs[2 * SW + c] = a.stat[c];
+      cs[3 * SW + c] = a.stat[HF + c];
+    }
   }
   const int64_t vbase = v0 - a.margin;
   const int nspan = (int)(v1 - v0 + 2 * a.margin);
@@ -57,6 +67,9 @@
   const __amdgpu_buffer_rsrc_t rs_if = __builtin_amdgcn_make_buffer_rsrc(INV ? a.inv_f + v0 * HF : a.hf, 0, INV ? (int)(v1 - v0) * HF * 4 : 0, 0x00020000);
   const __amdgpu_buffer_rsrc_t rs_hb = __builtin_amdgcn_make_buffer_rsrc(a.hb + vbase * HF, 0, nspan * HF * 4, 0x00020000);
   const __amdgpu_buffer_rsrc_t rs_ib = __builtin_amdgcn_make_buffer_rsrc(INV ? a.inv_b + vbase * HF : a.hb, 0, INV ? nspan * HF * 4 : 0, 0x00020000);
+  const __amdgpu_buffer_rsrc_t rs_xs = __builtin_amdgcn_make_buffer_rsrc(XS ? a.XT + vbase * (2 * HF) : a.hb, 0, XS ? nspan * 2 * HF * 4 : 0, 0x00020000);
+  const __amdgpu_buffer_rsrc_t rs_xd = __builtin_amdgcn_make_buffer_rsrc(XS ? a.XT + v0 * (2 * HF) + HF : a.hb, 0,
+                                                                         XS && v1 > v0 ? ((int)(v1 - v0) * 2 * HF - HF) * 4 : 0, 0x00020000);
   __syncthreads();
   if (ntile == 0) return;
 
@@ -125,6 +138,7 @@
       st4(i1 + row * SW + c4, sg * ga2);
       st4(i2 + row * SW + c4, sg);
       st4(i3 + row * SW + c4, sg * ga3);
+      if constexpr (XS) st4(i4 + row * SW + c4, live ? (pt - ld4(cs + 2 * SW + c4)) * ld4(cs + 3 * SW + c4) : f4(0.f));
       ring_put(k + 1);
     }
     __syncthreads();
@@ -144,7 +158,7 @@
       float* pd = dslots + ((wd >> 16) & 1u) * SW + c4;
       float* ps = sslots + ((ws_ >> 16) & (kSweepSlots - 1)) * SW + c4;
       const float4 e1 = ld4(pd), e2 = ld4(pd + 2 * SW);
-      const float4 q1 = ld4(ps), q2 = ld4(ps + kSweepSlots * SW);
+      const float4 q1 = ld4(ps), q2 = ld4(ps + NSL * SW);
       float4 x1[3] = {f4(0.f), f4(0.f), f4(0.f)}, x2[3] = {f4(0.f), f4(0.f), f4(0.f)};
 #pragma unroll
       for (int j = 0; j < 3; ++j) {
@@ -173,7 +187,7 @@
       if (ld_ && !(wd & kSweepOpen)) { dn_ += e1; dd += e2; }
       if (ls_ && !(ws_ & kSweepOpen)) { sn_ += q1; sdn += q2; }
       if (ld_ && !(wd & kSweepClose)) { st4(pd, dn_); st4(pd + 2 * SW, dd); }
-      if (ls_ && !(ws_ & kSweepClose)) { st4(ps, sn_); st4(ps + kSweepSlots * SW, sdn); }
+      if (ls_ && !(ws_ & kSweepClose)) { st4(ps, sn_); st4(ps + NSL * SW, sdn); }
       const bool outd = ld_ && (wd & kSweepClose), outs = ls_ && (ws_ & kSweepClose);
       if (__builtin_amdgcn_ballot_w64(outd) != 0) {
         const float4 inv = make_float4(1.f / (dd.x + kEpsDen), 1.f / (dd.y + kEpsDen), 1.f / (dd.z + kEpsDen), 1.f / (dd.w + kEpsDen));
@@ -187,6 +201,35 @@
         __builtin_amdgcn_raw_buffer_store_b128(bits4g(sn_ * inv), rs_hb, o, 0, 2);
         if constexpr (INV) __builtin_amdgcn_raw_buffer_store_b128(bits4g(inv), rs_ib, o, 0, 2);
       }
+      if constexpr (XS) {
+        float4 td = ld4(pd + 4 * SW);
+        const float4 q3 = ld4(ps + 2 * NSL * SW);
+        const float4 own = ld4(i4 + row * SW + c4);
+        float4 x3[3] = {f4(0.f), f4(0.f), f4(0.f)};
+#pragma unroll
+        for (int j = 0; j < 3; ++j)
+          if (j + 1 < nd) x3[j] = ld4(i4 + (row + 1 + j) * SW + c4);
+        if (!ld_ || (wd & kSweepOpen)) td = f4(0.f);
+        td += own;
+#pragma unroll
+        for (int j = 0; j < 3; ++j) td += x3[j];
+        for (int j = 4; j < nd; ++j) td += ld4(i4 + (row + j) * SW + c4);
+        float4 ts = own;
+        unsigned m3 = ws_ & 0xffffu;
+        m3 &= m3 - 1;
+        while (m3) {
+          const int b = __builtin_ctz(m3);
+          m3 &= m3 - 1;
+          ts += ld4(i4 + b * SW + c4);
+        }
+        if (ls_ && !(ws_ & kSweepOpen)) ts += q3;
+        if (ld_ && !(wd & kSweepClose)) st4(pd + 4 * SW, td);
+        if (ls_ && !(ws_ & kSweepClose)) st4(ps + 2 * NSL * SW, ts);
+        if (__builtin_amdgcn_ballot_w64(outd) != 0)
+          __builtin_amdgcn_raw_buffer_store_b128(bits4g(td), rs_xd, outd ? ((rk[GR + row] - (int)v0) * (2 * HF) + c4) * 4 : (int)0x80000000, 0, 2);
+        if (__builtin_amdgcn_ballot_w64(outs) != 0)
+          __builtin_amdgcn_raw_buffer_store_b128(bits4g(ts), rs_xs, outs ? ((rk[row] - (int)vbase) * (2 * HF) + c4) * 4 : (int)0x80000000, 0, 2);
+      }
     }
     __syncthreads();
   };
@@ -199,7 +242,7 @@
 
 template <int HF>
 __global__ __launch_bounds__(256) void gate2_empty_segments_k(int64_t N, const int32_t* __restrict__ in_ptr,
-                                                              float* __restrict__ hf, float* __restrict__ inv_f) {
+                                                              float* __restrict__ hf, float* __restrict__ inv_f, float* __restrict__ XT) {
   const int lane = threadIdx.x & 63;
   const int64_t wave0 = ((int64_t)blockIdx.x * 4 + (threadIdx.x >> 6)) * 64;
   const int64_t stride = (int64_t)gridDim.x * 4 * 64;
@@ -212,39 +255,48 @@
       m &= m - 1;
       const int64_t u = base + b;
       const int c4 = (lane & 31) * 4;
-      if (lane < 32) st4(hf + u * HF + c4, f4(0.f));
-      else if (inv_f) st4(inv_f + u * HF + c4, f4(1.f / kEpsDen));
-    }
-  }
-}
-
-template <int HF>
+      if (lane < 32) {
+        st4(hf + u * HF + c4, f4(0.f));
+        if (XT) st4(XT + u * (2 * HF) + HF + c4, f4(0.f));
+      } else if (inv_f) {
+        st4(inv_f + u * HF + c4, f4(1.f / kEpsDen));
+      }
+    }
+  }
+}
+
+template <int HF, bool XS = false>
 __global__ __launch_bounds__(kBlock, 8) void node_agg_src_fix_k(int64_t nfix, const int32_t* __restrict__ fix_nodes,
                                                                 const float* __restrict__ e_out, const float* __restrict__ P,
                                                                 const int32_t* __restrict__ out_ptr,
                                                                 const int32_t* __restrict__ out_pos,
                                                                 const int32_t* __restrict__ out_dst, float* __restrict__ hb,
-                                                                float* __restrict__ inv_b) {
+                                                                float* __restrict__ inv_b, const float* __restrict__ t = nullptr,
+                                                                const float* __restrict__ stat = nullptr, float* __restrict__ XT = nullptr) {
   constexpr int H = SW, G = H / 4, RPW = 64 / G;
   const int lane = threadIdx.x & 63;
   const int wave = __builtin_amdgcn_readfirstlane(threadIdx.x >> 6);
   const int sub = lane / G, c4 = (lane % G) * 4;
+  const float4 mu = XS ? ld4(stat + c4) : f4(0.f), rs = XS ? ld4(stat + HF + c4) : f4(0.f);
   for (int64_t i = (int64_t)blockIdx.x * kWavesPerBlock + wave; i < nfix; i += (int64_t)gridDim.x * kWavesPerBlock) {
     const int64_t v = fix_nodes[i];
     if (v < 0) continue;
     const int a = out_ptr[v], b = out_ptr[v + 1];
-    float4 num = f4(0.f), den = f4(0.f);
+    float4 num = f4(0.f), den = f4(0.f), ts = f4(0.f);
     for (int64_t m = a + sub; m < b; m += RPW) {
       const int64_t j = out_pos[m], d = out_dst[m];
       const float4 sg = sigmoid4(ld4_nt(e_out + j * HF + c4));
       num = fma4(sg, ld4(P + d * (5 * HF) + 2 * HF + c4), num);
       den += sg;
+      if constexpr (XS) ts += (ld4_nt(t + j * HF + c4) - mu) * rs;
     }
 #pragma unroll
     for (int off = G; off < 64; off <<= 1) {
       num += shfl_xor4(num, off);
       den += shfl_xor4(den, off);
-    }
+      if constexpr (XS) ts += shfl_xor4(ts, off);
+    }
+    if constexpr (XS) { if (sub == 0) st4_nt(XT + v * (2 * HF) + c4, ts); }
     if (sub == 0) {
       const float4 inv = make_float4(1.f / (den.x + kEpsDen), 1.f / (den.y + kEpsDen), 1.f / (den.z + kEpsDen),
                                      1.f / (den.w + kEpsDen));
@@ -293,7 +345,8 @@
                                const uint32_t* sinfo, const uint32_t* dinfo, int64_t plan_nodes_per_block,
                                int64_t nfix, const int32_t* fix_nodes, const int32_t* out_ptr, const int32_t* out_pos,
                                const int32_t* out_dst, float* e_out, float* hf, float* inv_f, float* hb, float* inv_b,
-                               float* z, double* partials, int* nblk_out, void* stream) {
+                               float* z, double* partials, int* nblk_out, void* stream, float* XT = nullptr) {
+  GNM_CHECK_ARG(!XT || (H == SW && !ln_gamma && inv_f && t), "edge_gate2_fwd_xt: H = 128, BatchNorm, inv_f / inv_b wanted");
   GNM_CHECK_ARG(H == SW || (H == 2 * SW && !ln_gamma), "edge_gate2_fwd: H=%d (128 and 256 are built; LayerNorm: 128)", H);
   GNM_CHECK_ARG(N > 0 && E > 0 && t && (stat_e || ln_gamma) && P && isrc && idst && in_ptr && sinfo && dinfo && (nfix == 0 || fix_nodes) &&
                     nfix >= 0 && out_ptr && out_pos && out_dst && e_out && hf && hb && z && partials && nblk_out &&
@@ -304,12 +357,12 @@
   a.N = N; a.E = E; a.t = t; a.e_in = e_in; a.stat = stat_e; a.P = P; a.isrc = isrc; a.idst = idst; a.in_ptr = in_ptr;
   a.sinfo = sinfo; a.dinfo = dinfo; a.e_out = e_out; a.hf = hf; a.inv_f = inv_f; a.hb = hb; a.inv_b = inv_b;
   a.margin = kSweepMargin;
-  a.gamma = ln_gamma; a.beta = ln_beta; a.width = ln_width;
+  a.gamma = ln_gamma; a.beta = ln_beta; a.width = ln_width; a.XT = XT;
   int grid = 0;
   gnm_sweep_partition(N, gate2_wg(), &a.nodes_per_block, &grid);
   GNM_CHECK_ARG(plan_nodes_per_block == a.nodes_per_block, "edge_gate2_fwd: the sweep plan was built for %lld nodes per workgroup, the "
                 "kernel uses %lld (gnm_sweep_partition(N, %d))", (long long)plan_nodes_per_block, (long long)a.nodes_per_block, gate2_wg());
-  GNM_CHECK_ARG((a.nodes_per_block + 2 * kSweepMargin) * H * 4 < (int64_t)INT32_MAX && (E / grid + 64) * H * 4 < (int64_t)INT32_MAX,
+  GNM_CHECK_ARG((a.nodes_per_block + 2 * kSweepMargin) * (XT ? 2 : 1) * H * 4 < (int64_t)INT32_MAX && (E / grid + 64) * H * 4 < (int64_t)INT32_MAX,
                 "edge_gate2_fwd: a workgroup's share exceeds the 32-bit buffer offsets");
   const int gz = H == SW ? persistent_grid(N, 256, occ_blocks<node_z_stats_k<SW>>()) : persistent_grid(N, 256, occ_blocks<node_z_stats_k<2 * SW>>());
   auto run = [&](auto hf_tag, int c0) -> int {
@@ -317,7 +370,7 @@
     Gate2Args b = a;
     b.t = t + c0; b.e_in = e_in ? e_in + c0 : nullptr; b.stat = stat_e ? stat_e + c0 : nullptr; b.P = P + c0; b.e_out = e_out + c0; b.hf = hf + c0;
     b.inv_f = inv_f ? inv_f + c0 : nullptr; b.hb = hb + c0; b.inv_b = inv_b ? inv_b + c0 : nullptr;
-    hipLaunchKernelGGL(gate2_empty_segments_k<HF>, dim3(num_cus() * 2), dim3(256), 0, st, N, in_ptr, b.hf, b.inv_f);
+    hipLaunchKernelGGL(gate2_empty_segments_k<HF>, dim3(num_cus() * 2), dim3(256), 0, st, N, in_ptr, b.hf, b.inv_f, XT);
     auto launch = [&](auto ln_tag) {
       constexpr bool LN_ = decltype(ln_tag)::value;
       if (e_in && inv_f) hipLaunchKernelGGL((edge_gate2_fwd_k<true, true, HF, LN_>), dim3(grid), dim3(GT), 0, st, b);
@@ -326,7 +379,9 @@
       else hipLaunchKernelGGL((edge_gate2_fwd_k<false, false, HF, LN_>), dim3(grid), dim3(GT), 0, st, b);
     };
     if constexpr (HF == SW) {
-      if (ln_gamma) launch(std::true_type{});
+      if (XT && e_in) hipLaunchKernelGGL((edge_gate2_fwd_k<true, true, SW, false, true>), dim3(grid), dim3(GT), 0, st, b);
+      else if (XT) hipLaunchKernelGGL((edge_gate2_fwd_k<false, true, SW, false, true>), dim3(grid), dim3(GT), 0, st, b);
+      else if (ln_gamma) launch(std::true_type{});
       else launch(std::false_type{});
     } else {
       launch(std::false_type{});
@@ -336,8 +391,14 @@
       int64_t g2 = (nfix + kWavesPerBlock - 1) / kWavesPerBlock;
       const int64_t cap = (int64_t)num_cus() * 8;
       if (g2 > cap) g2 = cap;
-      hipLaunchKernelGGL(node_agg_src_fix_k<HF>, dim3((int)g2), dim3(kBlock), 0, st, nfix, fix_nodes, b.e_out, b.P, out_ptr, out_pos,
-                         out_dst, b.hb, b.inv_b);
+      if constexpr (HF == SW) {
+        if (XT)
+          hipLaunchKernelGGL((node_agg_src_fix_k<HF, true>), dim3((int)g2), dim3(kBlock), 0, st, nfix, fix_nodes, b.e_out, b.P, out_ptr,
+                             out_pos, out_dst, b.hb, b.inv_b, b.t, b.stat, XT);
+      }
+      if (!XT)
+        hipLaunchKernelGGL((node_agg_src_fix_k<HF, false>), dim3((int)g2), dim3(kBlock), 0, st, nfix, fix_nodes, b.e_out, b.P, out_ptr, out_pos,
+                           out_dst, b.hb, b.inv_b, (const float*)nullptr, (const float*)nullptr, (float*)nullptr);
       GNM_LAUNCH_CHECK("edge_gate2_fwd fix");
     }
     hipLaunchKernelGGL(node_z_stats_k<HF>, dim3(gz), dim3(kBlock), 0, st, N, b.P, b.hf, b.hb, z + c0, partials + c0, (N + gz - 1) / gz);
@@ -375,3 +436,17 @@
   return edge_gate2_fwd_impl(N, E, H, t, e_in, nullptr, gamma_e, beta_e, width, P, isrc, idst, in_ptr, sinfo, dinfo, plan_nodes_per_block, nfix,
                              fix_nodes, out_ptr, out_pos, out_dst, e_out, hf, inv_f, hb, inv_b, z, partials, nblk_out, stream);
 }
+
+extern "C" int gnm_gate2_xt_slots(void) { return kGate2XSlots; }
+extern "C" int gnm_edge_gate2_fwd_xt(int64_t N, int64_t E, int H, const float* t, const float* e_in, const float* stat_e,
+                                     const float* P, const int32_t* isrc, const int32_t* idst, const int32_t* in_ptr,
+                                     const uint32_t* sinfo, const uint32_t* dinfo, int64_t plan_nodes_per_block, int plan_nslots,
+                                     int64_t nfix, const int32_t* fix_nodes, const int32_t* out_ptr, const int32_t* out_pos,
+                                     const int32_t* out_dst, float* e_out, float* hf, float* inv_f, float* hb, float* inv_b,
+                                     float* z, float* XT, double* partials, int* nblk_out, void* stream) {
+  GNM_CHECK_ARG(stat_e && XT, "edge_gate2_fwd_xt: stat_e / XT is null");
+  GNM_CHECK_ARG(plan_nslots >= 1 && plan_nslots <= kGate2XSlots, "edge_gate2_fwd_xt: the sweep plan uses %d slots, the kernel has %d",
+                plan_nslots, kGate2XSlots);
+  return edge_gate2_fwd_impl(N, E, H, t, e_in, stat_e, nullptr, nullptr, 0, P, isrc, idst, in_ptr, sinfo, dinfo, plan_nodes_per_block, nfix,
+                             fix_nodes, out_ptr, out_pos, out_dst, e_out, hf, inv_f, hb, inv_b, z, partials, nblk_out, stream, XT);
+}
diff --git a/gnnome_assembly_amd/csrc/gnm_tr.h b/gnnome_assembly_amd/csrc/gnm_tr.h
--- a/gnnome_assembly_amd/csrc/gnm_tr.h
+++ b/gnnome_assembly_amd/csrc/gnm_tr.h
@@ -200,6 +200,7 @@
 
 constexpr int kSweepTileRows = 16;
 constexpr int kSweepSlots = 32;
+constexpr int kGate2XSlots = 24;
 constexpr int64_t kSweepMargin = 1 << 16;
 constexpr unsigned kSweepOpen = 1u << 22, kSweepClose = 1u << 23;
 
diff --git a/gnnome_assembly_amd/csrc/gnm_tr.hip b/gnnome_assembly_amd/csrc/gnm_tr.hip
--- a/gnnome_assembly_amd/csrc/gnm_tr.hip
+++ b/gnnome_assembly_amd/csrc/gnm_tr.hip
@@ -648,8 +648,9 @@
 
 struct W3Frag16 { bf16x8 w[SW / 32][3]; };
 
-template <int ABL, bool SRC, bool WSKIP = true, bool HI = true, int HF = SW, bool H2 = false, bool LN = false>
+template <int ABL, bool SRC, bool WSKIP = true, bool HI = true, int HF = SW, bool H2 = false, bool LN = false, bool XF = false>
 __global__ __launch_bounds__(CT, 2) void edge_bwd_chain_k(const ChainArgs a) {
+  static_assert(!XF || (SRC && !LN && HF == SW), "that sums from the forward: the two-sided BatchNorm sweep, 128 wide");
   static_assert(HF == SW || !HI, "the chained (matrix) half of the kernel is built for 128-wide layers only");
   static_assert(HI || !H2, "f16x2 belongs to the matrix half");
   static_assert(!LN || (SRC && HF == SW), "the LayerNorm sweep: two-sided, 128 wide");
@@ -732,7 +733,7 @@
   const int trq0 = simg_tr_base(lane, 0), trq1 = simg_tr_base(lane, 1);
   const int ni = lane & 15, ng = lane >> 4;
   const int nnb = ni * SPITCH + ((((ni & 3) << 2) | (ng ^ (swz(ni) & 3))) << 4);
-  const bool walker = wave < 3 && lane < 32 && !(LN && wave == 1), bnsum = tid >= 256;
+  const bool walker = wave < 3 && lane < 32 && !((LN || XF) && wave == 1), bnsum = tid >= 256;
   const int role = wave, wc4 = (tid & 31) * 4;
   const int brow = 2 * ((tid - 256) >> 5);
   int cur = -1;
@@ -1049,11 +1050,11 @@
           const int b = rr[u];
           s1[u] = ld4(v5 + b * SW + wc4);
           s2[u] = ld4(v2 + b * SW + wc4);
-          s3[u] = ld4(v3 + b * SW + wc4);
+          if constexpr (!XF) s3[u] = ld4(v3 + b * SW + wc4);
           const float* p = slots + ((w[u] >> 16) & (kSweepSlots - 1)) * SW + wc4;
           p1[u] = ld4(p);
           p2[u] = ld4(p + kSweepSlots * SW);
-          p3[u] = ld4(p + 2 * kSweepSlots * SW);
+          if constexpr (!XF) p3[u] = ld4(p + 2 * kSweepSlots * SW);
           m[u] &= m[u] - 1;
         }
 #pragma unroll
@@ -1063,19 +1064,19 @@
             m[u] &= m[u] - 1;
             s1[u] += ld4(v5 + b * SW + wc4);
             s2[u] += ld4(v2 + b * SW + wc4);
-            s3[u] += ld4(v3 + b * SW + wc4);
+            if constexpr (!XF) s3[u] += ld4(v3 + b * SW + wc4);
           }
           const bool lead = (w[u] & 0xffffu) != 0;
           if (lead && !(w[u] & kSweepOpen)) {
             s1[u] += p1[u];
             s2[u] += p2[u];
-            s3[u] += p3[u];
+            if constexpr (!XF) s3[u] += p3[u];
           }
           float* p = slots + ((w[u] >> 16) & (kSweepSlots - 1)) * SW + wc4;
           if (lead && !(w[u] & kSweepClose)) {
             st4(p, s1[u]);
             st4(p + kSweepSlots * SW, s2[u]);
-            st4(p + 2 * kSweepSlots * SW, s3[u]);
+            if constexpr (!XF) st4(p + 2 * kSweepSlots * SW, s3[u]);
           }
           const bool out = lead && (w[u] & kSweepClose);
           const int sn = sdk[rr[u]] - (int)vbase;
@@ -1084,7 +1085,7 @@
           if (!(ABL & 16) && __builtin_amdgcn_ballot_w64(out) != 0) {
             __builtin_amdgcn_raw_buffer_store_b128(bits4(s1[u]), srs_g, og_, 0, 0);
             __builtin_amdgcn_raw_buffer_store_b128(bits4(s2[u]), srs_u, ou_, 0, 0);
-            if constexpr (!LN) __builtin_amdgcn_raw_buffer_store_b128(bits4(s3[u]), srs_u, ou_, HF * 4, 0);
+            if constexpr (!LN && !XF) __builtin_amdgcn_raw_buffer_store_b128(bits4(s3[u]), srs_u, ou_, HF * 4, 0);
           }
         }
       }
@@ -1160,7 +1161,7 @@
       const int c4 = (lane & 31) * 4;
       if (lane < 32) {
         st4(gP + u * (5 * HF) + 2 * HF + c4, f4(0.f));
-        st4(Td + u * ud_pitch + c4, f4(0.f));
+        if (Td) st4(Td + u * ud_pitch + c4, f4(0.f));
       } else {
         st4(Ud + u * ud_pitch + c4, f4(0.f));
       }
@@ -1178,8 +1179,8 @@
   int grid = 0;
   gnm_sweep_partition(a.N, 1, &a.nodes_per_block, &grid);
   if (a.hfull == 2 * SW) {
+    if (a.t_hi || !a.sinfo || !a.Td_lo) return -1;
     hipLaunchKernelGGL(zero_empty_segments_k<2 * SW>, dim3(num_cus() * 2), dim3(256), 0, st, a.N, a.in_ptr, a.gP_lo, a.Ud_lo, a.Td_lo, a.ud_pitch);
-    if (a.t_hi || !a.sinfo) return -1;
     hipLaunchKernelGGL((edge_bwd_chain_k<0, true, true, false, 2 * SW>), dim3(grid), dim3(CT), 0, st, a);
     return grid;
   }
@@ -1197,6 +1198,13 @@
     default: break;
   }
 #endif
+  if (!a.Td_lo) {
+    if (!a.sinfo || a.ln_gamma) return -1;
+    if (!a.t_hi) hipLaunchKernelGGL((edge_bwd_chain_k<0, true, true, false, SW, false, false, true>), dim3(grid), dim3(CT), 0, st, a);
+    else if (h2) hipLaunchKernelGGL((edge_bwd_chain_k<0, true, true, true, SW, true, false, true>), dim3(grid), dim3(CT), 0, st, a);
+    else hipLaunchKernelGGL((edge_bwd_chain_k<0, true, true, true, SW, false, false, true>), dim3(grid), dim3(CT), 0, st, a);
+    return grid;
+  }
   if (!a.t_hi) {
     if (a.ln_gamma) {
       if (!a.sinfo || !a.gt_out || !a.ln_beta) return -1;
diff --git a/gnnome_assembly_amd/engine.py b/gnnome_assembly_amd/engine.py
--- a/gnnome_assembly_amd/engine.py
+++ b/gnnome_assembly_amd/engine.py
@@ -42,6 +42,8 @@
             raise _lib.GnmError(f"engine.options: unknown switch {bad}; known: {_OPTION_NAMES}")
         if "ACTIVATIONS" in kw and kw["ACTIVATIONS"] not in ("saved", "lean"):
             raise _lib.GnmError(f"activation mode {kw['ACTIVATIONS']!r}: expected 'saved' or 'lean'")
+        if "TWO_SIDED_FWD" in kw and kw["TWO_SIDED_FWD"] not in (True, False, "xt"):
+            raise _lib.GnmError(f"TWO_SIDED_FWD {kw['TWO_SIDED_FWD']!r}: expected True, False or 'xt'")
         if "TN_AT" in kw and kw["TN_AT"] not in ("now", "next", "auto"):
             raise _lib.GnmError(f"TN_AT {kw['TN_AT']!r}: expected 'now', 'next' or 'auto'")
         d = {k: getattr(self, k) for k in _OPTION_NAMES}
@@ -405,6 +407,7 @@
     inv_b: torch.Tensor = None
     z: torch.Tensor = None
     stat_h: torch.Tensor = None
+    xt: torch.Tensor = None
     opts: "Options" = None
     chunks: list = None
     matmul: str = None
@@ -463,6 +466,7 @@
     hf = torch.empty(N, H, **f32)
     two_sided = plan is not None and (H in (128, 256) if batch_norm else H == 128) and current().TWO_SIDED_FWD
     inv_f = torch.empty(N, H, **f32) if (save or not two_sided) else None
+    xt = None
     if two_sided and not batch_norm:
         hb = torch.empty(N, H, **f32)
         inv_b = torch.empty(N, H, **f32) if save else None
@@ -477,10 +481,18 @@
         inv_b = torch.empty(N, H, **f32) if save else None
         z = torch.empty(N, H, **f32)
         stat_e = bn_finalize(sc.partials, nblk.value, E, H, prm.gamma_e, prm.beta_e)
-        _call("gnm_edge_gate2_fwd", N, E, H, _ptr(t), res_e, _ptr(stat_e), _ptr(P), _ptr(idx["isrc"]), _ptr(idx["idst"]),
-              _ptr(idx["in_ptr"]), _ptr(plan["sinfo"]), _ptr(plan["dinfo"]), plan["nodes_per_block"], plan["nfix"],
-              _ptr(plan["fix_nodes"]), _ptr(idx["out_ptr"]), _ptr(idx["out_pos"]), _ptr(idx["out_dst"]), _ptr(e_out),
-              _ptr(hf), _ptr(inv_f), _ptr(hb), _ptr(inv_b), _ptr(z), _ptr(sc.partials), C.byref(nblk), st)
+        if save and xt_forward(H, batch_norm) and plan.get("nslots", 1 << 30) <= lib.gnm_gate2_xt_slots():
+            xt = torch.empty(N, 2 * H, **f32)
+            _call("gnm_edge_gate2_fwd_xt", N, E, H, _ptr(t), res_e, _ptr(stat_e), _ptr(P), _ptr(idx["isrc"]), _ptr(idx["idst"]),
+                  _ptr(idx["in_ptr"]), _ptr(plan["sinfo"]), _ptr(plan["dinfo"]), plan["nodes_per_block"], plan["nslots"], plan["nfix"],
+                  _ptr(plan["fix_nodes"]), _ptr(idx["out_ptr"]), _ptr(idx["out_pos"]), _ptr(idx["out_dst"]), _ptr(e_out),
+                  _ptr(hf), _ptr(inv_f), _ptr(hb), _ptr(inv_b), _ptr(z), _ptr(xt), _ptr(sc.partials), C.byref(nblk), st,
+                  tag="gnm_edge_gate2_fwd")
+        else:
+            _call("gnm_edge_gate2_fwd", N, E, H, _ptr(t), res_e, _ptr(stat_e), _ptr(P), _ptr(idx["isrc"]), _ptr(idx["idst"]),
+                  _ptr(idx["in_ptr"]), _ptr(plan["sinfo"]), _ptr(plan["dinfo"]), plan["nodes_per_block"], plan["nfix"],
+                  _ptr(plan["fix_nodes"]), _ptr(idx["out_ptr"]), _ptr(idx["out_pos"]), _ptr(idx["out_dst"]), _ptr(e_out),
+                  _ptr(hf), _ptr(inv_f), _ptr(hb), _ptr(inv_b), _ptr(z), _ptr(sc.partials), C.byref(nblk), st)
     elif batch_norm:
         stat_e = bn_finalize(sc.partials, nblk.value, E, H, prm.gamma_e, prm.beta_e)
         _call("gnm_edge_gate_fwd", N, E, H, _ptr(t), res_e, _ptr(stat_e), _ptr(P), _ptr(idx["isrc"]),
@@ -507,7 +519,7 @@
     if save:
         lean = current().ACTIVATIONS == "lean"
         saved = LayerSaved(opts=current(), h_in=h_in, e_in=e_in, P=None if lean else P, t=None if lean else t, stat_e=stat_e, e_out=e_out,
-                           hf=hf, inv_f=inv_f, hb=hb, inv_b=inv_b, z=z, stat_h=stat_h, matmul=_lib.get_matmul_mode())
+                           hf=hf, inv_f=inv_f, hb=hb, inv_b=inv_b, z=z, stat_h=stat_h, xt=xt, matmul=_lib.get_matmul_mode())
     return h_out, e_out, saved
 
 
@@ -807,7 +819,7 @@
 
 
 _D_TWO_SIDED = os.environ.get("GNM_TWO_SIDED", "1") != "0"
-_D_TWO_SIDED_FWD = os.environ.get("GNM_TWO_SIDED_FWD", "1") != "0"
+_D_TWO_SIDED_FWD = {"0": False, "xt": "xt"}.get(os.environ.get("GNM_TWO_SIDED_FWD", "1").strip().lower(), True)
 _D_WIDE_FUSED = os.environ.get("GNM_WIDE_FUSED", "1") != "0"
 
 
@@ -828,6 +840,17 @@
 
 def chain_eligible(H: int, batch_norm: bool) -> bool:
     return current().CHAIN and current().FUSED and H == 128 and batch_norm and _lib.split_mode()
+
+
+def xt_forward(H: int, batch_norm: bool) -> bool:
+    o = current()
+    return o.TWO_SIDED_FWD == "xt" and o.TWO_SIDED and o.NODE_FUSED and chain_eligible(H, batch_norm)
+
+
+def gate2_plan(graph, dev, H: int, batch_norm: bool):
+    if xt_forward(H, batch_norm):
+        return graph.sweep_plan(dev, GATE2_WG, nslots=_lib.load().gnm_gate2_xt_slots())
+    return graph.sweep_plan(dev, GATE2_WG)
 
 
 def layers_backward_chained(idx, N: int, E: int, H: int, P: Dict[str, torch.Tensor], L: int, saved: List[LayerSaved],
@@ -866,6 +889,9 @@
         _call("gnm_node_bwd_apply", N, H, _ptr(s.z), _ptr(s.stat_h), _ptr(bstat_h), _ptr(prm.gamma_h),
               _ptr(gh_out), _ptr(s.inv_f), _ptr(s.inv_b), _ptr(gP), _ptr(Q), st)
         return gP, Q
+
+    def xt_of(s):
+        return s.xt is not None and plan is not None and current().NODE_FUSED
 
     need_f = lib.gnm_edge_bwd_fused_workspace_bytes()
     need_p = lib.gnm_node_proj_bwd_workspace_bytes(5 * H)
@@ -886,7 +912,7 @@
         Ud, Td = DT[:, :H], DT[:, H:]
         ws = sc.ws(max(need_p, need_f, need_t))
         _call("gnm_edge_bwd_top", N, E, H, _ptr(ge), _ptr(s.e_out), _ptr(s.t), _ptr(s.stat_e), _ptr(s.P), _ptr(Q), _ptr(s.hf),
-              _ptr(s.hb), _ptr(idx["isrc"]), _ptr(idx["idst"]), _ptr(idx["in_ptr"]), _ptr(gP), _ptr(Ud), _ptr(Td),
+              _ptr(s.hb), _ptr(idx["isrc"]), _ptr(idx["idst"]), _ptr(idx["in_ptr"]), _ptr(gP), _ptr(Ud), _ptr(None if xt_of(s) else Td),
               _ptr(sc.partials), _ptr(plan["sinfo"]), plan["nodes_per_block"], _ptr(UT), C.byref(nblk), _ptr(ws), need_f, st)
         _call("gnm_edge_bwd_src_fix", plan["nfix"], _ptr(plan["fix_nodes"]), N, E, H, _ptr(s.e_out), _ptr(s.t),
               _ptr(s.stat_e), _ptr(ge), _ptr(Q), _ptr(idx["out_ptr"]), _ptr(idx["out_pos"]), _ptr(idx["out_dst"]),
@@ -911,10 +937,16 @@
                 lane.begin()
                 lane.tn128(N, pending[0], 5 * H, 3, *pending[1:])
                 pending = None
-            _call("gnm_tn128_bgrad", N, H, _ptr(UT), _ptr(Ud), _ptr(Td), Ud.stride(0), _ptr(s.stat_e), _ptr(bstat_e),
-                  _ptr(prm.gamma_e), _ptr(idx["in_ptr"]), _ptr(idx["out_ptr"]), _ptr(gP),
-                  _ptr(s.h_in), _ptr(g["W5"][3 * H:]), _ptr(g["b5"][3 * H:]),
-                  _ptr(sc.partials), _ptr(ws), need_t, st)
+            if xt_of(s):
+                _call("gnm_tn128_bgrad_xt", N, H, _ptr(UT), _ptr(Ud), _ptr(s.xt), _ptr(s.stat_e), _ptr(bstat_e),
+                      _ptr(prm.gamma_e), _ptr(idx["in_ptr"]), _ptr(idx["out_ptr"]), _ptr(gP),
+                      _ptr(s.h_in), _ptr(g["W5"][3 * H:]), _ptr(g["b5"][3 * H:]),
+                      _ptr(sc.partials), _ptr(ws), need_t, st, tag="gnm_tn128_bgrad")
+            else:
+                _call("gnm_tn128_bgrad", N, H, _ptr(UT), _ptr(Ud), _ptr(Td), Ud.stride(0), _ptr(s.stat_e), _ptr(bstat_e),
+                      _ptr(prm.gamma_e), _ptr(idx["in_ptr"]), _ptr(idx["out_ptr"]), _ptr(gP),
+                      _ptr(s.h_in), _ptr(g["W5"][3 * H:]), _ptr(g["b5"][3 * H:]),
+                      _ptr(sc.partials), _ptr(ws), need_t, st)
             del Ud, Td, Q
             UT = None
             if i > 0:
@@ -999,8 +1031,8 @@
             _call("gnm_edge_bwd_chain_src", N, E, H, _ptr(ge), _ptr(ge), _ptr(s.t), _ptr(s.e_in), _ptr(s.stat_e), _ptr(bstat_e),
                   _ptr(prm.gamma_e), _ptr(prm.W3), _ptr(g["W3"]), _ptr(g["b3"]), _ptr(sc2.partials),
                   _ptr(s_j.t), _ptr(s_j.stat_e), _ptr(s_j.P), _ptr(Q), _ptr(s_j.hf), _ptr(s_j.hb),
-                  _ptr(idx["isrc"]), _ptr(idx["idst"]), _ptr(idx["in_ptr"]), _ptr(gP), _ptr(Ud), _ptr(Td), _ptr(sc.partials),
-                  _ptr(plan["sinfo"]), plan["nodes_per_block"], _ptr(UT), C.byref(nblk), _ptr(ws), need_f, st)
+                  _ptr(idx["isrc"]), _ptr(idx["idst"]), _ptr(idx["in_ptr"]), _ptr(gP), _ptr(Ud), _ptr(None if xt_of(s_j) else Td),
+                  _ptr(sc.partials), _ptr(plan["sinfo"]), plan["nodes_per_block"], _ptr(UT), C.byref(nblk), _ptr(ws), need_f, st)
             _call("gnm_edge_bwd_src_fix", plan["nfix"], _ptr(plan["fix_nodes"]), N, E, H, _ptr(s_j.e_out), _ptr(s_j.t),
                   _ptr(s_j.stat_e), _ptr(ge), _ptr(Q), _ptr(idx["out_ptr"]), _ptr(idx["out_pos"]), _ptr(idx["out_dst"]),
                   _ptr(gP), _ptr(UT), st)
@@ -1358,7 +1390,7 @@
         gemm(NT, e_int, P["linear1_edge.weight"], a1, bias=P["linear1_edge.bias"], relu=True)
         gemm(NT, a1, P["linear2_edge.weight"], e, bias=P["linear2_edge.bias"])
     ms = ModelSaved(pe=pe, e_int=e_int, a1=a1, e_raw=e_raw, opts=current(), matmul=_lib.get_matmul_mode()) if save else None
-    plan2 = graph.sweep_plan(dev, GATE2_WG) if (current().TWO_SIDED_FWD and sweep_width(H, batch_norm) and hasattr(graph, "sweep_plan")) else None
+    plan2 = gate2_plan(graph, dev, H, batch_norm) if (current().TWO_SIDED_FWD and sweep_width(H, batch_norm) and hasattr(graph, "sweep_plan")) else None
     if save and checkpoint:
         ms.checkpoint = checkpoint
         firsts = {a for a, _ in checkpoint_segments(num_layers, checkpoint)}
@@ -1414,8 +1446,8 @@
                                        and hasattr(graph, "sweep_plan")) else None
     lane = SideLane(dev) if (current().TN_SIDE and _prof is None and current().ACTIVATIONS != "lean") else None
     segs = checkpoint_segments(num_layers, ms.checkpoint) if ms.checkpoint else [(0, num_layers)]
-    plan2 = (graph.sweep_plan(dev, GATE2_WG) if (ms.checkpoint and current().TWO_SIDED_FWD and sweep_width(H, batch_norm)
-                                                 and hasattr(graph, "sweep_plan")) else None)
+    plan2 = (gate2_plan(graph, dev, H, batch_norm) if (ms.checkpoint and current().TWO_SIDED_FWD and sweep_width(H, batch_norm)
+                                                       and hasattr(graph, "sweep_plan")) else None)
     grads = [None] * num_layers
     try:
         for si in reversed(range(len(segs))):
diff --git a/gnnome_assembly_amd/graph.py b/gnnome_assembly_amd/graph.py
--- a/gnnome_assembly_amd/graph.py
+++ b/gnnome_assembly_amd/graph.py
@@ -209,9 +209,10 @@
         return self._dev_index[device]
 
 
-    def sweep_plan(self, device=None, wg_per_cu: int = 1):
+    def sweep_plan(self, device=None, wg_per_cu: int = 1, nslots=None):
         device = torch.device(device) if device is not None else self.device
-        key = (device, wg_per_cu)
+        nslots = SWEEP_SLOTS if nslots is None else int(nslots)
+        key = (device, wg_per_cu) if nslots == SWEEP_SLOTS else (device, wg_per_cu, nslots)
         if key in self._plans:
             return self._plans[key]
         plan = None
@@ -222,11 +223,11 @@
             npb, grid = C.c_int64(0), C.c_int(0)
             with torch.cuda.device(device):
                 _lib.check(lib.gnm_sweep_partition(n, wg_per_cu, C.byref(npb), C.byref(grid)), "gnm_sweep_partition")
-            plan = build_sweep_plan(h, n, npb.value)
+            plan = build_sweep_plan(h, n, npb.value, nslots=nslots)
             if plan is not None:
                 plan = {k: (torch.from_numpy(v).to(device) if isinstance(v, np.ndarray) else v) for k, v in plan.items()}
         elif self.num_edges() > 0 and device.type == "cuda" and DEVICE_PLANS:
-            plan = build_sweep_plan_device(self.index(device), self._n, device, wg_per_cu)
+            plan = build_sweep_plan_device(self.index(device), self._n, device, wg_per_cu, nslots=nslots)
         self._plans[key] = plan
         return plan
 
@@ -248,7 +249,7 @@
         return None
     _lib.check(rc, "gnm_graph_build_sweep_plan")
     return {"sinfo": sinfo.view(np.int32), "dinfo": dinfo.view(np.int32), "fix_nodes": fix[:nfix.value].copy(),
-            "nodes_per_block": int(nodes_per_block), "nfix": int(nfix.value), "peak_live": int(peak.value)}
+            "nodes_per_block": int(nodes_per_block), "nfix": int(nfix.value), "peak_live": int(peak.value), "nslots": int(nslots)}
 
 
 DEVICE_PLANS = os.environ.get("GNM_DEVICE_PLANS", "1") != "0"
@@ -277,7 +278,7 @@
                                                          C.c_void_p(torch.cuda.current_stream(device).cuda_stream)),
                    "gnm_graph_build_sweep_plan_device")
     return {"sinfo": sinfo, "dinfo": dinfo, "fix_nodes": fix, "nodes_per_block": int(npb.value), "nfix": int(n),
-            "peak_live": None, "served": served, "peak_dev": peak}
+            "peak_live": None, "served": served, "peak_dev": peak, "nslots": int(nslots)}
 
 
 def _to_numpy(a):
diff --git a/include/gnm.h b/include/gnm.h
--- a/include/gnm.h
+++ b/include/gnm.h
@@ -97,6 +97,13 @@
                        const int32_t* fix_nodes, const int32_t* out_ptr, const int32_t* out_pos, const int32_t* out_dst,
                        float* e_out, float* hf, float* inv_f, float* hb, float* inv_b, float* z, double* partials,
                        int* nblk_out, void* stream);
+int gnm_gate2_xt_slots(void);
+int gnm_edge_gate2_fwd_xt(int64_t N, int64_t E, int H, const float* t, const float* e_in, const float* stat_e,
+                          const float* P, const int32_t* isrc, const int32_t* idst, const int32_t* in_ptr,
+                          const uint32_t* sinfo, const uint32_t* dinfo, int64_t plan_nodes_per_block, int plan_nslots,
+                          int64_t nfix, const int32_t* fix_nodes, const int32_t* out_ptr, const int32_t* out_pos,
+                          const int32_t* out_dst, float* e_out, float* hf, float* inv_f, float* hb, float* inv_b, float* z,
+                          float* XT, double* partials, int* nblk_out, void* stream);
 int gnm_ln_edge_gate2_fwd(int64_t N, int64_t E, int H, const float* t, const float* e_in, const float* gamma_e,
                           const float* beta_e, int width, const float* P, const int32_t* isrc, const int32_t* idst,
                           const int32_t* in_ptr, const uint32_t* sinfo, const uint32_t* dinfo, int64_t plan_nodes_per_block,
@@ -211,6 +218,9 @@
                     const float* stat_e, const float* bstat_e, const float* gamma_e, const int32_t* in_ptr,
                     const int32_t* out_ptr, float* gP, const float* B, float* out, float* colsum,
                     double* partials, void* ws, size_t ws_bytes, void* stream);
+int gnm_tn128_bgrad_xt(int64_t M, int H, const float* UT, const float* Ud, const float* XT, const float* stat_e,
+                       const float* bstat_e, const float* gamma_e, const int32_t* in_ptr, const int32_t* out_ptr, float* gP,
+                       const float* B, float* out, float* colsum, double* partials, void* ws, size_t ws_bytes, void* stream);
 size_t gnm_edge_bwd_fused_workspace_bytes(void);
 int gnm_edge_bwd_fused(int64_t E, int H, const float* ge, float* ge_out, const float* t, const float* e_in,
                        const float* stat_e, const float* bstat_e, const float* gamma_e,
```
